# blackle/Megalania

Measured on AMD Instinct MI355X. Metric: SA neighbour-cost evals/s, higher is better.
Workload: dtype u64

## Files before the change

megalania_amd/csrc/mgl_api.hip:

```cpp
#include "mgl_kernels.hip"
#include "mgl_kernels2.hip"
#include "mgl_kernels3.hip"
#include "mgl_kernels4.hip"
#include "mgl_kernels5.hip"
#include "mgl_pbuild.hip"
#include "mgl_index.hip"
#include "../../include/megalania_hip.h"

#include <math.h>
#include <stdio.h>
#include <stdlib.h>
#include <string.h>
#include <string>
#include <vector>

static const uint16_t k_cost_table[2048] = {
#include "mgl_cost_table.inc"
};

#define MGL_MAX_INPUT 176000000ull
static thread_local std::string g_err;
static int fail(int code, const std::string& msg)
{
	g_err = msg;
	return code;
}
#define HIPCHK(expr)                                                                         \
	do {                                                                                     \
		hipError_t e_ = (expr);                                                              \
		if (e_ != hipSuccess)                                                                \
			return fail(MGL_EDEVICE, std::string(#expr) + ": " + hipGetErrorString(e_));     \
	} while (0)

__attribute__((constructor)) static void mgl_more_hw_queues(void) { if (getenv("MGL_LOOKAHEAD")) setenv("GPU_MAX_HW_QUEUES", "8", 0); }

extern "C" const char* mgl_version(void) { return "megalania-hip 0.1 (gfx950)"; }
extern "C" const char* mgl_last_error(void) { return g_err.c_str(); }
extern "C" int mgl_device_count(void)
{
	int n = 0;
	if (hipGetDeviceCount(&n) != hipSuccess) return 0;
	return n;
}
extern "C" uint32_t mgl_rng_draw_at(uint64_t seed, uint64_t step, uint32_t j, uint32_t n)
{
	return mgl_rng_draw(mgl_rng_key(seed, step, j), n);
}

struct BaseMem {
	BaseView v;
	Control* ctl;
};

struct mgl_sa {
	int device;
	hipStream_t stream;
	hipStream_t stream2;
	hipEvent_t ev_fork, ev_join;
	hipEvent_t ev_tgt = nullptr, ev_tgt_go = nullptr;
	int tgt_ahead = 0;
	hipStream_t stream3 = nullptr;
	hipEvent_t ev_rest[8] = { nullptr, nullptr, nullptr, nullptr, nullptr, nullptr, nullptr, nullptr }, ev_sim = nullptr;
	uint32_t halves;
	uint32_t n;
	mgl_properties props;
	mgl_sa_config cfg;
	uint64_t temperature = 0;
	DevCtx ctx;
	uint8_t* d_data;
	uint32_t* d_bucket_off;
	uint32_t* d_bucket_pos;
	uint16_t* d_bucket_nx;
	uint32_t* d_quad_pos;
	uint16_t* d_quad_nx;
	uint32_t *d_quad_rank = nullptr, *d_quad_run = nullptr;
	uint32_t* d_xpos[6] = { nullptr, nullptr, nullptr, nullptr, nullptr, nullptr };
	uint32_t* d_xrank[6] = { nullptr, nullptr, nullptr, nullptr, nullptr, nullptr };
	uint32_t* d_xrun[6] = { nullptr, nullptr, nullptr, nullptr, nullptr, nullptr };
	uint8_t* d_xnxb[6] = { nullptr, nullptr, nullptr, nullptr, nullptr, nullptr };
	uint32_t *d_oct_pos = nullptr, *d_oct_rank = nullptr, *d_oct_run = nullptr;
	uint32_t *d_hex_pos = nullptr, *d_hex_rank = nullptr, *d_hex_run = nullptr;
	uint64_t *d_oct_nx8 = nullptr, *d_hex_nx8 = nullptr;
	uint16_t* d_cost_tbl;
	BaseMem base, scratch;
	mgl_pk* d_best;
	NbrOut nbr;
	uint32_t* d_aos;
	uint64_t* d_cum;
	uint16_t* d_final_probs;
	mgl_pk* d_topk_pk;
	uint64_t* d_topk_cost;
	uint32_t* d_small;
	uint32_t* d_sub_offs;
	uint32_t* d_sub_lens;
	uint32_t sub_cap;
	uint64_t sqrt_thresh;
	uint32_t per_wave_bytes, waves_per_block, nbr_lds, walk_lds;
	bool incremental;
	Base2 b2;
	unsigned long long* d_prof;
	uint32_t* d_todo;
	uint32_t per_wave2, waves_per_block2, nbr2_lds, build_lds;
	uint32_t chg_cap = MGL_CHG_CAP;
	uint32_t per_wave_pick, per_wave_rest, pick_waves;
	size_t b2_bytes;
	BigScratch big;
	uint32_t* d_todo2;
	uint32_t* d_todo3 = nullptr;
	uint4* d_pickstate;
	uint4* d_pickrec;
	bool split_nbr, adaptive;
	bool form_single = false;
	uint32_t* d_counts;
	ApplyBuf ab;
	uint32_t apply_blocks;
	bool incremental_apply;
	bool snapshots;
	Base2 snap_lit, snap_best;
	SnapMeta* d_snap_meta;
	bool parallel_build;
	PBuild pb;
	hipEvent_t ev_begin, ev_end;
	std::vector<hipEvent_t> ev_pool;
	int accept_mode = MGL_ACCEPT_AUTO;
	uint32_t bulk_threshold = 0;
	bool bulk_now = true;
	uint64_t bulk_hold = 0;
	uint64_t blk_done = 0;
	uint64_t blk_imp0 = 0, blk_acc0 = 0;
	BulkBuf bulk;
	BatchBuf batch;
	bool batch_ok = false;
	uint32_t* d_strat_tgt = nullptr;
	uint32_t* d_strat_pre = nullptr;
	bool select_small = false;
	uint32_t* h_bstat = nullptr;
	hipEvent_t ev_bstat = nullptr;
	uint32_t force_batch_fail = 0;
	uint64_t batch_accepts = 0, batch_fallbacks = 0;
	std::vector<uint8_t> mode_log;
	uint32_t force_rollbacks = 0;
	uint64_t bulk_rollbacks = 0;
	bool best_unverified = false;
	struct NbrSet { NbrOut nbr; uint4* pickrec; uint4* pickstate; uint4* sim_hdr; uint16_t* sim_keys; uint32_t* sim_pos; uint32_t* todo; uint32_t* counts; };
	NbrSet alt = {};
	uint32_t sim_waves = MGL_SIM_WAVES;
	std::vector<hipEvent_t> ev_sim_pool;
	int64_t time_sim_step = -1;
	bool count_traffic = false;
	unsigned long long* d_traffic = nullptr;
	bool la_enabled = false, la_ready = false;
	hipGraph_t nbr_graph = nullptr; hipGraphExec_t nbr_graph_exec = nullptr; uint64_t nbr_graph_key = 0; bool graph_ok = false;
	uint32_t short_looks = 0;
	uint8_t* d_la_mark = nullptr;
	uint32_t* d_la_list = nullptr;
	uint32_t* d_la_hdr = nullptr;
	hipStream_t stream5 = nullptr, stream6 = nullptr;
	hipEvent_t ev_val = nullptr;
	hipEvent_t ev_la_check = nullptr, ev_la_zero = nullptr, ev_redo = nullptr, ev_spec[8] = { nullptr, nullptr, nullptr, nullptr, nullptr, nullptr, nullptr, nullptr };
};

static uint64_t ceil_sqrt_u64(uint64_t x)
{
	uint64_t r = (uint64_t)sqrt((double)x);
	while (r * r > x) r--;
	while ((r + 1) * (r + 1) <= x) r++;
	return r * r == x ? r : r + 1;
}

static void dfree(void* p) { if (p) (void)hipFree(p); }
static void free_base(BaseMem& b)
{
	dfree(b.v.slab); dfree(b.v.onwalk); dfree(b.v.ckpt_probs); dfree(b.v.ckpt_hdr); dfree(b.ctl);
	memset(&b, 0, sizeof b);
}
static hipError_t alloc_base(BaseMem& b, uint32_t n, uint32_t ckpt_elems)
{
	memset(&b, 0, sizeof b);
	hipError_t e;
	b.v.nckpt = (n + (1u << MGL_CKPT_SHIFT) - 1u) >> MGL_CKPT_SHIFT;
	b.v.ckpt_elems = ckpt_elems;
	if ((e = hipMalloc(&b.v.slab, sizeof(mgl_pk) * (size_t)n)) != hipSuccess) return e;
	if ((e = hipMalloc(&b.v.onwalk, sizeof(uint64_t) * (((size_t)n + 63) / 64 + 1))) != hipSuccess) return e;
	if ((e = hipMalloc(&b.v.ckpt_probs, sizeof(uint16_t) * (size_t)b.v.nckpt * ckpt_elems)) != hipSuccess) return e;
	if ((e = hipMalloc(&b.v.ckpt_hdr, sizeof(CkptHdr) * (size_t)b.v.nckpt)) != hipSuccess) return e;
	if ((e = hipMalloc(&b.ctl, sizeof(Control))) != hipSuccess) return e;
	if ((e = hipMemset(b.v.onwalk, 0, sizeof(uint64_t) * (((size_t)n + 63) / 64 + 1))) != hipSuccess) return e;
	return hipMemset(b.ctl, 0, sizeof(Control));
}

static size_t b2_pool_entries(const Base2& b) { return (size_t)b.pool_cap + 256; }
static int alloc_b2(Base2& b, size_t n, bool own_slab, bool init, size_t* bytes_out)
{
	size_t bytes = 0;
	if (own_slab) {
		HIPCHK(hipMalloc(&b.slab, sizeof(mgl_pk) * n)); bytes += sizeof(mgl_pk) * n;
		HIPCHK(hipMalloc(&b.onwalk, sizeof(uint64_t) * ((n + 63) / 64 + 1)));
	}
	HIPCHK(hipMalloc(&b.sp0, sizeof(uint64_t) * (b.nw0 + 64))); bytes += sizeof(uint64_t) * (b.nw0 + 64);
	HIPCHK(hipMalloc(&b.sp1, sizeof(uint64_t) * (b.nw1 + 64)));
	HIPCHK(hipMalloc(&b.sp2, sizeof(uint64_t) * (b.nw2 + 64)));
	HIPCHK(hipMalloc(&b.sp_state, sizeof(uint32_t) * 8 * n)); bytes += sizeof(uint32_t) * 8 * n;
	HIPCHK(hipMalloc(&b.ck_probs, sizeof(uint16_t) * (size_t)b.nck * b.ck_elems)); bytes += sizeof(uint16_t) * (size_t)b.nck * b.ck_elems;
	HIPCHK(hipMalloc(&b.ch_off, sizeof(uint32_t) * b.ck_elems));
	HIPCHK(hipMalloc(&b.ch_len, sizeof(uint32_t) * b.ck_elems));
	HIPCHK(hipMalloc(&b.ch_cap, sizeof(uint32_t) * b.ck_elems));
	HIPCHK(hipMalloc(&b.ch_pos, sizeof(uint32_t) * b2_pool_entries(b))); bytes += sizeof(uint32_t) * (size_t)b.pool_cap;
	HIPCHK(hipMalloc(&b.ch_ev, sizeof(uint16_t) * b2_pool_entries(b))); bytes += sizeof(uint16_t) * (size_t)b.pool_cap;
	HIPCHK(hipMalloc(&b.pool_top, sizeof(uint32_t)));
	HIPCHK(hipMalloc(&b.ch_sb, sizeof(uint32_t) * (size_t)b.ck_elems * b.sb_stride)); bytes += sizeof(uint32_t) * (size_t)b.ck_elems * b.sb_stride;
	if (init) {
		HIPCHK(hipMemset(b.ch_sb, 0, sizeof(uint32_t) * (size_t)b.ck_elems * b.sb_stride));
		HIPCHK(hipMemset(b.sp0, 0, sizeof(uint64_t) * (b.nw0 + 64)));
		HIPCHK(hipMemset(b.sp1, 0, sizeof(uint64_t) * (b.nw1 + 64)));
		HIPCHK(hipMemset(b.sp2, 0, sizeof(uint64_t) * (b.nw2 + 64)));
		HIPCHK(hipMemset(b.ch_pos, 0xFF, sizeof(uint32_t) * b2_pool_entries(b)));
		HIPCHK(hipMemset(b.ch_ev, 0, sizeof(uint16_t) * b2_pool_entries(b)));
	}
	if (bytes_out) *bytes_out = bytes;
	return MGL_OK;
}
static void free_b2(Base2& b, bool own_slab)
{
	if (own_slab) { dfree(b.slab); dfree(b.onwalk); }
	dfree(b.sp0); dfree(b.sp1); dfree(b.sp2); dfree(b.sp_state); dfree(b.ck_probs);
	dfree(b.ch_off); dfree(b.ch_len); dfree(b.ch_cap); dfree(b.ch_pos); dfree(b.ch_ev); dfree(b.pool_top); dfree(b.ch_sb);
	memset(&b, 0, sizeof b);
}
static int launch_snapshot(mgl_sa* sa, Base2& snap, uint32_t which, int dir, int cond)
{
	const Base2& from = dir == 0 ? sa->b2 : snap;
	const Base2& to = dir == 0 ? snap : sa->b2;
	const size_t n = sa->n;
	SnapPlan p;
	memset(&p, 0, sizeof p);
	uint32_t k = 0;
	auto seg = [&](const void* s, void* d, size_t bytes, uint32_t pool_elem) {
		p.seg[k].src = s; p.seg[k].dst = d; p.seg[k].bytes = bytes; p.seg[k].pool_elem = pool_elem; k++;
	};
	seg(from.slab, to.slab, sizeof(mgl_pk) * n, 0);
	seg(from.onwalk, to.onwalk, sizeof(uint64_t) * ((n + 63) / 64 + 1), 0);
	seg(from.sp0, to.sp0, sizeof(uint64_t) * (from.nw0 + 64), 0);
	seg(from.sp1, to.sp1, sizeof(uint64_t) * (from.nw1 + 64), 0);
	seg(from.sp2, to.sp2, sizeof(uint64_t) * (from.nw2 + 64), 0);
	seg(from.sp_state, to.sp_state, sizeof(uint32_t) * 8 * n, 0);
	seg(from.ck_probs, to.ck_probs, sizeof(uint16_t) * (size_t)from.nck * from.ck_elems, 0);
	seg(from.ch_off, to.ch_off, sizeof(uint32_t) * from.ck_elems, 0);
	seg(from.ch_len, to.ch_len, sizeof(uint32_t) * from.ck_elems, 0);
	seg(from.ch_cap, to.ch_cap, sizeof(uint32_t) * from.ck_elems, 0);
	seg(from.ch_pos, to.ch_pos, sizeof(uint32_t) * b2_pool_entries(from), 4);
	seg(from.ch_ev, to.ch_ev, sizeof(uint16_t) * b2_pool_entries(from), 2);
	seg(from.pool_top, to.pool_top, sizeof(uint32_t), 0);
	seg(from.ch_sb, to.ch_sb, sizeof(uint32_t) * (size_t)from.ck_elems * from.sb_stride, 0);
	p.nseg = k;
	p.src_pool_top = from.pool_top;
// ... 78 lines not shown
	hipLaunchKernelGGL(k_apply_walk, dim3(1), dim3(64), 0, sa->stream, sa->ctx, sa->b2, sa->base.ctl, sa->nbr, sa->ab);
	if (next_gstep != ~0ull) { int rc = launch_targets_ahead(sa, next_gstep); if (rc) return rc; }
	if (!sa->snapshots)
		hipLaunchKernelGGL(k_copy_best, dim3(256), dim3(256), 0, sa->stream, (const Control*)sa->base.ctl,
		                   (const mgl_pk*)sa->base.v.slab, sa->d_best, sa->ctx.n);
	hipLaunchKernelGGL(k_apply_chains, dim3(sa->apply_blocks), dim3(MGL_APPLY_THREADS), 0, sa->stream, sa->ctx, sa->b2, sa->base.ctl, sa->ab);
	hipLaunchKernelGGL(k_apply_jobs, dim3(1024), dim3(256), 0, sa->stream, sa->b2, (const Control*)sa->base.ctl, sa->ab, 0, (const uint32_t*)nullptr);
	hipLaunchKernelGGL(k_apply_jobs, dim3(1024), dim3(256), 0, sa->stream, sa->b2, (const Control*)sa->base.ctl, sa->ab, 1, (const uint32_t*)nullptr);
	hipLaunchKernelGGL(k_build_end, dim3(1), dim3(64), sa->build_lds, sa->stream, sa->ctx, sa->b2, sa->base.ctl, sa->snapshots ? 1 : 0, sa->d_counts, sa->adaptive ? 1 : 0, sa->form_single ? 1 : 0);
	HIPCHK(hipGetLastError());
	return MGL_OK;
}
static const bool g_trace = getenv("MGL_TRACE") != nullptr, g_prof_big = getenv("MGL_PROF_BIG") != nullptr, g_big_inline_sim = getenv("MGL_BIG_INLINE_SIM") != nullptr;
#define NBR_TRACE(name) do { if (g_trace) { fprintf(stderr, "[mgl] %s\n", name); hipError_t e_ = hipDeviceSynchronize(); if (e_ != hipSuccess) fprintf(stderr, "[mgl] %s -> %s\n", name, hipGetErrorString(e_)); } } while (0)
static hipEvent_t sim_event(mgl_sa* sa, size_t i)
{
	while (sa->ev_sim_pool.size() <= i) {
		hipEvent_t e = nullptr;
		if (hipEventCreate(&e) != hipSuccess) return nullptr;
		sa->ev_sim_pool.push_back(e);
	}
	return sa->ev_sim_pool[i];
}
static mgl_sa::NbrSet cur_set(const mgl_sa* sa)
{
	mgl_sa::NbrSet t = { sa->nbr, sa->d_pickrec, sa->d_pickstate, sa->big.sim_hdr, sa->big.sim_keys, sa->big.sim_pos, sa->d_todo, sa->d_counts };
	return t;
}
static void use_set(mgl_sa* sa, const mgl_sa::NbrSet& t)
{
	sa->nbr = t.nbr; sa->d_pickrec = t.pickrec; sa->d_pickstate = t.pickstate;
	sa->big.sim_hdr = t.sim_hdr; sa->big.sim_keys = t.sim_keys; sa->big.sim_pos = t.sim_pos;
	sa->d_todo = t.todo; sa->d_counts = t.counts;
	sa->big.todo_in = t.todo; sa->big.todo_in_count = t.counts; sa->big.spill_ctr = t.counts + 2;
}
static uint32_t nbr_slices(const mgl_sa* sa)
{
	const uint32_t K = sa->cfg.neighbours_per_step;
	return (sa->halves >= 2 && K >= 1024) ? sa->halves : 1u;
}
static int launch_pick_rest(mgl_sa* sa, const mgl_sa::NbrSet& t, uint64_t step_override, hipStream_t s_even, hipStream_t s_odd, hipEvent_t* done)
{
	const uint32_t K = sa->cfg.neighbours_per_step, slices = nbr_slices(sa);
	BigScratch g = sa->big;
	g.sim_hdr = t.sim_hdr; g.sim_keys = t.sim_keys; g.sim_pos = t.sim_pos;
	g.todo_in = t.todo; g.todo_in_count = t.counts; g.spill_ctr = t.counts + 2;
	for (uint32_t h = 0; h < slices; h++) {
		const uint32_t j0 = (uint32_t)((uint64_t)K * h / slices), j1 = (uint32_t)((uint64_t)K * (h + 1) / slices);
		hipStream_t st = (h & 1u) ? s_odd : s_even;
		hipLaunchKernelGGL((k_neighbours2<false, MGL_NBR_PICK>), dim3((j1 - j0 + sa->pick_waves - 1) / sa->pick_waves), dim3(64 * sa->pick_waves),
		                   (MGL_PICK_T_GLOBAL ? 0u : 4096u) + sa->pick_waves * sa->per_wave_pick, st, sa->ctx,
		                   sa->b2, sa->base.ctl, sa->cfg.seed, step_override, K, t.nbr, sa->per_wave_pick, t.todo, t.counts,
		                   (unsigned long long*)nullptr, g, t.pickrec, j0, j1, t.pickstate); NBR_TRACE("k_neighbours2<false, MGL_NBR_PICK>");
		hipLaunchKernelGGL((k_neighbours2<false, MGL_NBR_REST>), dim3(j1 - j0), dim3(64), sa->per_wave_rest, st, sa->ctx,
		                   sa->b2, sa->base.ctl, sa->cfg.seed, step_override, K, t.nbr, sa->per_wave_rest, t.todo, t.counts,
		                   g_prof_big ? (unsigned long long*)nullptr : sa->d_prof, g, t.pickrec, j0, j1, t.pickstate); NBR_TRACE("k_neighbours2<false, MGL_NBR_REST>");
		HIPCHK(hipEventRecord(done[h], st));
	}
	HIPCHK(hipGetLastError());
	return MGL_OK;
}
static int launch_lookahead(mgl_sa* sa, uint64_t gstep_next, bool after_check)
{
	const uint32_t slices = nbr_slices(sa);
	if (after_check) HIPCHK(hipStreamWaitEvent(sa->stream5, sa->ev_la_check, 0));
	else for (uint32_t h = 0; h < slices; h++) HIPCHK(hipStreamWaitEvent(sa->stream5, sa->ev_rest[h], 0));
	HIPCHK(hipMemsetAsync(sa->alt.counts, 0, 8 * sizeof(uint32_t), sa->stream5));
	HIPCHK(hipEventRecord(sa->ev_la_zero, sa->stream5));
	HIPCHK(hipStreamWaitEvent(sa->stream6, sa->ev_la_zero, 0));
	int rc = launch_pick_rest(sa, sa->alt, gstep_next, sa->stream5, sa->stream6, sa->ev_spec);
	if (rc) return rc;
	sa->la_ready = true;
	return MGL_OK;
}
static void launch_targets(mgl_sa* sa, hipStream_t st, uint64_t step_override)
{
	const uint32_t K = sa->cfg.neighbours_per_step;
	const uint64_t* onwalk = sa->incremental ? sa->b2.onwalk : sa->base.v.onwalk;
	const uint32_t nw0 = sa->incremental ? sa->b2.nw0 : (sa->ctx.n + 63u) >> 6;
	hipLaunchKernelGGL(k_rank_blocks, dim3(sa->ctx.strat_nblk), dim3(64), 0, st, onwalk, nw0, sa->d_strat_pre, sa->ctx.strat_nblk);
	hipLaunchKernelGGL(k_rank_scan, dim3(1), dim3(1024), 0, st, sa->d_strat_pre, sa->ctx.strat_nblk);
	hipLaunchKernelGGL(k_targets, dim3((K + 3u) / 4u), dim3(256), 0, st, sa->ctx, onwalk, nw0, (const Control*)sa->base.ctl, sa->cfg.seed, step_override, K, sa->d_strat_tgt);
}
static int launch_targets_ahead(mgl_sa* sa, uint64_t next_gstep)
{
	if (!sa->d_strat_pre || !sa->incremental) return MGL_OK;
	HIPCHK(hipEventRecord(sa->ev_tgt_go, sa->stream));
	HIPCHK(hipStreamWaitEvent(sa->stream2, sa->ev_tgt_go, 0));
	launch_targets(sa, sa->stream2, next_gstep);
	HIPCHK(hipEventRecord(sa->ev_tgt, sa->stream2));
	HIPCHK(hipGetLastError());
	sa->tgt_ahead = 1;
	return MGL_OK;
}
static uint64_t graph_key(const mgl_sa* sa);
static int launch_neighbours_body(mgl_sa* sa, uint64_t step_override, bool from_lookahead)
{
	const uint32_t K = sa->cfg.neighbours_per_step;
	const uint32_t blocks2 = (K + sa->waves_per_block2 - 1) / sa->waves_per_block2;
	const bool split_now = sa->split_nbr && !sa->form_single;
	const uint32_t sim_lds_regular = ((((sa->ctx.L.total + 31u) >> 5) + 3u) & ~3u) * 4u + sa->chg_cap * 16u;
	if (split_now) {
		const uint32_t slices = nbr_slices(sa);
		if (!from_lookahead) {
			HIPCHK(hipEventRecord(sa->ev_fork, sa->stream));
			if (slices >= 2) HIPCHK(hipStreamWaitEvent(sa->stream2, sa->ev_fork, 0));
			HIPCHK(hipStreamWaitEvent(sa->stream3, sa->ev_fork, 0));
			int rc = launch_pick_rest(sa, cur_set(sa), step_override, sa->stream, sa->stream2, sa->ev_rest);
			if (rc) return rc;
		} else {
			HIPCHK(hipMemsetAsync(sa->d_la_hdr, 0, 2 * sizeof(uint32_t), sa->stream));
			hipLaunchKernelGGL(k_la_check, dim3((K + 255u) / 256u), dim3(256), 0, sa->stream, sa->ctx, sa->b2, (const Control*)sa->base.ctl, sa->nbr,
			                   (const uint4*)sa->d_pickstate, sa->big.sim_hdr, (const uint32_t*)sa->d_counts, sa->d_la_mark, sa->d_la_list, sa->d_la_hdr, sa->cfg.seed, K); NBR_TRACE("k_la_check");
			HIPCHK(hipEventRecord(sa->ev_la_check, sa->stream));
			HIPCHK(hipStreamWaitEvent(sa->stream3, sa->ev_la_check, 0));
			HIPCHK(hipStreamWaitEvent(sa->stream2, sa->ev_la_check, 0));
		}
		for (uint32_t h = 0; h < slices; h++) {
			const uint32_t j0 = (uint32_t)((uint64_t)K * h / slices), j1 = (uint32_t)((uint64_t)K * (h + 1) / slices);
			if (!from_lookahead) HIPCHK(hipStreamWaitEvent(sa->stream3, sa->ev_rest[h], 0));
			if (sa->time_sim_step >= 0 && h < 2) HIPCHK(hipEventRecord(sim_event(sa, 6 * (size_t)sa->time_sim_step + 2 * h), sa->stream3));
			if (sa->count_traffic)
				hipLaunchKernelGGL(k_sim<true>, dim3(j1 - j0), dim3(64 * sa->sim_waves), sim_lds_regular, sa->stream3, sa->ctx, sa->b2, sa->base.ctl,
				                   sa->nbr, sa->big, j0, j1, sa->d_todo3, sa->d_counts + 4, (const uint32_t*)nullptr, (const uint32_t*)nullptr, sa->d_traffic);
			else
				hipLaunchKernelGGL(k_sim<false>, dim3(j1 - j0), dim3(64 * sa->sim_waves), sim_lds_regular, sa->stream3, sa->ctx, sa->b2, sa->base.ctl,
				                   sa->nbr, sa->big, j0, j1, sa->d_todo3, sa->d_counts + 4, (const uint32_t*)nullptr, (const uint32_t*)nullptr, (unsigned long long*)nullptr);
			NBR_TRACE("k_sim");
			if (sa->time_sim_step >= 0 && h < 2) HIPCHK(hipEventRecord(sim_event(sa, 6 * (size_t)sa->time_sim_step + 2 * h + 1), sa->stream3));
		}
		HIPCHK(hipEventRecord(sa->ev_sim, sa->stream3));
		if (!from_lookahead) {
			for (uint32_t h = 1; h < slices; h += 2) HIPCHK(hipStreamWaitEvent(sa->stream, sa->ev_rest[h], 0));
		} else {
			BigScratch g = sa->big;
			g.la_list = sa->d_la_list; g.la_count = sa->d_la_hdr;
			const uint32_t grid = blocks2 < 4096u ? blocks2 : 4096u;
			hipLaunchKernelGGL((k_neighbours2<false, MGL_NBR_FULL, true>), dim3(grid), dim3(64 * sa->waves_per_block2), sa->nbr2_lds, sa->stream2, sa->ctx,
			                   sa->b2, sa->base.ctl, sa->cfg.seed, step_override, K, sa->nbr, sa->per_wave2, sa->d_todo, sa->d_counts,
			                   sa->d_prof, g, sa->d_pickrec, 0u, K, sa->d_pickstate); NBR_TRACE("k_neighbours2<false, MGL_NBR_FULL, true>");
			HIPCHK(hipEventRecord(sa->ev_redo, sa->stream2));
		}
	}
	if (!sa->split_nbr || sa->form_single) {
		hipLaunchKernelGGL((k_neighbours2<false, MGL_NBR_FULL>), dim3(blocks2), dim3(64 * sa->waves_per_block2), sa->nbr2_lds, sa->stream, sa->ctx,
		                   sa->b2, sa->base.ctl, sa->cfg.seed, step_override, K, sa->nbr, sa->per_wave2, sa->d_todo, sa->d_counts,
		                   sa->d_prof, sa->big, sa->d_pickrec, 0u, K, sa->d_pickstate); NBR_TRACE("k_neighbours2<false, MGL_NBR_FULL>");
	}
	const uint32_t bigneed = (sa->big.slots + sa->waves_per_block2 - 1) / sa->waves_per_block2;
	const uint32_t bigblocks = bigneed < 1024u ? bigneed : 1024u;
	BigScratch big_now = sa->big;
	big_now.lds_cache = 1u;
	const uint32_t big_lds = sa->nbr2_lds + 12u * MGL_BIG_CAP;
	if (!split_now || g_big_inline_sim) big_now.sim_hdr2 = nullptr;
	const bool la_step = from_lookahead && split_now;
	if (la_step) {
		if (!sa->d_la_mark || !sa->d_la_hdr || !sa->d_la_list || !sa->d_todo || !sa->d_todo2 || !sa->d_pickrec || !sa->d_pickstate || !sa->big.ins_key || !sa->big.sim_slot2)
			return fail(MGL_EDEVICE, "launch_neighbours: look-ahead step without its buffers");
		big_now.la_mark = sa->d_la_mark; big_now.la_spec_count = sa->d_la_hdr + 1;
		big_now.todo_in_count = sa->d_la_hdr + 1;
	}
	if (la_step) {
		hipLaunchKernelGGL((k_neighbours2<true, MGL_NBR_FULL, true>), dim3(bigblocks), dim3(64 * sa->waves_per_block2), big_lds, sa->stream, sa->ctx,
		                   sa->b2, sa->base.ctl, sa->cfg.seed, step_override, K, sa->nbr, sa->per_wave2, sa->d_todo2, sa->d_counts + 1,
		                   (unsigned long long*)nullptr, big_now, sa->d_pickrec, 0u, K, sa->d_pickstate); NBR_TRACE("k_neighbours2<true, MGL_NBR_FULL, true>");
	} else {
		hipLaunchKernelGGL((k_neighbours2<true, MGL_NBR_FULL>), dim3(bigblocks), dim3(64 * sa->waves_per_block2), big_lds, sa->stream, sa->ctx,
		                   sa->b2, sa->base.ctl, sa->cfg.seed, step_override, K, sa->nbr, sa->per_wave2, sa->d_todo2, sa->d_counts + 1,
		                   g_prof_big ? sa->d_prof : (unsigned long long*)nullptr, big_now, (sa->split_nbr && !sa->form_single) ? sa->d_pickrec : (uint4*)nullptr, 0u, K, sa->d_pickstate); NBR_TRACE("k_neighbours2<true, MGL_NBR_FULL>");
	}
	if (la_step) {
		HIPCHK(hipStreamWaitEvent(sa->stream, sa->ev_redo, 0));
		big_now.todo_in_count = sa->d_counts;
		big_now.todo_first = sa->d_la_hdr + 1;
		hipLaunchKernelGGL((k_neighbours2<true, MGL_NBR_FULL, true>), dim3(bigblocks < 256u ? bigblocks : 256u), dim3(64 * sa->waves_per_block2), big_lds, sa->stream, sa->ctx,
		                   sa->b2, sa->base.ctl, sa->cfg.seed, step_override, K, sa->nbr, sa->per_wave2, sa->d_todo2, sa->d_counts + 1,
		                   (unsigned long long*)nullptr, big_now, sa->d_pickrec, 0u, K, sa->d_pickstate); NBR_TRACE("k_neighbours2<true, MGL_NBR_FULL, true>");
		big_now.todo_first = nullptr;
	}
	if (split_now) {
		const uint32_t sim_lds = ((((sa->ctx.L.total + 31u) >> 5) + 3u) & ~3u) * 4u + MGL_SIM2_CAP * 16u;
		if (sa->time_sim_step >= 0) HIPCHK(hipEventRecord(sim_event(sa, 6 * (size_t)sa->time_sim_step + 4), sa->stream));
		if (sa->count_traffic)
			hipLaunchKernelGGL(k_sim<true>, dim3(256), dim3(64 * MGL_SIM_WAVES_LIST), sim_lds, sa->stream, sa->ctx, sa->b2, sa->base.ctl, sa->nbr, big_now, 0u, K,
			                   sa->d_todo3, sa->d_counts + 4, (const uint32_t*)sa->d_todo, (const uint32_t*)sa->d_counts, sa->d_traffic);
		else
			hipLaunchKernelGGL(k_sim<false>, dim3(256), dim3(64 * MGL_SIM_WAVES_LIST), sim_lds, sa->stream, sa->ctx, sa->b2, sa->base.ctl, sa->nbr, big_now, 0u, K,
			                   sa->d_todo3, sa->d_counts + 4, (const uint32_t*)sa->d_todo, (const uint32_t*)sa->d_counts, (unsigned long long*)nullptr);
		NBR_TRACE("k_sim");
		if (sa->time_sim_step >= 0) HIPCHK(hipEventRecord(sim_event(sa, 6 * (size_t)sa->time_sim_step + 5), sa->stream));
		HIPCHK(hipStreamWaitEvent(sa->stream, sa->ev_sim, 0));
		BigScratch late = sa->big;
		late.todo_in = sa->d_todo3; late.todo_in_count = sa->d_counts + 4; late.sim_hdr2 = nullptr; late.lds_cache = 1u;
		late.cont = nullptr;
		hipLaunchKernelGGL((k_neighbours2<true, MGL_NBR_FULL>), dim3(bigblocks < 64u ? bigblocks : 64u), dim3(64 * sa->waves_per_block2), big_lds, sa->stream, sa->ctx,
		                   sa->b2, sa->base.ctl, sa->cfg.seed, step_override, K, sa->nbr, sa->per_wave2, sa->d_todo2, sa->d_counts + 1,
		                   (unsigned long long*)nullptr, late, sa->d_pickrec, 0u, K, sa->d_pickstate); NBR_TRACE("k_neighbours2<true, MGL_NBR_FULL>");
	}
	const uint32_t blocks = (K + sa->waves_per_block - 1) / sa->waves_per_block;
	hipLaunchKernelGGL(k_neighbours, dim3(blocks < 256u ? blocks : 256u), dim3(64 * sa->waves_per_block), sa->nbr_lds, sa->stream, sa->ctx, sa->base.v,
	                   (const Control*)sa->base.ctl, sa->cfg.seed, step_override, K, sa->nbr, sa->per_wave_bytes,
	                   (const uint32_t*)sa->d_todo2, (const uint32_t*)(sa->d_counts + 1)); NBR_TRACE("k_neighbours");
	HIPCHK(hipGetLastError());
	return MGL_OK;
}

static int launch_neighbours(mgl_sa* sa, uint64_t step_override, bool zero_counts = true, bool from_lookahead = false)
{
	const uint32_t K = sa->cfg.neighbours_per_step;
	if (sa->d_strat_pre) {
		if (sa->tgt_ahead) HIPCHK(hipStreamWaitEvent(sa->stream, sa->ev_tgt, 0));
		if (sa->tgt_ahead != 1) launch_targets(sa, sa->stream, step_override);
		sa->tgt_ahead = 0;
	}
	if (!sa->incremental) {
		const uint32_t blocks = (K + sa->waves_per_block - 1) / sa->waves_per_block;
		hipLaunchKernelGGL(k_neighbours, dim3(blocks), dim3(64 * sa->waves_per_block), sa->nbr_lds, sa->stream, sa->ctx, sa->base.v,
		                   (const Control*)sa->base.ctl, sa->cfg.seed, step_override, K, sa->nbr, sa->per_wave_bytes,
		                   (const uint32_t*)nullptr, (const uint32_t*)nullptr); NBR_TRACE("k_neighbours");
		HIPCHK(hipGetLastError());
		return MGL_OK;
	}
	if (zero_counts) HIPCHK(hipMemsetAsync(sa->d_counts, 0, 8 * sizeof(uint32_t), sa->stream));
	if (sa->graph_ok && step_override == ~0ull && !from_lookahead && !sa->la_enabled && sa->time_sim_step < 0 && !sa->count_traffic && !g_trace && !g_prof_big && sa->d_prof == nullptr) {
		const uint64_t key = graph_key(sa);
		if (sa->nbr_graph_exec == nullptr || key != sa->nbr_graph_key) {
			if (sa->nbr_graph_exec) { (void)hipGraphExecDestroy(sa->nbr_graph_exec); sa->nbr_graph_exec = nullptr; }
			if (sa->nbr_graph) { (void)hipGraphDestroy(sa->nbr_graph); sa->nbr_graph = nullptr; }
			HIPCHK(hipStreamBeginCapture(sa->stream, hipStreamCaptureModeRelaxed));
			const int rc = launch_neighbours_body(sa, ~0ull, false);
			const hipError_t ec = hipStreamEndCapture(sa->stream, &sa->nbr_graph);
			if (rc) return rc;
			if (ec != hipSuccess || sa->nbr_graph == nullptr) return fail(MGL_EDEVICE, "launch_neighbours: graph capture failed");
			HIPCHK(hipGraphInstantiate(&sa->nbr_graph_exec, sa->nbr_graph, nullptr, nullptr, 0));
			sa->nbr_graph_key = key;
		}
		HIPCHK(hipGraphLaunch(sa->nbr_graph_exec, sa->stream));
		return MGL_OK;
	}
	return launch_neighbours_body(sa, step_override, from_lookahead);
}

static uint64_t graph_key(const mgl_sa* sa)
{
	uint64_t h = 1469598103934665603ull;
	auto mix = [&](const void* p, size_t n) { const unsigned char* c = (const unsigned char*)p; for (size_t i = 0; i < n; i++) { h ^= c[i]; h *= 1099511628211ull; } };
	mix(&sa->ctx, sizeof sa->ctx); mix(&sa->b2, sizeof sa->b2); mix(&sa->base, sizeof sa->base); mix(&sa->nbr, sizeof sa->nbr); mix(&sa->big, sizeof sa->big);
	const uint64_t w[] = { sa->cfg.neighbours_per_step, sa->cfg.seed, (uint64_t)sa->form_single, (uint64_t)sa->split_nbr, sa->halves, sa->waves_per_block, sa->waves_per_block2,
	                       sa->pick_waves, sa->per_wave_pick, sa->per_wave_rest, sa->per_wave2, sa->per_wave_bytes, sa->nbr_lds, sa->nbr2_lds, sa->chg_cap, sa->sim_waves,
	                       (uint64_t)(uintptr_t)sa->d_todo, (uint64_t)(uintptr_t)sa->d_todo2, (uint64_t)(uintptr_t)sa->d_todo3, (uint64_t)(uintptr_t)sa->d_counts,
	                       (uint64_t)(uintptr_t)sa->d_pickrec, (uint64_t)(uintptr_t)sa->d_pickstate, (uint64_t)g_big_inline_sim };
	mix(w, sizeof w);
	return h;
}

static int import_slab(mgl_sa* sa, const mgl_packet* packets, mgl_pk* d_slab)
{
	HIPCHK(hipMemcpyAsync(sa->d_aos, packets, sizeof(mgl_packet) * (size_t)sa->n, hipMemcpyHostToDevice, sa->stream));
	hipLaunchKernelGGL(k_import, dim3(1024), dim3(256), 0, sa->stream, (const uint32_t*)sa->d_aos, d_slab, sa->n);
	HIPCHK(hipGetLastError());
	return MGL_OK;
}
static int export_slab(mgl_sa* sa, const mgl_pk* d_slab, mgl_packet* packets)
{
	hipLaunchKernelGGL(k_export, dim3(1024), dim3(256), 0, sa->stream, d_slab, sa->d_aos, sa->n);
	HIPCHK(hipGetLastError());
	HIPCHK(hipMemcpyAsync(packets, sa->d_aos, sizeof(mgl_packet) * (size_t)sa->n, hipMemcpyDeviceToHost, sa->stream));
	HIPCHK(hipStreamSynchronize(sa->stream));
	return MGL_OK;
}

extern "C" void mgl_sa_destroy(mgl_sa* sa)
{
	if (!sa) return;
	(void)hipSetDevice(sa->device);
	if (sa->stream) (void)hipStreamSynchronize(sa->stream);
	dfree(sa->d_data); dfree(sa->d_bucket_off); dfree(sa->d_bucket_pos); dfree(sa->d_bucket_nx); dfree(sa->d_quad_pos); dfree(sa->d_quad_nx); dfree(sa->d_cost_tbl);
	dfree(sa->d_quad_rank); dfree(sa->d_quad_run); dfree(sa->d_oct_pos);
	for (int i = 0; i < 6; i++) { if (i != 0 && i != 2) { dfree(sa->d_xpos[i]); dfree(sa->d_xrank[i]); dfree(sa->d_xrun[i]); } dfree(sa->d_xnxb[i]); } dfree(sa->d_oct_rank); dfree(sa->d_oct_run);
	dfree(sa->d_hex_pos); dfree(sa->d_hex_rank); dfree(sa->d_hex_run); dfree(sa->d_oct_nx8); dfree(sa->d_hex_nx8);
	free_base(sa->base); free_base(sa->scratch);
	if (!sa->snapshots) dfree(sa->d_best);
	dfree(sa->nbr.cost); dfree(sa->nbr.ndiffs); dfree(sa->nbr.walked); dfree(sa->nbr.win); dfree(sa->nbr.win2); dfree(sa->nbr.dpos);
	dfree(sa->bulk.ckey); dfree(sa->bulk.cwin); dfree(sa->bulk.taken); dfree(sa->bulk.cstate); dfree(sa->bulk.cflags); dfree(sa->bulk.hdr);
	dfree(sa->nbr.dold); dfree(sa->nbr.dnew);
	dfree(sa->d_aos); dfree(sa->d_cum); dfree(sa->d_final_probs);
	free_b2(sa->b2, false);
	free_b2(sa->snap_lit, true); free_b2(sa->snap_best, true); dfree(sa->d_snap_meta);
	dfree(sa->pb.exits); dfree(sa->pb.entry); dfree(sa->pb.gexits); dfree(sa->pb.gentry); dfree(sa->pb.gsum); dfree(sa->pb.ch_map); dfree(sa->pb.ch_vs); dfree(sa->pb.ch_pk); dfree(sa->pb.ch_state); dfree(sa->pb.tf_ctx); dfree(sa->pb.tf_dist); dfree(sa->pb.tf_pk);
	dfree(sa->pb.st_in); dfree(sa->pb.hist); dfree(sa->pb.stage); dfree(sa->pb.stage_n); dfree(sa->pb.stage_over); dfree(sa->pb.acc); dfree(sa->pb.seg_off); dfree(sa->pb.unres);
	{
		mgl_sa::NbrSet& t = sa->alt;
		dfree(t.nbr.cost); dfree(t.nbr.ndiffs); dfree(t.nbr.walked); dfree(t.nbr.win); dfree(t.nbr.win2); dfree(t.nbr.dpos); dfree(t.nbr.dold); dfree(t.nbr.dnew);
		dfree(t.pickrec); dfree(t.pickstate); dfree(t.sim_hdr); dfree(t.sim_keys); dfree(t.sim_pos); dfree(t.todo); dfree(t.counts);
		dfree(sa->d_la_mark); dfree(sa->d_la_list); dfree(sa->d_la_hdr);
		if (sa->stream5) (void)hipStreamDestroy(sa->stream5);
		if (sa->stream6) (void)hipStreamDestroy(sa->stream6);
		if (sa->ev_la_check) (void)hipEventDestroy(sa->ev_la_check);
		if (sa->ev_la_zero) (void)hipEventDestroy(sa->ev_la_zero);
		if (sa->ev_redo) (void)hipEventDestroy(sa->ev_redo);
		for (int i = 0; i < 8; i++) if (sa->ev_spec[i]) (void)hipEventDestroy(sa->ev_spec[i]);
	}
	dfree(sa->d_todo); dfree(sa->d_prof);
	dfree(sa->big.sim_hdr); dfree(sa->big.sim_keys); dfree(sa->big.sim_pos);
	dfree(sa->big.ins_key); dfree(sa->big.rem_key); dfree(sa->big.ins_pos); dfree(sa->big.rem_pos); dfree(sa->big.uctx);
	if (sa->h_bstat) (void)hipHostFree(sa->h_bstat);
	if (sa->ev_bstat) (void)hipEventDestroy(sa->ev_bstat);
	dfree(sa->big.cont); dfree(sa->d_traffic); dfree(sa->d_strat_pre); dfree(sa->d_strat_tgt);
	{
		BatchBuf& bt = sa->batch;
		dfree(bt.hdr); dfree(bt.cl); dfree(bt.jpos); dfree(bt.jnew); dfree(bt.jold); dfree(bt.st_ikey); dfree(bt.st_rkey); dfree(bt.st_ipos);
		dfree(bt.st_rpos); dfree(bt.ops); dfree(bt.ins_cl); dfree(bt.rem_cl); dfree(bt.acc); dfree(bt.runs);
		dfree(bt.cnt_i); dfree(bt.cnt_r); dfree(bt.off_i); dfree(bt.off_r); dfree(bt.cur_i); dfree(bt.cur_r); dfree(bt.touched);
		dfree(bt.bk_ipos); dfree(bt.bk_rpos); dfree(bt.bk_ibit); dfree(bt.bk_icl); dfree(bt.bk_rcl);
	}
	for (hipEvent_t e : sa->ev_sim_pool) if (e) (void)hipEventDestroy(e);
	dfree(sa->d_todo2); dfree(sa->d_todo3); dfree(sa->d_counts); dfree(sa->big.sim_hdr2); dfree(sa->big.sim_slot2); dfree(sa->d_pickrec); dfree(sa->d_pickstate);
	dfree(sa->ab.hdr); dfree(sa->ab.ins_key); dfree(sa->ab.rem_key); dfree(sa->ab.ins_pos); dfree(sa->ab.rem_pos);
	dfree(sa->ab.tctx); dfree(sa->ab.scratch_pos); dfree(sa->ab.scratch_ev);
	dfree(sa->ab.span_pos); dfree(sa->ab.span_ev); dfree(sa->ab.jobs_b); dfree(sa->ab.jobs_c);
	dfree(sa->d_topk_pk); dfree(sa->d_topk_cost); dfree(sa->d_small); dfree(sa->d_sub_offs); dfree(sa->d_sub_lens);
	for (hipEvent_t e : sa->ev_pool) (void)hipEventDestroy(e);
	if (sa->ev_begin) (void)hipEventDestroy(sa->ev_begin);
	if (sa->ev_end) (void)hipEventDestroy(sa->ev_end);
	if (sa->stream2) (void)hipStreamDestroy(sa->stream2);
	if (sa->stream3) (void)hipStreamDestroy(sa->stream3);
	for (auto& e : sa->ev_rest) if (e) (void)hipEventDestroy(e);
	if (sa->ev_sim) (void)hipEventDestroy(sa->ev_sim);
	if (sa->ev_val) (void)hipEventDestroy(sa->ev_val);
	if (sa->nbr_graph_exec) (void)hipGraphExecDestroy(sa->nbr_graph_exec);
	if (sa->nbr_graph) (void)hipGraphDestroy(sa->nbr_graph);
	if (sa->ev_fork) (void)hipEventDestroy(sa->ev_fork);
	if (sa->ev_tgt) (void)hipEventDestroy(sa->ev_tgt);
	if (sa->ev_tgt_go) (void)hipEventDestroy(sa->ev_tgt_go);
	if (sa->ev_join) (void)hipEventDestroy(sa->ev_join);
	if (sa->stream) (void)hipStreamDestroy(sa->stream);
	delete sa;
}

static int create_impl(mgl_sa* sa, const uint8_t* data, size_t n)
{
	HIPCHK(hipSetDevice(sa->device));
	HIPCHK(hipStreamCreate(&sa->stream));
	HIPCHK(hipStreamCreate(&sa->stream2));
	HIPCHK(hipEventCreateWithFlags(&sa->ev_fork, hipEventDisableTiming));
	HIPCHK(hipEventCreateWithFlags(&sa->ev_join, hipEventDisableTiming));
	HIPCHK(hipEventCreateWithFlags(&sa->ev_tgt, hipEventDisableTiming));
	HIPCHK(hipEventCreateWithFlags(&sa->ev_tgt_go, hipEventDisableTiming));
// ... 177 lines not shown
		if (sa->parallel_build) {
			PBuild& pb = sa->pb;
			memset(&pb, 0, sizeof pb);
			pb.shift = b.sb_shift;
			pb.nblk = (uint32_t)((n + (1u << pb.shift) - 1) >> pb.shift);
			HIPCHK(hipMalloc(&pb.exits, sizeof(uint16_t) * (size_t)pb.nblk * MGL_PB_ENTRIES));
			HIPCHK(hipMalloc(&pb.entry, sizeof(uint32_t) * ((size_t)pb.nblk + 1)));
			pb.ngrp = (pb.nblk + MGL_PB_GROUP - 1u) / MGL_PB_GROUP;
			HIPCHK(hipMalloc(&pb.gexits, sizeof(uint16_t) * (size_t)pb.ngrp * MGL_PB_ENTRIES));
			HIPCHK(hipMalloc(&pb.gentry, sizeof(uint16_t) * (size_t)pb.ngrp));
			{
				const size_t nch = ((size_t)pb.nblk + MGL_PB_SCAN_CHUNK - 1u) / MGL_PB_SCAN_CHUNK;
				HIPCHK(hipMalloc(&pb.ch_map, sizeof(uint64_t) * nch));
				HIPCHK(hipMalloc(&pb.ch_vs, sizeof(uint32_t) * 8 * nch));
				HIPCHK(hipMalloc(&pb.ch_pk, sizeof(uint32_t) * nch));
				HIPCHK(hipMalloc(&pb.ch_state, sizeof(uint32_t) * 8 * nch));
			}
			HIPCHK(hipMalloc(&pb.gsum, sizeof(uint32_t) * (size_t)((pb.nblk + MGL_PB_OFF_ROWS - 1u) / MGL_PB_OFF_ROWS) * ckpt_elems));
			HIPCHK(hipMalloc(&pb.tf_ctx, sizeof(uint64_t) * pb.nblk));
			HIPCHK(hipMalloc(&pb.tf_dist, sizeof(uint32_t) * 8 * (size_t)pb.nblk));
			HIPCHK(hipMalloc(&pb.tf_pk, sizeof(uint32_t) * pb.nblk));
			HIPCHK(hipMalloc(&pb.st_in, sizeof(uint32_t) * 8 * (size_t)pb.nblk));
			HIPCHK(hipMalloc(&pb.hist, sizeof(uint32_t) * (size_t)pb.nblk * ckpt_elems));
			HIPCHK(hipMalloc(&pb.stage, sizeof(uint64_t) * (size_t)pb.nblk * ((MGL_PB_STAGE_PER_POS << pb.shift) + 32u)));
			HIPCHK(hipMalloc(&pb.stage_n, sizeof(uint32_t) * (size_t)pb.nblk));
			HIPCHK(hipMalloc(&pb.stage_over, sizeof(uint32_t)));
			HIPCHK(hipMemset(pb.stage_over, 0, sizeof(uint32_t)));
			HIPCHK(hipMalloc(&pb.acc, sizeof(unsigned long long) * 16));
			HIPCHK(hipMemset(pb.acc, 0, sizeof(unsigned long long) * 16));
			pb.seg_cap = b.pool_cap / MGL_PB_SEG + ckpt_elems + 64u;
			HIPCHK(hipMalloc(&pb.seg_off, sizeof(uint32_t) * (ckpt_elems + 1)));
			HIPCHK(hipMalloc(&pb.unres, pb.seg_cap));
		}
		sa->snapshots = !(sa->cfg.flags & MGL_F_NO_SNAPSHOTS);
		if (sa->snapshots) {
			for (Base2* s : { &sa->snap_lit, &sa->snap_best }) {
				*s = b;
				s->slab = nullptr; s->onwalk = nullptr; s->sp0 = s->sp1 = s->sp2 = nullptr; s->sp_state = nullptr;
				s->ck_probs = nullptr; s->ch_off = s->ch_len = s->ch_cap = s->ch_pos = nullptr; s->ch_ev = nullptr;
				s->pool_top = nullptr;
				int rc = alloc_b2(*s, n, true, false, nullptr);
				if (rc) return rc;
			}
			HIPCHK(hipMalloc(&sa->d_snap_meta, sizeof(SnapMeta) * 2));
			HIPCHK(hipMemset(sa->d_snap_meta, 0, sizeof(SnapMeta) * 2));
			sa->d_best = sa->snap_best.slab;
		}
		if (sa->cfg.flags & MGL_F_PROFILE) {
			HIPCHK(hipMalloc(&sa->d_prof, sizeof(unsigned long long) * (32 + K)));
			HIPCHK(hipMemset(sa->d_prof, 0, sizeof(unsigned long long) * (32 + K)));
		}
		HIPCHK(hipMalloc(&sa->d_todo, sizeof(uint32_t) * (K + 1)));
		HIPCHK(hipMemset(sa->d_todo, 0, sizeof(uint32_t) * (K + 1)));
		sa->b2_bytes = bytes;
		sa->incremental_apply = getenv("MGL_NO_INCREMENTAL_APPLY") == nullptr;
		{
			ApplyBuf& ab = sa->ab;
			memset(&ab, 0, sizeof ab);
			sa->apply_blocks = 256;
			ab.scratch_cap = b.pool_cap + 256u;
			ab.span_cap = 1u << 22;
			ab.job_cap = 1u << 20;
			HIPCHK(hipMalloc(&ab.hdr, sizeof(uint32_t) * 16));
			HIPCHK(hipMemset(ab.hdr, 0, sizeof(uint32_t) * 16));
			HIPCHK(hipMalloc(&ab.ins_key, sizeof(uint16_t) * MGL_BATCH_ALLOC));
			HIPCHK(hipMalloc(&ab.rem_key, sizeof(uint16_t) * MGL_BATCH_ALLOC));
			HIPCHK(hipMalloc(&ab.ins_pos, sizeof(uint32_t) * MGL_BATCH_ALLOC));
			HIPCHK(hipMalloc(&ab.rem_pos, sizeof(uint32_t) * MGL_BATCH_ALLOC));
			HIPCHK(hipMalloc(&ab.tctx, sizeof(uint16_t) * 16384));
			HIPCHK(hipMalloc(&ab.scratch_pos, sizeof(uint32_t) * (size_t)ab.scratch_cap));
			HIPCHK(hipMalloc(&ab.scratch_ev, sizeof(uint16_t) * (size_t)ab.scratch_cap));
			HIPCHK(hipMalloc(&ab.span_pos, sizeof(uint32_t) * (size_t)ab.span_cap));
			HIPCHK(hipMalloc(&ab.span_ev, sizeof(uint16_t) * (size_t)ab.span_cap));
			HIPCHK(hipMalloc(&ab.jobs_b, sizeof(uint4) * (size_t)ab.job_cap));
			HIPCHK(hipMalloc(&ab.jobs_c, sizeof(uint4) * (size_t)ab.job_cap));
			BatchBuf& bt = sa->batch;
			memset(&bt, 0, sizeof bt);
			HIPCHK(hipMalloc(&bt.hdr, sizeof(uint32_t) * 16));
			HIPCHK(hipMemset(bt.hdr, 0, sizeof(uint32_t) * 16));
			HIPCHK(hipMalloc(&bt.cl, sizeof(uint32_t) * 8 * MGL_BATCH_MAX));
			HIPCHK(hipMalloc(&bt.jpos, sizeof(uint32_t) * MGL_BATCH_MAX * MGL_MAX_DIFFS));
			HIPCHK(hipMalloc(&bt.jnew, sizeof(mgl_pk) * MGL_BATCH_MAX * MGL_MAX_DIFFS));
			HIPCHK(hipMalloc(&bt.jold, sizeof(mgl_pk) * MGL_BATCH_MAX * MGL_MAX_DIFFS));
			HIPCHK(hipMalloc(&bt.st_ikey, sizeof(uint16_t) * MGL_BATCH_ALLOC));
			HIPCHK(hipMalloc(&bt.st_rkey, sizeof(uint16_t) * MGL_BATCH_ALLOC));
			HIPCHK(hipMalloc(&bt.st_ipos, sizeof(uint32_t) * MGL_BATCH_ALLOC));
			HIPCHK(hipMalloc(&bt.st_rpos, sizeof(uint32_t) * MGL_BATCH_ALLOC));
			HIPCHK(hipMalloc(&bt.ops, sizeof(uint4) * 2 * (size_t)MGL_BATCH_MAX * MGL_BATCH_OPCAP));
			HIPCHK(hipMalloc(&bt.ins_cl, MGL_BATCH_ALLOC));
			HIPCHK(hipMalloc(&bt.rem_cl, MGL_BATCH_ALLOC));
			bt.nctx = L.total;
			bt.runs_cap = 1u << 17;
			HIPCHK(hipMalloc(&bt.runs, sizeof(uint4) * 2 * (size_t)bt.runs_cap));
			for (uint32_t** p : { &bt.cnt_i, &bt.cnt_r, &bt.off_i, &bt.off_r, &bt.cur_i, &bt.cur_r, &bt.touched }) {
				HIPCHK(hipMalloc(p, sizeof(uint32_t) * (bt.nctx + 64u)));
				HIPCHK(hipMemset(*p, 0, sizeof(uint32_t) * (bt.nctx + 64u)));
			}
			HIPCHK(hipMalloc(&bt.bk_ipos, sizeof(uint32_t) * MGL_BATCH_ALLOC));
			HIPCHK(hipMalloc(&bt.bk_rpos, sizeof(uint32_t) * MGL_BATCH_ALLOC));
			HIPCHK(hipMalloc(&bt.bk_ibit, sizeof(uint16_t) * MGL_BATCH_ALLOC));
			HIPCHK(hipMalloc(&bt.bk_icl, MGL_BATCH_ALLOC));
			HIPCHK(hipMalloc(&bt.bk_rcl, MGL_BATCH_ALLOC));
			HIPCHK(hipMalloc(&bt.acc, sizeof(long long) * 4));
			HIPCHK(hipMemset(bt.acc, 0, sizeof(long long) * 4));
			HIPCHK(hipHostMalloc((void**)&sa->h_bstat, sizeof(uint32_t) * 16, hipHostMallocDefault));
			HIPCHK(hipEventCreateWithFlags(&sa->ev_bstat, hipEventDisableTiming));
			sa->batch_ok = sa->incremental_apply && getenv("MGL_NO_BATCH") == nullptr;

		}
		{
			const uint32_t fixed = MGL_MAX_DIFFS * (8u + 8u + 4u) + (((((L.total + 31u) >> 5) + 3u) & ~3u) * 4u) ;
			const uint32_t model = ckpt_elems * 2u + MGL_PRICE_WORDS * 4u;
			sa->chg_cap = K <= 1024u ? 4u * MGL_CHG_CAP : (K <= 2048u ? 2u * MGL_CHG_CAP : MGL_CHG_CAP);
			const uint32_t lists = sa->chg_cap * (4u + 4u + 2u + 2u) + 2u * sa->chg_cap * 2u;
			sa->per_wave2 = (fixed + (model > lists ? model : lists) + 15u) & ~15u;
			sa->per_wave_pick = (model + 15u) & ~15u;
			sa->per_wave_rest = (fixed + lists + 15u) & ~15u;
		}
		{
			BigScratch& g = sa->big;
			memset(&g, 0, sizeof g);
			g.chg_cap = sa->chg_cap;
			g.cap = MGL_BIG_CAP; g.uctx_cap = ckpt_elems; g.slots = (uint32_t)(K > 512 ? K : 512);
			HIPCHK(hipMalloc(&g.ins_key, sizeof(uint16_t) * (size_t)g.cap * g.slots));
			HIPCHK(hipMalloc(&g.rem_key, sizeof(uint16_t) * (size_t)g.cap * g.slots));
			HIPCHK(hipMalloc(&g.ins_pos, sizeof(uint32_t) * (size_t)g.cap * g.slots));
			HIPCHK(hipMalloc(&g.rem_pos, sizeof(uint32_t) * (size_t)g.cap * g.slots));
			HIPCHK(hipMalloc(&g.uctx, sizeof(uint16_t) * (size_t)g.uctx_cap * g.slots));
			HIPCHK(hipMalloc(&sa->d_todo2, sizeof(uint32_t) * (K + 1)));
			HIPCHK(hipMemset(sa->d_todo2, 0, sizeof(uint32_t) * (K + 1)));
		}
		{
			uint32_t best_w = 1, best_total = 0;
			for (uint32_t w = 1; w <= 8; w++) {
				const uint32_t bytes = 4096u + w * sa->per_wave2;
				if (bytes > 160u * 1024u) break;
				const uint32_t tot = (160u * 1024u / bytes) * w;
				if (tot > best_total) { best_total = tot; best_w = w; }
			}
			(void)best_w;
			sa->waves_per_block2 = 1;
		}
		sa->nbr2_lds = 4096u + sa->waves_per_block2 * sa->per_wave2;
		sa->build_lds = 4096u + ckpt_elems * 2u + ckpt_elems * 8u;
		HIPCHK(hipMalloc(&sa->d_counts, sizeof(uint32_t) * 16));
		HIPCHK(hipMemset(sa->d_counts, 0, sizeof(uint32_t) * 16));
		HIPCHK(hipMalloc(&sa->d_todo3, sizeof(uint32_t) * (K + 1)));
		HIPCHK(hipMemset(sa->d_todo3, 0, sizeof(uint32_t) * (K + 1)));
		sa->big.todo_in = sa->d_todo; sa->big.todo_in_count = sa->d_counts; sa->big.spill_ctr = sa->d_counts + 2;
		HIPCHK(hipFuncSetAttribute((const void*)k_neighbours2<false, MGL_NBR_FULL>, hipFuncAttributeMaxDynamicSharedMemorySize, (int)sa->nbr2_lds));
		HIPCHK(hipFuncSetAttribute((const void*)k_neighbours2<false, MGL_NBR_FULL, true>, hipFuncAttributeMaxDynamicSharedMemorySize, (int)sa->nbr2_lds));
		HIPCHK(hipFuncSetAttribute((const void*)k_neighbours2<false, MGL_NBR_PICK>, hipFuncAttributeMaxDynamicSharedMemorySize, 160 * 1024));
		HIPCHK(hipFuncSetAttribute((const void*)k_neighbours2<false, MGL_NBR_REST>, hipFuncAttributeMaxDynamicSharedMemorySize, (int)sa->nbr2_lds));
		HIPCHK(hipFuncSetAttribute((const void*)k_neighbours2<true, MGL_NBR_FULL>, hipFuncAttributeMaxDynamicSharedMemorySize, (int)(sa->nbr2_lds + 12u * MGL_BIG_CAP)));
		HIPCHK(hipFuncSetAttribute((const void*)k_neighbours2<true, MGL_NBR_FULL, true>, hipFuncAttributeMaxDynamicSharedMemorySize, (int)(sa->nbr2_lds + 12u * MGL_BIG_CAP)));
		HIPCHK(hipMalloc(&sa->d_pickrec, sizeof(uint4) * K));
		HIPCHK(hipMalloc(&sa->d_pickstate, sizeof(uint4) * 2 * K));
		sa->split_nbr = getenv("MGL_NO_SPLIT") == nullptr;
		if (sa->split_nbr) {
			BigScratch& g = sa->big;
			HIPCHK(hipMalloc(&g.sim_hdr, sizeof(uint4) * (size_t)K));
			HIPCHK(hipMalloc(&g.sim_keys, sizeof(uint16_t) * 2u * sa->chg_cap * (size_t)K));
			HIPCHK(hipMalloc(&g.sim_pos, sizeof(uint32_t) * 2u * sa->chg_cap * (size_t)K));
			HIPCHK(hipMemset(g.sim_hdr, 0xFF, sizeof(uint4) * (size_t)K));
			HIPCHK(hipMalloc(&g.sim_hdr2, sizeof(uint4) * (size_t)K));
			HIPCHK(hipMalloc(&g.sim_slot2, sizeof(uint32_t) * (size_t)K));
			HIPCHK(hipMemset(g.sim_hdr2, 0xFF, sizeof(uint4) * (size_t)K));
			if (getenv("MGL_NO_CONT") == nullptr && getenv("MGL_LOOKAHEAD") == nullptr) {
				HIPCHK(hipMalloc(&g.cont, sizeof(uint32_t) * MGL_CONT_WORDS * (size_t)g.slots));
				HIPCHK(hipMemset(g.cont, 0, sizeof(uint32_t) * MGL_CONT_WORDS * (size_t)g.slots));
			}
			sa->la_enabled = sa->incremental_apply && getenv("MGL_LOOKAHEAD") != nullptr;
			if (sa->la_enabled) {
				mgl_sa::NbrSet& t = sa->alt;
				HIPCHK(hipMalloc(&t.nbr.cost, sizeof(uint64_t) * K));
				HIPCHK(hipMalloc(&t.nbr.ndiffs, sizeof(uint32_t) * K));
				HIPCHK(hipMalloc(&t.nbr.walked, sizeof(uint32_t) * K));
				HIPCHK(hipMalloc(&t.nbr.win, sizeof(uint32_t) * 2 * K));
				HIPCHK(hipMemset(t.nbr.win, 0xFF, sizeof(uint32_t) * 2 * K));
				HIPCHK(hipMalloc(&t.nbr.win2, sizeof(uint32_t) * K));
				HIPCHK(hipMemset(t.nbr.win2, 0xFF, sizeof(uint32_t) * K));
				HIPCHK(hipMalloc(&t.nbr.dpos, sizeof(uint32_t) * K * MGL_MAX_DIFFS));
				HIPCHK(hipMalloc(&t.nbr.dold, sizeof(mgl_pk) * K * MGL_MAX_DIFFS));
				HIPCHK(hipMalloc(&t.nbr.dnew, sizeof(mgl_pk) * K * MGL_MAX_DIFFS));
				HIPCHK(hipMalloc(&t.pickrec, sizeof(uint4) * K));
				HIPCHK(hipMalloc(&t.pickstate, sizeof(uint4) * 2 * K));
				HIPCHK(hipMalloc(&t.sim_hdr, sizeof(uint4) * (size_t)K));
				HIPCHK(hipMemset(t.sim_hdr, 0xFF, sizeof(uint4) * (size_t)K));
				HIPCHK(hipMalloc(&t.sim_keys, sizeof(uint16_t) * 2u * sa->chg_cap * (size_t)K));
				HIPCHK(hipMalloc(&t.sim_pos, sizeof(uint32_t) * 2u * sa->chg_cap * (size_t)K));
				HIPCHK(hipMalloc(&t.todo, sizeof(uint32_t) * (K + 1)));
				HIPCHK(hipMemset(t.todo, 0, sizeof(uint32_t) * (K + 1)));
				HIPCHK(hipMalloc(&t.counts, sizeof(uint32_t) * 16));
				HIPCHK(hipMemset(t.counts, 0, sizeof(uint32_t) * 16));
				HIPCHK(hipMalloc(&sa->d_la_mark, K));
				HIPCHK(hipMemset(sa->d_la_mark, 0, K));
				HIPCHK(hipMalloc(&sa->d_la_list, sizeof(uint32_t) * K));
				HIPCHK(hipMalloc(&sa->d_la_hdr, sizeof(uint32_t) * 2));
				HIPCHK(hipMemset(sa->d_la_hdr, 0, sizeof(uint32_t) * 2));
				int plo = 0, phi = 0;
				HIPCHK(hipDeviceGetStreamPriorityRange(&plo, &phi));
				HIPCHK(hipStreamCreateWithPriority(&sa->stream5, hipStreamDefault, plo));
				HIPCHK(hipStreamCreateWithPriority(&sa->stream6, hipStreamDefault, plo));
				HIPCHK(hipEventCreateWithFlags(&sa->ev_redo, hipEventDisableTiming));
				HIPCHK(hipEventCreateWithFlags(&sa->ev_la_check, hipEventDisableTiming));
				HIPCHK(hipEventCreateWithFlags(&sa->ev_la_zero, hipEventDisableTiming));
				for (int i = 0; i < 8; i++) HIPCHK(hipEventCreateWithFlags(&sa->ev_spec[i], hipEventDisableTiming));
			}
		}
		if (getenv("MGL_SIMW")) { const int w = atoi(getenv("MGL_SIMW")); if (w == 1 || w == 2 || w == 4 || w == 8) sa->sim_waves = (uint32_t)w; }
		sa->adaptive = sa->split_nbr && getenv("MGL_NO_ADAPT") == nullptr;
		sa->form_single = !sa->split_nbr;
		sa->pick_waves = getenv("MGL_PICK_WAVES") ? (uint32_t)atoi(getenv("MGL_PICK_WAVES")) : 0u;
		if (sa->pick_waves != 1 && sa->pick_waves != 2 && sa->pick_waves != 4 && sa->pick_waves != 8) sa->pick_waves = 0;
		{
			uint32_t best_w = 1, best_resident = 0;
			for (uint32_t w = 1; w <= 8; w *= 2) {
				const uint32_t bytes = (MGL_PICK_T_GLOBAL ? 0u : 4096u) + w * sa->per_wave_pick;
				if (bytes > 160u * 1024u) break;
				const uint32_t resident = (160u * 1024u / ((bytes + 1279u) / 1280u * 1280u)) * w;
				if (resident > best_resident) { best_resident = resident; best_w = w; }
			}
			if (n > (1u << 20)) best_w = 1;
			if (sa->pick_waves == 0 || (MGL_PICK_T_GLOBAL ? 0u : 4096u) + sa->pick_waves * sa->per_wave_pick > 160u * 1024u) sa->pick_waves = best_w;
		}
		HIPCHK(hipFuncSetAttribute((const void*)k_sim<false>, hipFuncAttributeMaxDynamicSharedMemorySize, 96 * 1024));
		HIPCHK(hipFuncSetAttribute((const void*)k_sim<true>, hipFuncAttributeMaxDynamicSharedMemorySize, 96 * 1024));
		HIPCHK(hipMalloc(&sa->d_traffic, sizeof(unsigned long long) * 2));
		HIPCHK(hipMemset(sa->d_traffic, 0, sizeof(unsigned long long) * 2));
		HIPCHK(hipFuncSetAttribute((const void*)k_build, hipFuncAttributeMaxDynamicSharedMemorySize, (int)sa->build_lds));
		HIPCHK(hipFuncSetAttribute((const void*)k_build_end, hipFuncAttributeMaxDynamicSharedMemorySize, (int)sa->build_lds));
	}

	if (!(sa->cfg.flags & MGL_F_POSITION_TARGETS) && !sa->la_enabled && getenv("MGL_POSITION_TARGETS") == nullptr) {
		sa->ctx.strat_nblk = (uint32_t)((n + 4095u) / 4096u);
		HIPCHK(hipMalloc(&sa->d_strat_pre, sizeof(uint32_t) * (sa->ctx.strat_nblk + 2u)));
		HIPCHK(hipMemset(sa->d_strat_pre, 0, sizeof(uint32_t) * (sa->ctx.strat_nblk + 2u)));
		sa->ctx.strat_pre = sa->d_strat_pre;
		HIPCHK(hipMalloc(&sa->d_strat_tgt, sizeof(uint32_t) * sa->cfg.neighbours_per_step));
		sa->ctx.strat_tgt = sa->d_strat_tgt;
	}
	sa->sqrt_thresh = ceil_sqrt_u64(sa->cfg.iters_per_epoch);
	sa->bulk_threshold = getenv("MGL_BULK_THRESHOLD") ? (uint32_t)atoi(getenv("MGL_BULK_THRESHOLD"))
	                     : sa->batch_ok ? 2u : (n <= (1u << 20) ? 16u : n <= (1u << 24) ? 32u : 128u);
	if (sa->bulk_threshold == 0) sa->bulk_threshold = 1;

	hipLaunchKernelGGL(k_fill_literal, dim3(1024), dim3(256), 0, sa->stream, sa->base.v.slab, sa->ctx.n);
	if (!sa->d_best) HIPCHK(hipMalloc(&sa->d_best, sizeof(mgl_pk) * n));
	hipLaunchKernelGGL(k_fill_literal, dim3(1024), dim3(256), 0, sa->stream, sa->d_best, sa->ctx.n);
	HIPCHK(hipGetLastError());
	int rc = rebuild_base(sa, 0);
	if (rc) return rc;
	if (sa->incremental && sa->snapshots && (rc = launch_snapshot(sa, sa->snap_lit, 0, 0, 0))) return rc;
	HIPCHK(hipStreamSynchronize(sa->stream));
	{
		Control c0;
		HIPCHK(hipMemcpy(&c0, sa->base.ctl, sizeof c0, hipMemcpyDeviceToHost));
		if (c0.error_flags) return fail(MGL_EDEVICE, "mgl_sa_create: building the base structures of the all-literal slab failed");
	}
	return MGL_OK;
}

extern "C" mgl_sa* mgl_sa_create(const uint8_t* data, size_t n, mgl_properties props, const mgl_sa_config* cfg)
{
	if (!data || n == 0 || !cfg) { fail(MGL_EINVAL, "mgl_sa_create: bad data/size/config"); return nullptr; }
	if (n > MGL_MAX_INPUT) { fail(MGL_EINVAL, "mgl_sa_create: input larger than 176 000 000 bytes is not supported"); return nullptr; }
	if (props.lc + props.lp > 4 || props.pb > 4 || props.lc > 8) { fail(MGL_EINVAL, "mgl_sa_create: unsupported lc/lp/pb"); return nullptr; }
	mgl_sa* sa = new (std::nothrow) mgl_sa();
	if (!sa) { fail(MGL_ENOMEM, "mgl_sa_create: out of host memory"); return nullptr; }
	sa->cfg = *cfg;
	sa->props = props;
	sa->n = (uint32_t)n;
	sa->device = cfg->device;
	if (sa->cfg.neighbours_per_step == 0) sa->cfg.neighbours_per_step = 1;
	if (sa->cfg.neighbours_per_step > (1u << 20)) { delete sa; fail(MGL_EINVAL, "neighbours_per_step > 2^20"); return nullptr; }
	if (sa->cfg.top_k == 0) sa->cfg.top_k = 20;
	if (sa->cfg.top_k > MGL_MAX_TOPK) { delete sa; fail(MGL_EINVAL, "top_k > 32"); return nullptr; }
	if (sa->cfg.dict_limit == 0) sa->cfg.dict_limit = 0x400000u;
	if (sa->cfg.iters_per_epoch == 0) sa->cfg.iters_per_epoch = n;
	int rc = create_impl(sa, data, n);
	if (rc != MGL_OK) {
		std::string keep = g_err;
		mgl_sa_destroy(sa);
		g_err = keep;
		return nullptr;
	}
	return sa;
}

static int read_ctl(mgl_sa* sa, BaseMem& b, Control* out)
{
	HIPCHK(hipMemcpyAsync(out, b.ctl, sizeof(Control), hipMemcpyDeviceToHost, sa->stream));
	HIPCHK(hipStreamSynchronize(sa->stream));
	return MGL_OK;
}
static int write_ctl(mgl_sa* sa, BaseMem& b, const Control* in)
{
	HIPCHK(hipMemcpyAsync(b.ctl, in, sizeof(Control), hipMemcpyHostToDevice, sa->stream));
	HIPCHK(hipStreamSynchronize(sa->stream));
	return MGL_OK;
}

static int keep_best_before_overwrite(mgl_sa* sa, Control& c)
{
	if (!(sa->incremental && sa->snapshots) || !c.best_is_current) return MGL_OK;
	int rc = launch_snapshot(sa, sa->snap_best, 1, 0, 0);
	if (rc) return rc;
	c.best_is_current = 0;
	return MGL_OK;
}

// ... 630 lines not shown
```

megalania_amd/csrc/mgl_kernels.hip:

```cpp
#include "mgl_device.h"


struct TopK {
	uint64_t key;
	uint32_t count;
	uint32_t k;
};

__device__ __forceinline__ uint64_t topk_make_key(uint32_t cost, uint64_t seq)
{
	return ((uint64_t)cost << 44) | (MGL_SEQ_MASK - seq);
}
__device__ __forceinline__ uint64_t topk_threshold(const TopK& t)
{
	return t.count < t.k ? MGL_INVALID_COST : rdlane64(t.key, t.k - 1u);
}
__device__ __forceinline__ void topk_offer(TopK& t, uint64_t cand, uint32_t lane, bool allow_batch = true)
{
	const uint64_t thr0 = topk_threshold(t);
	unsigned long long m = __ballot(cand < thr0);
	if (!m) return;
	if (allow_batch && __popcll(m) >= 4) {
		uint32_t less_e = 0, less_c = 0, e_less = 0;
		for (unsigned long long mm = m; mm; mm &= mm - 1ull) {
			const uint32_t j = (uint32_t)__ffsll((long long)mm) - 1u;
			const uint64_t x = rdlane64(cand, j);
			less_e += x < t.key ? 1u : 0u;
			less_c += x < cand ? 1u : 0u;
			const uint32_t below = (uint32_t)__popcll(__ballot(t.key < x));
			if (lane == j) e_less = below;
		}
		const bool mine = (m >> lane) & 1ull;
		uint32_t dest_e = lane < t.count ? lane + less_e : 63u;
		uint32_t dest_c = mine ? e_less + less_c : 63u;
		dest_e = dest_e < 63u ? dest_e : 63u; dest_c = dest_c < 63u ? dest_c : 63u;
		const uint64_t ve = lane < t.count ? t.key : 0ull, vc = mine ? cand : 0ull;
		const uint32_t lo = (uint32_t)__builtin_amdgcn_ds_permute((int)(dest_e << 2), (int)(uint32_t)ve) |
		                    (uint32_t)__builtin_amdgcn_ds_permute((int)(dest_c << 2), (int)(uint32_t)vc);
		const uint32_t hi = (uint32_t)__builtin_amdgcn_ds_permute((int)(dest_e << 2), (int)(uint32_t)(ve >> 32)) |
		                    (uint32_t)__builtin_amdgcn_ds_permute((int)(dest_c << 2), (int)(uint32_t)(vc >> 32));
		uint32_t nc = t.count + (uint32_t)__popcll(m);
		nc = nc < t.k ? nc : t.k;
		t.count = nc;
		t.key = lane < nc ? ((uint64_t)lo | ((uint64_t)hi << 32)) : MGL_INVALID_COST;
		return;
	}
	for (;;) {
		uint64_t thr = topk_threshold(t);
		m = __ballot(cand < thr);
		if (!m) break;
		int src = __ffsll((long long)m) - 1;
		uint64_t x = rdlane64(cand, (uint32_t)src);
		uint32_t r = (uint32_t)__popcll(__ballot(t.key < x));
		uint64_t up = shfl_up64(t.key, 1);
		if (lane == r) t.key = x;
		else if (lane > r) t.key = up;
		if (lane >= t.k) t.key = MGL_INVALID_COST;
		if (t.count < t.k) t.count++;
		if ((int)lane == src) cand = MGL_INVALID_COST;
	}
}

__device__ __forceinline__ uint32_t bit_cost(const uint16_t* probs, const uint16_t* T, uint32_t ctx, uint32_t bit)
{
	uint32_t p = probs[ctx];
	return T[bit ? 2048u - p : p];
}
__device__ __forceinline__ uint32_t tree_cost(const uint16_t* probs, const uint16_t* T, uint32_t base,
                                              uint32_t val, uint32_t nbits)
{
	uint32_t m = 1, c = 0;
	for (uint32_t i = nbits; i-- > 0;) {
		uint32_t b = (val >> i) & 1u;
		c += bit_cost(probs, T, base + m, b);
		m = (m << 1) | b;
	}
	return c;
}
__device__ __forceinline__ uint32_t rev_tree_cost(const uint16_t* probs, const uint16_t* T, uint32_t base,
                                                  uint32_t val, uint32_t nbits)
{
	uint32_t m = 1, c = 0;
	for (uint32_t i = 0; i < nbits; i++) {
		uint32_t b = val & 1u;
		val >>= 1;
		c += bit_cost(probs, T, base + m, b);
		m = (m << 1) | b;
	}
	return c;
}
__device__ __forceinline__ uint32_t length_cost(const uint16_t* probs, const uint16_t* T, uint32_t base,
                                                uint32_t len, uint32_t pos_state)
{
	uint32_t l = len - 2;
	if (l < 8) return bit_cost(probs, T, base, 0) + tree_cost(probs, T, base + MGL_LEN_LOW + pos_state * 8, l, 3);
	uint32_t c = bit_cost(probs, T, base, 1);
	if (l < 16) return c + bit_cost(probs, T, base + 1, 0) + tree_cost(probs, T, base + MGL_LEN_MID + pos_state * 8, l - 8, 3);
	return c + bit_cost(probs, T, base + 1, 1) + tree_cost(probs, T, base + MGL_LEN_HIGH, l - 16, 8);
}

__device__ __forceinline__ uint32_t bucket_lower_bound(const uint32_t* bp, uint32_t a, uint32_t b, uint32_t x, uint32_t lane)
{
	while (b > a) {
		uint32_t span = b - a;
		uint32_t step = (span + 63u) / 64u;
		uint32_t idx = a + lane * step;
		bool ge = idx >= b ? true : (bp[idx] >= x);
		unsigned long long m = __ballot(ge);
		int f = m ? __ffsll((long long)m) - 1 : 64;
		if (f == 0) break;
		uint32_t na = a + (uint32_t)(f - 1) * step + 1u;
		uint32_t nb = a + (uint32_t)f * step;
		if (nb > b) nb = b;
		a = na; b = nb;
	}
	return a;
}

__device__ __forceinline__ uint32_t nx_lower_bound(const uint16_t* a, uint32_t lo, uint32_t hi, uint32_t x, uint32_t lane)
{
	while (hi > lo) {
		const uint32_t span = hi - lo, step = (span + 63u) / 64u;
		const uint32_t idx = lo + lane * step;
		const bool ge = idx >= hi ? true : ((uint32_t)a[idx] >= x);
		const unsigned long long m = __ballot(ge);
		const int f = m ? __ffsll((long long)m) - 1 : 64;
		if (f == 0) break;
		const uint32_t na = lo + (uint32_t)(f - 1) * step + 1u;
		uint32_t nb = lo + (uint32_t)f * step;
		if (nb > hi) nb = hi;
		lo = na; hi = nb;
	}
	return lo;
}

template <int W>
__device__ void topk_find(TopK& t, const DevCtx& c, const Walk& w, const uint16_t* probs, const uint16_t* T,
                          uint32_t* lencost, mgl_pk incumbent, uint32_t lane)
{
	const uint32_t pos = w.st.pos;
	const uint32_t state = w.st.ctx_state;
	const uint32_t pos_state = pos & ((1u << c.L.pb) - 1u);
	const uint32_t sp = (state << 4) + pos_state;
	t.key = MGL_INVALID_COST;
	t.count = 0;
	t.k = c.top_k;

	const uint32_t c_m1 = bit_cost(probs, T, MGL_CS_IS_MATCH + sp, 1);
	const uint32_t c_r0 = bit_cost(probs, T, MGL_CS_IS_REP + state, 0);
	const uint32_t c_r1 = bit_cost(probs, T, MGL_CS_IS_REP + state, 1);
	const uint32_t g0_0 = bit_cost(probs, T, MGL_CS_G0 + state, 0), g0_1 = bit_cost(probs, T, MGL_CS_G0 + state, 1);
	const uint32_t g1_0 = bit_cost(probs, T, MGL_CS_G1 + state, 0), g1_1 = bit_cost(probs, T, MGL_CS_G1 + state, 1);
	const uint32_t g2_0 = bit_cost(probs, T, MGL_CS_G2 + state, 0), g2_1 = bit_cost(probs, T, MGL_CS_G2 + state, 1);
	const uint32_t l_0 = bit_cost(probs, T, MGL_CS_REP0_LONG + sp, 0), l_1 = bit_cost(probs, T, MGL_CS_REP0_LONG + sp, 1);
	const uint32_t hdr_match = c_m1 + c_r0;
	const uint32_t hdr_rep = c_m1 + c_r1;
	const uint32_t hdr_lr0 = hdr_rep + g0_0 + l_1, hdr_lr1 = hdr_rep + g0_1 + g1_0;
	const uint32_t hdr_lr2 = hdr_rep + g0_1 + g1_1 + g2_0, hdr_lr3 = hdr_rep + g0_1 + g1_1 + g2_1;

	uint32_t* slotcost = lencost + 544;
	uint32_t* disttail = lencost + 800;
	uint32_t* aligncost = lencost + 928;
	if (lane < 32) {
		const uint32_t l = 2 + (lane & 15u);
		const uint32_t base = lane < 16 ? MGL_OFF_LEN : MGL_OFF_REP_LEN;
		lencost[(lane < 16 ? 0 : 272) + l - 2] = length_cost(probs, T, base, l, pos_state);
	}
	for (uint32_t e = lane; e < 256; e += 64) slotcost[e] = tree_cost(probs, T, MGL_OFF_DIST + (e & ~63u), e & 63u, 6);
	for (uint32_t d = 4 + lane; d < 128; d += 64) {
		const uint32_t nlow = mgl_msb32(d) - 2, low = d & ((1u << nlow) - 1u), high = d >> nlow;
		disttail[d] = rev_tree_cost(probs, T, MGL_OFF_DIST + MGL_DIST_POS + (high << nlow) - (nlow * 2 + high), low, nlow);
	}
	if (lane < 16) aligncost[lane] = rev_tree_cost(probs, T, MGL_OFF_DIST + MGL_DIST_ALIGN, lane, 4);
	bool high_ready = false;
	wave_sync();
	uint32_t* lbslot = lencost + 944;
	uint32_t* sufmin = lencost + 1008;
	{
		const uint32_t slot = lane;
		uint32_t m = slotcost[slot];
		for (uint32_t k = 1; k < 4; k++) { const uint32_t v = slotcost[64u * k + slot]; m = v < m ? v : m; }
		uint32_t amin = lane < 16 ? aligncost[lane] : 0xFFFFFFFFu;
		for (int o = 8; o > 0; o >>= 1) { const uint32_t a2 = (uint32_t)__shfl_xor((int)amin, o, 64); amin = a2 < amin ? a2 : amin; }
		amin = uni(amin);
		if (slot >= 14) m += (((slot >> 1) - 5u) << 11) + amin;
		lbslot[slot] = m;
		uint32_t sm = m;
		for (int o = 1; o < 64; o <<= 1) {
			const uint32_t tdn = (uint32_t)__shfl_down((int)sm, o, 64);
			if ((int)lane + o < 64) sm = tdn < sm ? tdn : sm;
		}
		sufmin[slot] = sm;
	}
	wave_sync();
	if (c.diag_stop == 31) return;
	uint32_t minlen_m, minlen_r;
	{
		uint32_t a = lane < 16 ? lencost[lane] : 0xFFFFFFFFu, b = lane < 16 ? lencost[272 + lane] : 0xFFFFFFFFu;
		for (int o = 8; o > 0; o >>= 1) {
			const uint32_t a2 = (uint32_t)__shfl_xor((int)a, o, 64), b2 = (uint32_t)__shfl_xor((int)b, o, 64);
			a = a2 < a ? a2 : a; b = b2 < b ? b2 : b;
		}
		minlen_m = uni(a); minlen_r = uni(b);
	}

	{
		uint64_t cand = MGL_INVALID_COST;
		uint32_t byte = walk_byte_at(w, pos);
		uint32_t rep_byte = (pos > 0 && w.st.dists[0] < pos) ? c.data[pos - w.st.dists[0] - 1] : 0x100u;
		uint32_t prev_byte = (c.L.lc > 0 && pos > 0) ? c.data[pos - 1] : 0;
		mgl_plan pl;
		mgl_plan_packet(&c.L, &w.st, MGL_LITERAL, 0, 1, byte, rep_byte, prev_byte, &pl);
		uint32_t ec = 0;
		if (lane < pl.nev) {
			uint32_t ctx, bit;
			mgl_plan_event(&pl, lane, &ctx, &bit);
			ec = bit_cost(probs, T, ctx, bit);
		}
		uint32_t lit = (uint32_t)wave_sum64(ec);
		if (lane == 0 && incumbent != MGL_PK_LITERAL) cand = topk_make_key(lit, 0);
		if (lane == 1 && pos > 0 && byte == rep_byte && incumbent != MGL_PK_SHORT_REP)
			cand = topk_make_key(hdr_rep + g0_0 + l_0, 1);
		topk_offer(t, cand, lane);
	}

	if (c.diag_stop == 32) return;
	if (pos == 0 || pos >= c.n - 1) return;
	const uint32_t bigram = ((uint32_t)walk_byte_at(w, pos) << 8) | c.data[pos + 1];
	uint32_t lo = c.bucket_off[bigram];
	const uint32_t end = c.bucket_off[bigram + 1];
	const uint32_t hi = bucket_lower_bound(c.bucket_pos, lo, end, pos, lane);
	if (pos > c.dict_limit) lo = bucket_lower_bound(c.bucket_pos, lo, hi, pos - c.dict_limit, lane);
	if (c.max_scan && hi - lo > c.max_scan) lo = hi - c.max_scan;
	const uint32_t nhits = hi - lo;
	if (c.diag_stop == 33) { t.count += nhits & 1u; return; }
	if (nhits == 0) return;
	const uint32_t wpos = c.bucket_pos[lo];
	const uint32_t maxlen = (c.n - pos) < MGL_MAX_MATCH ? (c.n - pos) : MGL_MAX_MATCH;
	const uint32_t inc_type = mgl_pk_type(incumbent), inc_len = mgl_pk_len(incumbent), inc_dist = mgl_pk_dist(incumbent);

	auto price_high_lengths = [&]() {
		for (uint32_t l = 18 + lane; l <= MGL_MAX_MATCH; l += 64) {
			lencost[l - 2] = length_cost(probs, T, MGL_OFF_LEN, l, pos_state);
			lencost[272 + l - 2] = length_cost(probs, T, MGL_OFF_REP_LEN, l, pos_state);
		}
		high_ready = true;
		wave_sync();
		uint32_t a = 0xFFFFFFFFu, b = 0xFFFFFFFFu;
		for (uint32_t l = 16 + lane; l < 272; l += 64) { a = lencost[l] < a ? lencost[l] : a; b = lencost[272 + l] < b ? lencost[272 + l] : b; }
		for (int o = 32; o > 0; o >>= 1) {
			const uint32_t a2 = (uint32_t)__shfl_xor((int)a, o, 64), b2 = (uint32_t)__shfl_xor((int)b, o, 64);
			a = a2 < a ? a2 : a; b = b2 < b ? b2 : b;
		}
		minlen_m = a < minlen_m ? uni(a) : minlen_m; minlen_r = b < minlen_r ? uni(b) : minlen_r;
	};

	if (c.diag_stop == 34) return;
	{
		const uint32_t b0 = bigram >> 8, b1 = bigram & 0xFFu;
#pragma unroll
		for (uint32_t k = 0; k < 4; k++) {
			const uint32_t dk = mgl_dist_at(&w.st, k);
			if (dk >= pos) continue;
			const uint32_t q = pos - dk - 1u;
			if (q < wpos || c.data[q] != b0 || c.data[q + 1] != b1) continue;
			uint32_t L = maxlen;
			for (uint32_t base = 0; base < maxlen; base += 64) {
				const uint32_t i = base + lane;
				const bool stop = i >= maxlen || c.data[q + i] != c.data[pos + i];
				const unsigned long long m = __ballot(stop);
				if (m) { const uint32_t f = base + (uint32_t)__ffsll((long long)m) - 1u; L = f < maxlen ? f : maxlen; break; }
			}
			if (L >= 18 && !high_ready) price_high_lengths();
			const uint32_t hdr = k == 0 ? hdr_lr0 : k == 1 ? hdr_lr1 : k == 2 ? hdr_lr2 : hdr_lr3;
			for (uint32_t top = L; top >= 2;) {
				const uint64_t thr = topk_threshold(t);
				const bool nolim = thr == MGL_INVALID_COST;
				const uint32_t lim = nolim ? 0u : (uint32_t)(thr >> 44) + 1u;
				if (!nolim && hdr + minlen_r >= lim * top) break;
				uint64_t cand = MGL_INVALID_COST;
				if (lane + 2u <= top) {
					const uint32_t len = top - lane;
					const uint32_t perp = hdr + lencost[272 + len - 2];
					if ((nolim || perp < lim * len) && !(inc_type == MGL_LONG_REP && len == inc_len && inc_dist == k)) {
						const uint64_t key = topk_make_key(perp / len, ((uint64_t)(q + 1) << 12) | ((uint64_t)len << 3) | (1u + k));
						if (key < thr) cand = key;
					}
				}
				topk_offer(t, cand, lane);
				top = top > 64u + 1u ? top - 64u : 0u;
			}
		}
	}

	uint64_t x8, x16, x0;
	__builtin_memcpy(&x0, c.data + pos, 8);
	__builtin_memcpy(&x8, c.data + pos + 8, 8);
	__builtin_memcpy(&x16, c.data + pos + 16, 8);
	const uint32_t r8 = c.oct_rank[pos], r16 = c.hex_rank[pos];
	const uint32_t l8 = bucket_lower_bound(c.oct_pos, c.oct_run[r8], r8, wpos, lane);
	const uint32_t l16 = bucket_lower_bound(c.hex_pos, c.hex_run[r16], r16, wpos, lane);
	if (c.diag_stop == 35) return;
	uint32_t min15;
	{
		uint32_t m15 = lane < 14 ? lencost[lane] : 0xFFFFFFFFu;
		for (int o = 8; o > 0; o >>= 1) { const uint32_t d2 = (uint32_t)__shfl_xor((int)m15, o, 64); m15 = d2 < m15 ? d2 : m15; }
		min15 = uni(m15);
	}
	uint32_t lim32;
	{ const uint64_t th = topk_threshold(t); lim32 = th == MGL_INVALID_COST ? 0xFFFFFFFFu : (uint32_t)(th >> 44) + 1u; }
	auto price_hits = [&](uint32_t hq, uint32_t hL, bool have) {
		if (!high_ready && __ballot(have && hL >= 18)) price_high_lengths();
		const uint32_t d = pos - hq - 1u;
		uint32_t slot = d, lb = 0;
		if (have) {
			if (d >= 4) { const uint32_t nlow = mgl_msb32(d) - 2; slot = nlow * 2 + (d >> nlow); }
			lb = hdr_match + minlen_m + lbslot[slot];
			if (lim32 != 0xFFFFFFFFu && lb >= lim32 * hL) have = false;
		}
		if (!__ballot(have)) return;
		uint32_t s0 = 0, s1 = 0, s2 = 0, s3 = 0, tail = 0;
		if (have) {
			if (d >= 4) {
				const uint32_t nlow = mgl_msb32(d) - 2;
				tail = d < 128 ? disttail[d] : ((nlow - 4) << 11) + aligncost[d & 15u];
			}
			s0 = slotcost[slot]; s1 = slotcost[64 + slot]; s2 = slotcost[128 + slot]; s3 = slotcost[192 + slot];
		}
		uint32_t len = hL;
		while (__ballot(have)) {
			const uint64_t thr = topk_threshold(t);
			const bool nolim = thr == MGL_INVALID_COST;
			const uint32_t lim = nolim ? 0u : (uint32_t)(thr >> 44) + 1u;
			uint64_t cand = MGL_INVALID_COST;
			while (have) {
				if (!nolim && lb >= lim * len) { have = false; break; }
				const uint32_t sc = len == 2 ? s0 : len == 3 ? s1 : len == 4 ? s2 : s3;
				const uint32_t perp = hdr_match + lencost[len - 2] + sc + tail;
				const uint32_t clen = len;
				len--;
				if (len < 2) have = false;
				if (!nolim && perp >= lim * clen) continue;
				if (inc_type == MGL_MATCH && clen == inc_len && d == inc_dist) continue;
				const uint64_t key = topk_make_key(perp / clen, ((uint64_t)(hq + 1) << 12) | ((uint64_t)clen << 3));
				if (key < thr) { cand = key; break; }
			}
			topk_offer(t, cand, lane);
		}
		{ const uint64_t th = topk_threshold(t); lim32 = th == MGL_INVALID_COST ? 0xFFFFFFFFu : (uint32_t)(th >> 44) + 1u; }
	};

	for (uint32_t ph = 0; ph < 2; ph++) {
		if (c.diag_stop >= 36 && c.diag_stop <= 38 && ph > c.diag_stop - 36u) break;
		const uint32_t* spos = ph == 0 ? c.hex_pos : c.oct_pos;
		const uint64_t* snx = ph == 0 ? c.hex_nx8 : c.oct_nx8;
		const uint32_t top = ph == 0 ? r16 : r8;
		const uint32_t cnt = top - (ph == 0 ? l16 : l8);
		const uint32_t lcap = ph == 0 ? maxlen : 15u;
		uint32_t q = 0, q1 = 0;
		uint64_t y = 0, y1 = 0;
		if (lane < cnt) { q = spos[top - 1u - lane]; y = snx[top - 1u - lane]; }
		for (uint32_t hb = 0; hb < cnt; hb += 64) {
			bool have = hb + lane < cnt;
			if (hb + 64u + lane < cnt) { q1 = spos[top - 65u - hb - lane]; y1 = snx[top - 65u - hb - lane]; }
			const uint32_t cq = q;
			const uint64_t cy = y;
			q = q1; y = y1;
			{
				const uint32_t dn = pos - rdlane(cq, 0) - 1u;
				uint32_t sn = dn;
				if (dn >= 4) { const uint32_t nl = mgl_msb32(dn) - 2; sn = nl * 2 + (dn >> nl); }
				const uint32_t ml = ph == 0 ? minlen_m : min15;
				if (lim32 != 0xFFFFFFFFu && hdr_match + ml + sufmin[sn] >= lim32 * lcap) break;
			}
			uint32_t L = 0;
			if (have) {
				if (ph == 0) {
					const uint64_t df = x16 ^ cy;
					if (df) L = 16u + (((uint32_t)__ffsll((long long)df) - 1u) >> 3);
					else {
						L = 24;
						while (L < maxlen) {
							uint64_t x, yy;
							__builtin_memcpy(&x, c.data + pos + L, 8);
							__builtin_memcpy(&yy, c.data + cq + L, 8);
							const uint64_t df2 = x ^ yy;
							if (df2) { L += ((uint32_t)__ffsll((long long)df2) - 1u) >> 3; break; }
							L += 8;
						}
					}
				} else {
					const uint64_t df = x8 ^ cy;
					if (!df) have = false;
					else L = 8u + (((uint32_t)__ffsll((long long)df) - 1u) >> 3);
				}
				if (L > maxlen) L = maxlen;
			}
			price_hits(cq, L, have);
		}
	}
	if (c.diag_stop == 36 || c.diag_stop == 37) return;

	for (uint32_t D = 7; D >= 2; D--) {
		if (c.diag_stop == 38 && D < 4) break;
		const uint32_t li = D - 2u;
		const uint32_t* spos = c.xpos[li];
		const uint8_t* snxb = c.xnxb[li];
		uint32_t top, low;
		if (D == 2) { top = hi; low = lo; }
		else {
			top = c.xrank[li][pos];
			low = bucket_lower_bound(spos, c.xrun[li][top], top, wpos, lane);
		}
		const uint32_t cnt = top - low;
		if (cnt == 0) continue;
		const uint32_t xb = (uint32_t)(x0 >> (8u * D)) & 0xFFu;
		const uint32_t hitlen = D < maxlen ? D : maxlen;
		uint32_t minup;
		{
			uint32_t v = lane < D - 1u ? lencost[lane] : 0xFFFFFFFFu;
			for (int o = 4; o > 0; o >>= 1) { const uint32_t a2 = (uint32_t)__shfl_xor((int)v, o, 64); v = a2 < v ? a2 : v; }
			minup = uni(v);
		}
		uint32_t dthr = 0xFFFFFFFFu, lim_seen = 0xFFFFFFFFu;
		auto refresh_threshold = [&]() {
			lim_seen = lim32;
			dthr = 0xFFFFFFFFu;
			if (lim32 == 0xFFFFFFFFu) return;
			const uint32_t fixed = hdr_match + minup, need = lim32 * D;
			const unsigned long long m = __ballot(need <= fixed || sufmin[lane] >= need - fixed);
			if (m) {
				const uint32_t sl = (uint32_t)__ffsll((long long)m) - 1u;
				dthr = sl < 4u ? sl : ((2u | (sl & 1u)) << ((sl >> 1) - 1u));
			}
		};
		auto loadw = [&](uint32_t hb, uint32_t qv[W], uint32_t& yv) {
			const uint32_t e0 = hb + (uint32_t)W * lane;
			if (W == 4 && e0 + 3u < cnt) {
				const uint32_t base = top - 4u - e0;
				uint4 qq;
				__builtin_memcpy(&qq, spos + base, 16);
				qv[0] = qq.w; qv[1 % W] = qq.z; qv[2 % W] = qq.y; qv[3 % W] = qq.x;
				uint32_t yy;
				__builtin_memcpy(&yy, snxb + base, 4);
				yv = __builtin_bswap32(yy);
			} else {
				yv = 0;
#pragma unroll
				for (uint32_t r = 0; r < (uint32_t)W; r++) {
					const bool in = e0 + r < cnt;
					const uint32_t idx = in ? top - 1u - (e0 + r) : top - 1u;
					qv[r] = in ? spos[idx] : pos;
					yv |= (uint32_t)snxb[idx] << (8u * r);
				}
			}
		};
		refresh_threshold();
		uint32_t qa[W], qb[W], ya, yb = 0;
#pragma unroll
		for (uint32_t r = 0; r < (uint32_t)W; r++) qb[r] = 0;
		loadw(0, qa, ya);
		for (uint32_t hb = 0; hb < cnt; hb += 64u * W) {
			if (hb + 64u * W < cnt) loadw(hb + 64u * W, qb, yb);
			if (lim_seen != lim32) refresh_threshold();
			if (pos - rdlane(qa[0], 0) - 1u >= dthr) break;
			uint32_t prmask = 0;
#pragma unroll
			for (uint32_t r = 0; r < (uint32_t)W; r++) {
				const uint32_t d = pos - qa[r] - 1u;
				const bool p = ((ya >> (8u * r)) & 0xFFu) != xb && d < dthr && d != 0xFFFFFFFFu;
				prmask |= (p ? 1u : 0u) << r;
			}
			if (c.diag_stop == 39) prmask = 0;
			for (uint32_t r = 0; r < (uint32_t)W && __ballot(prmask != 0); r++) {
				const bool p = (prmask >> r) & 1u;
				if (!__ballot(p)) continue;
				uint32_t q_r = qa[0];
#pragma unroll
				for (uint32_t k = 1; k < (uint32_t)W; k++) q_r = r == k ? qa[k] : q_r;
				price_hits(q_r, hitlen, p);
				prmask &= ~(1u << r);
			}
#pragma unroll
			for (uint32_t r = 0; r < (uint32_t)W; r++) qa[r] = qb[r];
			ya = yb;
		}
	}
}

__device__ __forceinline__ mgl_pk topk_packet(uint64_t key, uint32_t pos)
{
	uint64_t seq = MGL_SEQ_MASK - (key & MGL_SEQ_MASK);
	if (seq == 0) return MGL_PK_LITERAL;
	if (seq == 1) return MGL_PK_SHORT_REP;
	uint32_t q1 = (uint32_t)(seq >> 12), len = (uint32_t)(seq >> 3) & 0x1FFu, kind = (uint32_t)seq & 7u;
	if (kind == 0) return mgl_pack(MGL_MATCH, pos - q1, len);
	return mgl_pack(MGL_LONG_REP, kind - 1, len);
}


__device__ __forceinline__ void ckpt_store(const BaseView& b, const DevCtx& c, uint32_t ci, const uint16_t* probs,
                                           const Walk& w, uint64_t cum, uint32_t lane)
{
	uint32_t* dst = (uint32_t*)(b.ckpt_probs + (size_t)ci * b.ckpt_elems);
	const uint32_t* src = (const uint32_t*)probs;
	for (uint32_t i = lane; i < b.ckpt_elems / 2; i += 64) dst[i] = src[i];
	if (lane == 0) {
		CkptHdr h;
		h.pos = w.st.pos; h.ctx_state = w.st.ctx_state;
		h.dists[0] = w.st.dists[0]; h.dists[1] = w.st.dists[1]; h.dists[2] = w.st.dists[2]; h.dists[3] = w.st.dists[3];
		h.ordinal = w.packets; h.pad = 0; h.cum = cum;
		b.ckpt_hdr[ci] = h;
	}
}
__device__ __forceinline__ uint64_t ckpt_load(const BaseView& b, const DevCtx& c, uint32_t ci, uint16_t* probs,
                                              Walk& w, uint32_t lane)
{
	const uint32_t* src = (const uint32_t*)(b.ckpt_probs + (size_t)ci * b.ckpt_elems);
	uint32_t* dst = (uint32_t*)probs;
	for (uint32_t i = lane; i < b.ckpt_elems / 2; i += 64) dst[i] = src[i];
	const CkptHdr* h = &b.ckpt_hdr[ci];
	walk_reset(w);
	w.st.pos = uni(h->pos); w.st.ctx_state = uni(h->ctx_state);
	w.st.dists[0] = uni(h->dists[0]); w.st.dists[1] = uni(h->dists[1]);
	w.st.dists[2] = uni(h->dists[2]); w.st.dists[3] = uni(h->dists[3]);
	w.packets = uni(h->ordinal);
	uint64_t cum = uni64(h->cum);
	wave_sync();
	return cum;
}

__global__ void __launch_bounds__(64) k_rebuild(DevCtx c, BaseView b, Control* ctl, int from_dirty, uint64_t* cum_out,
                                                uint16_t* final_probs)
{
	extern __shared__ __attribute__((aligned(16))) unsigned char smem[];
	uint16_t* T = (uint16_t*)smem;
	uint16_t* probs = (uint16_t*)(smem + 4096);
	const uint32_t lane = threadIdx.x;
	for (uint32_t i = lane; i < 2048; i += 64) T[i] = c.cost_tbl[i];

	Walk w;
	uint64_t base_cum = 0;
	uint32_t ci = 0;
	if (from_dirty) {
		if (!ctl->accepted_flag) return;
		ci = uni(ctl->dirty_pos) >> MGL_CKPT_SHIFT;
	}
	if (ci == 0) {
		for (uint32_t i = lane; i < b.ckpt_elems; i += 64) probs[i] = MGL_PROB_INIT;
		walk_reset(w);
		wave_sync();
	} else {
		base_cum = ckpt_load(b, c, ci, probs, w, lane);
	}
	uint32_t next_ck = ci;
	uint32_t word = w.st.pos >> 6;
	uint64_t bits = 0;
	if (w.st.pos & 63u) bits = b.onwalk[word] & ((1ull << (w.st.pos & 63u)) - 1ull);

	uint32_t guard = 0;
	while (w.st.pos < c.n) {
		const uint32_t pos = w.st.pos;
		if (++guard > c.n) { if (lane == 0) atomicOr(&ctl->error_flags, MGL_ERR_WALK_OVERRUN); break; }
		while (next_ck < b.nckpt && (next_ck << MGL_CKPT_SHIFT) <= pos) {
			uint64_t cum = base_cum + wave_sum64(w.acc);
			ckpt_store(b, c, next_ck, probs, w, cum, lane);
			next_ck++;
		}
		const uint32_t pw = pos >> 6;
		if (pw != word) {
			if (lane == 0) b.onwalk[word] = bits;
			for (uint32_t z = word + 1 + lane; z < pw; z += 64) b.onwalk[z] = 0;
			word = pw; bits = 0;
		}
		bits |= 1ull << (pos & 63u);
		walk_window(w, c, b.slab, lane);
		const mgl_pk pk = walk_slab_at(w, pos);
		uint32_t type = mgl_pk_type(pk), len = mgl_pk_len(pk), dist = mgl_pk_dist(pk);
		if (type < MGL_LITERAL || type > MGL_LONG_REP || len == 0 || pos + len > c.n) {
			type = MGL_LITERAL; len = 1; dist = 0;
			if (lane == 0) atomicOr(&ctl->error_flags, MGL_ERR_WALK_OVERRUN);
		}
		walk_packet<true>(w, c, probs, T, type, dist, len, lane);
		if (cum_out) {
			uint64_t cum = base_cum + wave_sum64(w.acc);
			if (lane == 0) cum_out[w.packets - 1] = cum;
		}
	}
	if (lane == 0) b.onwalk[word] = bits;
	{
		const uint32_t nwords = (c.n + 63u) >> 6;
		for (uint32_t z = word + 1 + lane; z < nwords; z += 64) b.onwalk[z] = 0;
	}
	const uint64_t total = base_cum + wave_sum64(w.acc);
	wave_sync();
	if (final_probs) for (uint32_t i = lane; i < c.L.total; i += 64) final_probs[i] = probs[i];
	if (lane == 0) {
		ctl->packets = w.packets;
		ctl->rebuild_cost = total;
		ctl->final_ctx_state = w.st.ctx_state;
		ctl->final_dists[0] = w.st.dists[0]; ctl->final_dists[1] = w.st.dists[1];
		ctl->final_dists[2] = w.st.dists[2]; ctl->final_dists[3] = w.st.dists[3];
		if (from_dirty) {
			if (ctl->cur_cost != total) atomicOr(&ctl->error_flags, MGL_ERR_REBUILD_MISMATCH);
			ctl->accepted_flag = 0;
		}
	}
}


struct Journal {
	uint32_t* pos;
	mgl_pk* old;
	mgl_pk* neu;
	uint32_t count;
	bool overflow;
};
__device__ __forceinline__ void journal_set(Journal& jn, uint32_t pos, mgl_pk old, mgl_pk neu, uint32_t lane)
{
	for (uint32_t i = 0; i < jn.count && i < 2; i++) {
		if (jn.pos[i] == pos) { if (lane == 0) jn.neu[i] = neu; wave_sync(); return; }
	}
	if (jn.count >= MGL_MAX_DIFFS) { jn.overflow = true; return; }
	if (lane == 0) { jn.pos[jn.count] = pos; jn.old[jn.count] = old; jn.neu[jn.count] = neu; }
	jn.count++;
	wave_sync();
}

struct NbrRng { uint64_t key; uint32_t n; };
__device__ __forceinline__ uint32_t nbr_draw(NbrRng& r) { return mgl_rng_draw(r.key, r.n++); }

template <int W>
__device__ bool pick_from_top_k(const DevCtx& c, const Walk& w, const uint16_t* probs, const uint16_t* T, uint32_t* lencost,
                                mgl_pk incumbent, bool best, NbrRng& rng, uint32_t lane, mgl_pk* picked)
{
	TopK t;
	topk_find<W>(t, c, w, probs, T, lencost, incumbent, lane);
	const uint32_t count = t.count;
	if (count == 0) return false;
	uint32_t choice = nbr_draw(rng) % count;
	for (int i = 0; i < 7; i++) { uint32_t x = nbr_draw(rng) % count; choice = x > choice ? x : choice; }
	if (nbr_draw(rng) % 8u == 0 || best) choice = count - 1;
	uint64_t key = shfl64(t.key, (int)(count - 1 - choice));
	*picked = topk_packet(key, w.st.pos);
	return true;
}

__device__ __forceinline__ bool long_rep_ok(const DevCtx& c, const Walk& w, uint32_t idx, uint32_t len, uint32_t lane)
{
	const uint32_t rd = mgl_dist_at(&w.st, idx);
	if (rd >= w.st.pos || w.st.pos + len > c.n) return false;
	const uint32_t src = w.st.pos - rd - 1u;
	bool bad = false;
	for (uint32_t i = lane; i < len; i += 64) bad |= c.data[src + i] != c.data[w.st.pos + i];
	return __ballot(bad) == 0;
}

__device__ __forceinline__ mgl_pk journal_or_base(const Journal& jn, const mgl_pk* slab, uint32_t p, uint32_t lane)
{
	const bool hit = lane < jn.count && jn.pos[lane] == p;
	const unsigned long long m = __ballot(hit);
	if (m) return jn.neu[(uint32_t)__ffsll((long long)m) - 1u];
	return slab[p];
}
__device__ __forceinline__ uint32_t lit_steps_(uint32_t s, uint32_t n)
{
	if (n > 3) n = 3;
	for (uint32_t i = 0; i < n; i++) s = mgl_next_ctx_state(s, MGL_LITERAL);
	return s;
}
struct WinInfo { uint32_t end, soft, n_ins, n_rem, walked; };
__device__ __forceinline__ uint32_t packet_events(const DevCtx& c, const mgl_wstate& st, mgl_pk pk)
{
	mgl_plan pl;
	mgl_plan_packet(&c.L, &st, mgl_pk_type(pk), mgl_pk_dist(pk), mgl_pk_len(pk), 0u, 0u, 0u, &pl);
	return pl.nev;
}
__device__ WinInfo window_end_from_journal(const DevCtx& c, const mgl_pk* slab, const Journal& jn, mgl_wstate st, uint32_t lane)
{
	mgl_wstate nb = st, bs = st;
	uint32_t count = 0, wsoft = 0xFFFFFFFFu, taint = 0xFu, dep = 0u, wend = c.n, n_ins = 0, n_rem = 0, walked = 0;
	bool first = true;
	for (;;) {
		if (!first && nb.pos == bs.pos && count >= 3 && nb.ctx_state == bs.ctx_state) {
			if (wsoft == 0xFFFFFFFFu) wsoft = nb.pos;
			if (nb.dists[0] == bs.dists[0] && nb.dists[1] == bs.dists[1] && nb.dists[2] == bs.dists[2] && nb.dists[3] == bs.dists[3]) { wend = nb.pos; break; }
			if (nb.ctx_state < 7u && nb.pos < c.n) {
				uint32_t sx = nb.pos;
				while (sx < c.n && mgl_pk_type(uni64(slab[sx])) == MGL_LITERAL) sx++;
				if (sx > nb.pos) {
					const uint32_t cs = lit_steps_(nb.ctx_state, sx - nb.pos);
					nb.pos = bs.pos = sx; nb.ctx_state = bs.ctx_state = cs;
					count = 8;
					continue;
				}
			}
		}
		if (nb.pos >= c.n && bs.pos >= c.n) { wend = c.n; break; }
		if (walked > MGL_MAX_WALK) break;
		if (nb.pos <= bs.pos && nb.pos < c.n) {
			if (!first && count < 8) count++;
			first = false;
			walked++;
			const uint32_t p = nb.pos;
			const mgl_pk pk = uni64(journal_or_base(jn, slab, p, lane));
			const uint32_t ntype = mgl_pk_type(pk), ndist = mgl_pk_dist(pk);
			if (count > 0 && pk != uni64(slab[p])) wsoft = 0xFFFFFFFFu;
			if (ntype == MGL_SHORT_REP || ntype == MGL_LONG_REP) {
				const uint32_t slot = ntype == MGL_SHORT_REP ? 0u : ndist;
				const bool same_read = bs.pos == p && uni64(slab[p]) == pk && mgl_dist_at(&nb, slot) == mgl_dist_at(&bs, slot);
				if (!same_read) wsoft = 0xFFFFFFFFu;
				dep |= ntype == MGL_SHORT_REP ? (taint & 1u) : ((taint >> ndist) & 1u);
			}
			if (ntype == MGL_MATCH) taint = (taint << 1) & 0xFu;
			else if (ntype == MGL_LONG_REP) taint = (taint & ~((2u << ndist) - 1u)) | ((taint & ((1u << ndist) - 1u)) << 1) | ((taint >> ndist) & 1u);
			const bool paired = bs.pos == p;
			mgl_pk bpk = pk;
			bool cancelled = false;
			if (paired) {
				bpk = uni64(slab[p]);
				cancelled = bpk == pk && nb.ctx_state == bs.ctx_state;
				if (cancelled && ntype == MGL_LITERAL && nb.ctx_state >= 7) {
					const uint32_t mn = nb.dists[0] < p ? c.data[p - nb.dists[0] - 1] : 0u;
					const uint32_t mb = bs.dists[0] < p ? c.data[p - bs.dists[0] - 1] : 0u;
					cancelled = mn == mb;
				}
			}
			if (!cancelled) {
				n_ins += packet_events(c, nb, pk);
				if (paired) n_rem += packet_events(c, bs, bpk);
			}
			if (paired) mgl_advance(&bs, mgl_pk_type(bpk), mgl_pk_dist(bpk), mgl_pk_len(bpk));
			mgl_advance(&nb, ntype, ndist, mgl_pk_len(pk));
		} else {
			const mgl_pk pk = uni64(slab[bs.pos]);
			n_rem += packet_events(c, bs, pk);
			mgl_advance(&bs, mgl_pk_type(pk), mgl_pk_dist(pk), mgl_pk_len(pk));
		}
	}
	WinInfo wi;
	wi.n_ins = n_ins; wi.n_rem = n_rem; wi.walked = walked;
	wi.end = wend;
	wi.soft = (wsoft < wend ? wsoft : wend) | (dep << 31);
	return wi;
}

__device__ void nbr_fullwalk_one(const DevCtx& c, const BaseView& b, const Control* ctl, uint64_t seed, uint64_t step_override, uint32_t K,
                                 const NbrOut& out, uint32_t per_wave_bytes, bool from_zero, unsigned char* smem, const uint16_t* T, uint32_t j,
                                 uint32_t lane, uint32_t wid)
{
	if (j >= K) return;
	unsigned char* mine = smem + 4096 + (size_t)wid * per_wave_bytes;
	uint16_t* probs = (uint16_t*)mine;
	uint32_t* lencost = (uint32_t*)(mine + (size_t)b.ckpt_elems * 2);
	Journal jn;
	jn.old = (mgl_pk*)(lencost + MGL_PRICE_WORDS);
	jn.neu = jn.old + MGL_MAX_DIFFS;
	jn.pos = (uint32_t*)(jn.neu + MGL_MAX_DIFFS);
	jn.count = 0; jn.overflow = false;

	const uint64_t gstep = step_override != ~0ull ? step_override : ctl->gstep;
	NbrRng rng; rng.key = mgl_rng_key(seed, gstep, j); rng.n = 0;

	uint32_t target;
	if (c.strat_pre != nullptr) {
		target = uni(c.strat_tgt[j]);
		rng.n = 1;
	} else {
		uint32_t mydraw = lane < 32 ? mgl_rng_draw(rng.key, lane) % c.n : 0;
		bool on = lane < 32 && ((b.onwalk[mydraw >> 6] >> (mydraw & 63u)) & 1ull);
		unsigned long long m = __ballot(on);
		if (m) {
			int f = __ffsll((long long)m) - 1;
			target = rdlane(mydraw, (uint32_t)f);
			rng.n = (uint32_t)f + 1;
		} else {
			rng.n = 32;
			uint32_t p = rdlane(mydraw, 31);
			const uint32_t nwords = (c.n + 63u) >> 6;
			uint32_t wd = p >> 6;
			uint64_t bits = b.onwalk[wd] & (~0ull << (p & 63u));
			while (!bits && ++wd < nwords) bits = b.onwalk[wd];
			target = bits ? (wd << 6) + (uint32_t)__ffsll((long long)bits) - 1u : 0u;
			target = uni(target);
		}
	}

	Walk w;
	uint64_t base_cum = 0;
	if (from_zero) {
		for (uint32_t i = lane; i < b.ckpt_elems; i += 64) probs[i] = MGL_PROB_INIT;
		walk_reset(w);
		wave_sync();
	} else {
		base_cum = ckpt_load(b, c, target >> MGL_CKPT_SHIFT, probs, w, lane);
	}
	const uint32_t first_packet = w.packets;
	while (w.st.pos < target) {
// ... 206 lines not shown
```

megalania_amd/csrc/mgl_kernels2.hip:

```cpp
#include "mgl_base2.h"


struct BitAcc {
	uint32_t word;
	uint64_t bits;
};
__device__ __forceinline__ void bitacc_move(BitAcc& a, uint64_t* arr, uint32_t new_word, uint32_t lane)
{
	if (new_word == a.word) return;
	if (lane == 0) arr[a.word] = a.bits;
	for (uint32_t z = a.word + 1 + lane; z < new_word; z += 64) arr[z] = 0;
	a.word = new_word; a.bits = 0;
}

__device__ void build_body(const DevCtx& c, const Base2& b, Control* ctl, int check_cost)
{
	extern __shared__ __attribute__((aligned(16))) unsigned char smem[];
	uint16_t* T = (uint16_t*)smem;
	uint16_t* probs = (uint16_t*)(smem + 4096);
	uint32_t* cnt = (uint32_t*)(smem + 4096 + (size_t)b.ck_elems * 2);
	uint32_t* off = cnt + b.ck_elems;
	const uint32_t lane = threadIdx.x;
	const uint32_t total = c.L.total;
	if (check_cost && !ctl->accepted_flag) return;
// ... 342 lines not shown
					if (nxt >= limit) { ended = true; break; }
					chain_block(b, cx, nxt, &blo, &bhi);
					k = chain_lower_bound(cpos, bhi, nxt, traffic ? &probes : nullptr, blo > k ? blo : k);
					if (traffic) *traffic += 8u;
					chunk(k);
					p = ev_at(k) & 0x7FFu;
					continue;
				}
			}
			delta -= T[bb ? 2048u - bp : bp];
			if (rpos == bpos) {
				ri = next_with_ctx(ch.rem_key, ri + 1, ch.n_rem, cx, 0xFFFFu);
				rpos = ri < ch.n_rem ? ch.rem_pos[ri] : MGL_POS_INF;
			} else {
				delta += T[bb ? 2048u - p : p];
				p = mgl_prob_update(p, bb);
			}
			k++;
		}
		if (ch.diag == 43) { delta += p; continue; }
		if (!ended) {
			uint32_t kb = k & ~15u;
			uint4 a0 = *reinterpret_cast<const uint4*>(cev + kb);
			uint4 a1 = *reinterpret_cast<const uint4*>(cev + kb + 8);
			int32_t d32 = 0;
			while (!ended) {
				const uint4 n0 = *reinterpret_cast<const uint4*>(cev + kb + 16);
				const uint4 n1 = *reinterpret_cast<const uint4*>(cev + kb + 24);
				if (traffic) *traffic += 32u;
#pragma unroll
				for (uint32_t e = 0; e < 16; e++) {
					const uint32_t idx = kb + e;
					if (ended || idx < k) continue;
					if (idx >= clen) { ended = true; continue; }
					const uint4 q = e < 8 ? a0 : a1;
					const uint32_t h = e & 7u;
					const uint32_t wd = h < 2 ? q.x : h < 4 ? q.y : h < 6 ? q.z : q.w;
					const uint32_t ev = (wd >> ((h & 1u) * 16u)) & 0xFFFFu;
					const uint32_t bp = ev & 0x7FFu, bb = ev >> 15;
					if (p == bp) { ended = true; continue; }
					d32 += (int32_t)T[bb ? 2048u - p : p] - (int32_t)T[bb ? 2048u - bp : bp];
					p = mgl_prob_update(p, bb);
				}
				delta += d32; d32 = 0;
				a0 = n0; a1 = n1; kb += 16;
			}
			k = kb;
		}
		if (ch.dbg) atomicMax(&ch.dbg[21], (unsigned long long)iters);
		if (traffic) *traffic += 4u * probes;
		if (overlay && (at_limit || (limit != MGL_POS_INF && cpos[k] == MGL_POS_INF))) overlay[cx] = (uint16_t)p;
		(void)c_base;
	}
	return delta;
}
__device__ int64_t chain_sim(const Base2& b, Changes& ch, const uint16_t* T, uint32_t limit, uint16_t* overlay,
                             uint32_t lane, bool* too_many)
{
	const uint32_t nu = chain_list(ch, lane, too_many);
	if (*too_many) return 0;
	if (ch.diag == 41) return (int64_t)nu;
	const int64_t delta = chain_sim_contexts(b, ch, T, limit, overlay, lane, 0u, 64u, nu);
	uint64_t u = (uint64_t)delta;
	u = wave_sum64(u);
	wave_sync();
	return (int64_t)u;
}


struct Prof {
	unsigned long long* acc;
	unsigned long long t;
};
__device__ __forceinline__ void prof_start(Prof& p, unsigned long long* acc) { p.acc = acc; if (acc) p.t = __builtin_readcyclecounter(); }
__device__ __forceinline__ void prof_mark(Prof& p, int phase, uint32_t lane)
{
	if (!p.acc) return;
	const unsigned long long now = __builtin_readcyclecounter();
	if (lane == 0) { atomicAdd(&p.acc[phase], now - p.t); atomicAdd(&p.acc[8 + phase], 1ull); atomicMax(&p.acc[16 + phase], now - p.t); }
	p.t = __builtin_readcyclecounter();
}

struct Win {
	uint32_t base;
	mgl_pk pk;
	uint32_t byte;
};
__device__ __forceinline__ void win_cover(Win& w, const DevCtx& c, const mgl_pk* slab, uint32_t pos, uint32_t lane)
{
	const uint32_t base = pos & ~63u;
	if (base != w.base) {
		const uint32_t p = base + lane;
		w.pk = p < c.n ? slab[p] : 0;
		w.byte = c.data[p < c.n ? p : c.n];
		w.base = base;
	}
}
__device__ __forceinline__ mgl_pk win_pk(const Win& w, uint32_t pos) { return rdlane64(w.pk, pos - w.base); }
__device__ __forceinline__ uint32_t win_byte(const Win& w, uint32_t pos) { return rdlane(w.byte, pos - w.base); }

__device__ __forceinline__ void plan_at(const DevCtx& c, const mgl_wstate& st, uint32_t type, uint32_t dist, uint32_t len,
                                        uint32_t byte, mgl_plan& pl)
{
	uint32_t match_byte = 0, prev_byte = 0;
	if (type == MGL_LITERAL) {
		if (st.ctx_state >= 7 && st.dists[0] < st.pos) match_byte = c.data[st.pos - st.dists[0] - 1];
		if (c.L.lc > 0 && st.pos > 0) prev_byte = c.data[st.pos - 1];
	}
	mgl_plan_packet(&c.L, &st, type, dist, len, byte, match_byte, prev_byte, &pl);
}

template <bool INS>
__device__ __forceinline__ uint32_t literal_run_events(const DevCtx& c, Changes& ch, const Win& win, mgl_wstate& st, uint32_t limit, uint32_t lane)
{
	if (st.ctx_state >= 7u) return 0;
	const uint32_t o = st.pos - win.base;
	const unsigned long long lit = __ballot(mgl_pk_type(win.pk) == MGL_LITERAL) >> o;
	uint32_t run = (uint32_t)__ffsll((long long)~lit) - 1u;
	if (~lit == 0ull) run = 64u;
	run = run < 64u - o ? run : 64u - o;
	run = run < limit ? run : limit;
	if (run < 2u) return 0;
	const uint32_t take = run < 7u ? run : 7u;
	uint32_t& n = INS ? ch.n_ins : ch.n_rem;
	if (n + 9u * take > ch.cap) { ch.overflow = true; ch.list_full = true; return take; }
	const uint32_t i = lane / 9u, slot = lane - i * 9u;
	const uint32_t p = st.pos + i;
	const bool active = i < take;
	const uint32_t byte = (uint32_t)__shfl((int)win.byte, (int)((p - win.base) & 63u), 64);
	uint32_t prev_byte = 0;
	if (c.L.lc > 0) {
		const uint32_t wprev = (uint32_t)__shfl((int)win.byte, (int)((p - 1u - win.base) & 63u), 64);
		prev_byte = p == 0 ? 0u : (p - 1u >= win.base ? wprev : (uint32_t)c.data[p - 1u]);
	}
	mgl_wstate sv = st;
	sv.pos = p;
	sv.ctx_state = lit_steps(st.ctx_state, i);
	mgl_plan pl;
	mgl_plan_packet(&c.L, &sv, MGL_LITERAL, 0, 1, byte, 0, prev_byte, &pl);
	if (__ballot(active && pl.nev != 9u)) return 0;
	if (active) {
		uint32_t ctx, bit;
		mgl_plan_event(&pl, slot, &ctx, &bit);
		const uint32_t at = n + i * 9u + slot;
		if (INS) { ch.ins_key[at] = (uint16_t)(ctx | (bit << 15)); ch.ins_pos[at] = p; }
		else { ch.rem_key[at] = (uint16_t)ctx; ch.rem_pos[at] = p; }
	}
	n += 9u * take;
	st.pos += take;
	st.ctx_state = lit_steps(st.ctx_state, take);
	return take;
}

__device__ void model_load(const DevCtx& c, const Base2& b, uint16_t* probs, const uint16_t* T, uint32_t y, uint32_t lane)
{
	const uint32_t ck = y >> MGL_CK2_SHIFT;
	const uint4* src = (const uint4*)(b.ck_probs + (size_t)ck * b.ck_elems);
	uint4* dst = (uint4*)probs;
	const uint32_t n16 = b.ck_elems / 8u;
	for (uint32_t base = 0; base < n16; base += 256u) {
		uint4 r[4];
#pragma unroll
		for (uint32_t u = 0; u < 4; u++) { const uint32_t i = base + u * 64u + lane; if (i < n16) r[u] = src[i]; }
#pragma unroll
		for (uint32_t u = 0; u < 4; u++) { const uint32_t i = base + u * 64u + lane; if (i < n16) dst[i] = r[u]; }
	}
	const uint32_t first = ck << MGL_CK2_SHIFT;
	const uint64_t bits = b.onwalk[first >> 6] & ((y & 63u) ? ((1ull << (y & 63u)) - 1ull) : 0ull) & (~0ull << (first & 63u));
	wave_sync();
	if (bits) {
		const uint32_t start = uni(((first >> 6) << 6) + ctz64(bits));
		Walk w;
		walk_reset(w);
		w.st = uni_state(base_state_at(b, start));
		while (w.st.pos < y) {
			walk_window(w, c, b.slab, lane);
			if (w.st.ctx_state < 7u) {
				const uint32_t o = w.st.pos - w.wbase;
				const unsigned long long lit = __ballot(mgl_pk_type(w.wpk) == MGL_LITERAL) >> o;
				uint32_t run = ~lit == 0ull ? 64u : (uint32_t)__ffsll((long long)~lit) - 1u;
				run = run < 64u - o ? run : 64u - o;
				run = run < y - w.st.pos ? run : y - w.st.pos;
				if (run >= 2u) {
					const uint32_t take = run < 7u ? run : 7u;
					const uint32_t i = lane / 9u, slot = lane - i * 9u, p = w.st.pos + i;
					const bool active = i < take;
					const uint32_t byte = (uint32_t)__shfl((int)w.wbyte, (int)((p - w.wbase) & 63u), 64);
					uint32_t prev_byte = 0;
					if (c.L.lc > 0) {
						const uint32_t wprev = (uint32_t)__shfl((int)w.wbyte, (int)((p - 1u - w.wbase) & 63u), 64);
						prev_byte = p == 0 ? 0u : (p - 1u >= w.wbase ? wprev : (uint32_t)c.data[p - 1u]);
					}
					mgl_wstate sv = w.st;
					sv.pos = p; sv.ctx_state = lit_steps(w.st.ctx_state, i);
					mgl_plan pl;
					mgl_plan_packet(&c.L, &sv, MGL_LITERAL, 0, 1, byte, 0, prev_byte, &pl);
					if (!__ballot(active && pl.nev != 9u)) {
						uint32_t ctx = 0, bit = 0;
						if (active) mgl_plan_event(&pl, slot, &ctx, &bit);
						for (uint32_t r = 0; r < take; r++) {
							if (active && i == r) probs[ctx] = (uint16_t)mgl_prob_update(probs[ctx], bit);
							wave_sync();
						}
						w.st.pos += take; w.st.ctx_state = lit_steps(w.st.ctx_state, take);
						w.packets += take;
						continue;
					}
				}
			}
			const mgl_pk pk = walk_slab_at(w, w.st.pos);
			walk_packet<true>(w, c, probs, T, mgl_pk_type(pk), mgl_pk_dist(pk), mgl_pk_len(pk), lane);
		}
		wave_sync();
	}
}

__device__ __forceinline__ void walk_from_state(Walk& w, const mgl_wstate& st)
{
	walk_reset(w);
	w.st = st;
}

struct BigScratch {
	uint16_t* ins_key; uint32_t* ins_pos; uint16_t* rem_key; uint32_t* rem_pos; uint16_t* uctx;
	uint32_t cap, uctx_cap, slots;
	const uint32_t* todo_in; const uint32_t* todo_in_count;
	uint32_t* spill_ctr;
	uint32_t chg_cap;
	uint4* sim_hdr;
	uint4* sim_hdr2;
	uint32_t* sim_slot2;
	uint32_t lds_cache;
	uint16_t* sim_keys;
	uint32_t* sim_pos;
	const uint32_t* la_list; const uint32_t* la_count;
	const uint8_t* la_mark; const uint32_t* la_spec_count;
	const uint32_t* todo_first;
	uint32_t* cont;
};
#define MGL_CONT_WORDS 368u
#define MGL_CONT_MAGIC 0x434F4E54u
#ifndef MGL_PICK_T_GLOBAL
#define MGL_PICK_T_GLOBAL 1
#endif
#ifndef MGL_REST_WAVES_PER_SIMD
#define MGL_REST_WAVES_PER_SIMD 4
#endif
#define MGL_SIM2_CAP 4096u
#define MGL_NBR_FULL 0
#define MGL_NBR_PICK 1
#define MGL_NBR_REST 2
template <bool BIG, int MODE, bool LIST>
__device__ __forceinline__ void nbr2_one(const DevCtx& c, const Base2& b, Control* ctl, uint64_t seed,
                                         uint64_t step_override, uint32_t K, const NbrOut& out, uint32_t per_wave_bytes,
                                         uint32_t* todo, uint32_t* todo_count, unsigned long long* prof_acc,
                                         const BigScratch& big, uint4* pickrec, uint32_t j_base, uint32_t j_end, uint4* pickstate,
                                         unsigned char* smem, const uint16_t* T, uint32_t unit, uint32_t lane, uint32_t wid)
{
	uint32_t j = j_base + unit;
	uint32_t slot = 0;
	const unsigned long long t_begin = prof_acc ? __builtin_readcyclecounter() : 0ull;
	if (!BIG && LIST) j = uni(big.la_list[unit]);
	if (BIG) {
		slot = unit + ((LIST && big.todo_first != nullptr) ? *big.todo_first : 0u);
		const uint32_t nflag = *big.todo_in_count;
		if (slot >= nflag) return;
		j = uni(big.todo_in[slot]);
		if (LIST && big.la_mark != nullptr && slot < *big.la_spec_count && j < K && big.la_mark[j]) return;
		if (lane == 0) atomicAdd((unsigned long long*)&ctl->big_nbrs, 1ull);
	}
	if (j >= K || (!BIG && j >= j_end)) return;
	unsigned char* mine = smem + ((MODE == MGL_NBR_REST || (MODE == MGL_NBR_PICK && MGL_PICK_T_GLOBAL)) ? 0u : 4096u) + (size_t)wid * per_wave_bytes;
	Journal jn;
	jn.old = (mgl_pk*)mine;
	jn.neu = jn.old + MGL_MAX_DIFFS;
	jn.pos = (uint32_t*)(jn.neu + MGL_MAX_DIFFS);
	jn.count = 0; jn.overflow = false;
	Changes ch;
	ch.nbitwords = (c.L.total + 31u) >> 5;
	ch.ctxbits = jn.pos + MGL_MAX_DIFFS;
	unsigned char* uni_base = MODE == MGL_NBR_PICK ? mine : (unsigned char*)(ch.ctxbits + ((ch.nbitwords + 3u) & ~3u));
	uint16_t* probs = (uint16_t*)uni_base;
	uint32_t* lencost = (uint32_t*)(uni_base + (size_t)b.ck_elems * 2);
	ch.ins_pos = (uint32_t*)uni_base;
	ch.rem_pos = ch.ins_pos + big.chg_cap;
	ch.ins_key = (uint16_t*)(ch.rem_pos + big.chg_cap);
	ch.rem_key = ch.ins_key + big.chg_cap;
	ch.uctx = ch.rem_key + big.chg_cap;
	ch.cap = big.chg_cap; ch.uctx_cap = 2 * big.chg_cap;
	if (BIG) {
		if (slot >= big.slots) {
			if (lane == 0) { const uint32_t s2 = atomicAdd(todo_count, 1u); todo[s2] = j; }
			return;
		}
		ch.ins_key = big.ins_key + (size_t)slot * big.cap; ch.ins_pos = big.ins_pos + (size_t)slot * big.cap;
		ch.rem_key = big.rem_key + (size_t)slot * big.cap; ch.rem_pos = big.rem_pos + (size_t)slot * big.cap;
		ch.uctx = big.uctx + (size_t)slot * big.uctx_cap;
		ch.cap = big.cap; ch.uctx_cap = big.uctx_cap;
	}
	ch.n_ins = ch.n_rem = 0; ch.direct = 0; ch.overflow = false; ch.list_full = false;
	bool too_many = false;
	bool spilled = BIG;
	const bool spilled_lds = false;

	const uint64_t gstep = step_override != ~0ull ? step_override : ctl->gstep;
	NbrRng rng; rng.key = mgl_rng_key(seed, gstep, j); rng.n = 0;
	uint32_t* const crec = (BIG && big.cont != nullptr) ? big.cont + (size_t)slot * MGL_CONT_WORDS : nullptr;
	bool resumed = false;
	if (BIG && crec != nullptr) resumed = uni(crec[0]) == MGL_CONT_MAGIC && uni(crec[1]) == j;

	uint32_t target;
	mgl_wstate nb;
	if (MODE == MGL_NBR_REST && lane == 0) big.sim_hdr[j] = make_uint4(0xFFFFFFFFu, 0u, 0u, 0u);
	if (BIG && big.sim_hdr2 != nullptr && lane == 0) big.sim_hdr2[j] = make_uint4(0xFFFFFFFFu, 0u, 0u, 0u);
	if (MODE == MGL_NBR_REST) {
		const uint4 s0 = pickstate[2u * j], s1 = pickstate[2u * j + 1u];
		target = s0.x; rng.n = s0.y;
		nb.pos = target; nb.ctx_state = s0.z;
		nb.dists[0] = s0.w; nb.dists[1] = s1.x; nb.dists[2] = s1.y; nb.dists[3] = s1.z;
	} else if (BIG && resumed) {
		target = uni(crec[2]);
		nb.pos = uni(crec[3]); nb.ctx_state = uni(crec[4]);
		nb.dists[0] = uni(crec[5]); nb.dists[1] = uni(crec[6]); nb.dists[2] = uni(crec[7]); nb.dists[3] = uni(crec[8]);
	} else if (c.strat_pre != nullptr) {
		target = uni(c.strat_tgt[j]);
		rng.n = 1;
		nb = uni_state(base_state_at(b, target));
		if (MODE == MGL_NBR_PICK && lane == 0) {
			pickstate[2u * j] = make_uint4(target, rng.n, nb.ctx_state, nb.dists[0]);
			pickstate[2u * j + 1u] = make_uint4(nb.dists[1], nb.dists[2], nb.dists[3], 0u);
		}
	} else {
		uint32_t mydraw = lane < 32 ? mgl_rng_draw(rng.key, lane) % c.n : 0;
		bool on = lane < 32 && ((b.onwalk[mydraw >> 6] >> (mydraw & 63u)) & 1ull);
		unsigned long long m = __ballot(on);
		if (m) {
			int f = __ffsll((long long)m) - 1;
			target = rdlane(mydraw, (uint32_t)f);
			rng.n = (uint32_t)f + 1;
		} else {
			rng.n = 32;
			uint32_t p = rdlane(mydraw, 31);
			uint32_t wd = p >> 6;
			uint64_t bits = b.onwalk[wd] & (~0ull << (p & 63u));
			while (!bits && ++wd < b.nw0) bits = b.onwalk[wd];
			target = uni(bits ? (wd << 6) + ctz64(bits) : 0u);
		}
		nb = uni_state(base_state_at(b, target));
		if (MODE == MGL_NBR_PICK && lane == 0) {
			pickstate[2u * j] = make_uint4(target, rng.n, nb.ctx_state, nb.dists[0]);
			pickstate[2u * j + 1u] = make_uint4(nb.dists[1], nb.dists[2], nb.dists[3], 0u);
		}
	}
	Prof prof;
	prof_start(prof, prof_acc);
	ch.dbg = prof_acc;
	ch.diag = c.diag_stop;
	const uint32_t pos = target;
	mgl_wstate bs = nb;
	Win win; win.base = 0xFFFFFFFFu; win.pk = 0; win.byte = 0;
	Walk tw;

	win_cover(win, c, b.slab, pos, lane);
	const mgl_pk first = win_pk(win, pos);
	mgl_pk m_first = first, m_second = 0;
	bool second_set = false, mutated = false;
	prof_mark(prof, 0, lane);
	if (c.diag_stop == 1) { if (lane == 0) { out.cost[j] = MGL_INVALID_COST; out.ndiffs[j] = 0; out.walked[j] = first; } return; }
	if (!(BIG && resumed) && pos + 1 < c.n && (nbr_draw(rng) % 2u) == 0) {
		const mgl_pk second = uni64(b.slab[pos + 1]);
		const uint32_t ft = mgl_pk_type(first), flen = mgl_pk_len(first);
		const uint32_t st = mgl_pk_type(second), slen = mgl_pk_len(second), sdist = mgl_pk_dist(second);
		if ((ft == MGL_LONG_REP || ft == MGL_MATCH) && flen > 2) {
			m_second = mgl_pack(ft, mgl_pk_dist(first), flen - 1);
			m_first = MGL_PK_LITERAL;
			if (MODE != MGL_NBR_PICK) { journal_set(jn, pos, first, m_first, lane); journal_set(jn, pos + 1, second, m_second, lane); }
			second_set = true; mutated = true;
		} else if ((ft == MGL_LITERAL || ft == MGL_SHORT_REP) && (st == MGL_MATCH || st == MGL_LONG_REP)) {
			uint32_t rep_start = pos - (st == MGL_LONG_REP ? mgl_dist_at(&nb, sdist) : sdist);
			if (slen < MGL_MAX_MATCH && rep_start > 0 && rep_start <= pos && win_byte(win, pos) == c.data[rep_start - 1]) {
				m_first = mgl_pack(st, sdist, slen + 1);
				if (MODE != MGL_NBR_PICK) journal_set(jn, pos, first, m_first, lane);
				mutated = true;
			}
		}
	}
	enum { P_MODEL, P_SIM, P_TOPK, P_WALK, P_OUT };
	uint32_t phase = mutated ? P_WALK : P_MODEL;
	if (MODE == MGL_NBR_PICK && mutated) return;
	if (MODE == MGL_NBR_REST && c.diag_stop != 0 && c.diag_stop != 4 && c.diag_stop < 40) return;
	bool pick_is_mutation = !mutated;
	uint32_t pick_pos = pos;
	mgl_pk pick_inc = first;
	bool pick_best = false;
	bool have_pick = false;
	mgl_pk picked_pk = 0, resume_old = 0;
	uint32_t sim_limit = MGL_POS_INF;
	bool sim_overlay = false;
	int64_t delta = 0;
	bool generate_failed = false, sim_deferred = false, walk_long = false;
	uint32_t npicks = 0;
	uint32_t count = 0;
	uint32_t walked = 0;
	uint32_t wend = 0;
	uint32_t wsoft = 0xFFFFFFFFu, taint = 0xFu, dep = 0u;
	bool first_packet = true;
	uint32_t guard = 0;
	if (BIG && resumed) {
		bs.pos = uni(crec[9]); bs.ctx_state = uni(crec[10]);
		bs.dists[0] = uni(crec[11]); bs.dists[1] = uni(crec[12]); bs.dists[2] = uni(crec[13]); bs.dists[3] = uni(crec[14]);
		count = uni(crec[15]); walked = uni(crec[16]); npicks = uni(crec[17]); wsoft = uni(crec[18]); taint = uni(crec[19]); dep = uni(crec[20]);
		rng.n = uni(crec[21]); guard = uni(crec[22]); jn.count = uni(crec[23]); ch.n_ins = uni(crec[24]); ch.n_rem = uni(crec[25]);
		const uint32_t fl = uni(crec[26]);
		pick_best = (fl & 1u) != 0; second_set = (fl & 2u) != 0;
		pick_inc = (mgl_pk)uni(crec[28]) | ((mgl_pk)uni(crec[29]) << 32);
		resume_old = (mgl_pk)uni(crec[30]) | ((mgl_pk)uni(crec[31]) << 32);
		m_second = (mgl_pk)uni(crec[32]) | ((mgl_pk)uni(crec[33]) << 32);
		ch.direct = (int64_t)((uint64_t)uni(crec[34]) | ((uint64_t)uni(crec[35]) << 32));
		if (lane < jn.count) {
			jn.pos[lane] = crec[48u + lane];
			jn.old[lane] = reinterpret_cast<const mgl_pk*>(crec + 112u)[lane];
			jn.neu[lane] = reinterpret_cast<const mgl_pk*>(crec + 240u)[lane];
		}
		wave_sync();
		if (lane == 0) crec[0] = 0u;
		pick_pos = nb.pos;
		mutated = true; pick_is_mutation = false; first_packet = false;
		phase = P_MODEL;
	}
	if ((MODE == MGL_NBR_REST || (BIG && pickrec != nullptr)) && !mutated) {
		const uint4 rec = pickrec[j];
		if (!(rec.w & 1u)) { generate_failed = true; phase = P_OUT; }
		else {
			m_first = (mgl_pk)rec.x | ((mgl_pk)rec.y << 32);
			journal_set(jn, pos, first, m_first, lane);
			rng.n = rec.z;
			pick_is_mutation = false;
			phase = P_WALK;
		}
	}

	for (;;) {
		if (MODE == MGL_NBR_REST && (phase == P_MODEL || phase == P_TOPK)) { ch.overflow = true; phase = P_OUT; continue; }
		if (MODE != MGL_NBR_REST && phase == P_MODEL) {
			if ((ch.n_ins + ch.n_rem) != 0 && !spilled) {
				if (!BIG && LIST) { ch.overflow = true; phase = P_OUT; continue; }
				uint32_t sl = 0;
				if (lane == 0) sl = atomicAdd(big.spill_ctr, 1u);
				sl = uni(sl);
				if (sl >= big.slots) { ch.overflow = true; phase = P_OUT; continue; }
				uint16_t* gik = big.ins_key + (size_t)sl * big.cap; uint32_t* gip = big.ins_pos + (size_t)sl * big.cap;
				uint16_t* grk = big.rem_key + (size_t)sl * big.cap; uint32_t* grp = big.rem_pos + (size_t)sl * big.cap;
				for (uint32_t i = lane; i < ch.n_ins; i += 64) { gik[i] = ch.ins_key[i]; gip[i] = ch.ins_pos[i]; }
				for (uint32_t i = lane; i < ch.n_rem; i += 64) { grk[i] = ch.rem_key[i]; grp[i] = ch.rem_pos[i]; }
				__threadfence_block();
				wave_sync();
				ch.ins_key = gik; ch.ins_pos = gip; ch.rem_key = grk; ch.rem_pos = grp;
				ch.uctx = big.uctx + (size_t)sl * big.uctx_cap;
				ch.cap = big.cap; ch.uctx_cap = big.uctx_cap;
				spilled = true;
			}
			model_load(c, b, probs, T, pick_pos, lane);
			if (!pick_is_mutation) prof_mark(prof, 5, lane);
			if (pick_is_mutation) {
				prof_mark(prof, 1, lane);
				if (c.diag_stop == 2) { if (lane == 0) { out.cost[j] = MGL_INVALID_COST; out.ndiffs[j] = 0; out.walked[j] = probs[lane]; } return; }
			}
			if ((ch.n_ins + ch.n_rem) != 0) { sim_limit = pick_pos; sim_overlay = true; phase = P_SIM; }
			else phase = P_TOPK;
		}
		if (BIG && big.sim_hdr2 != nullptr && !sim_overlay && !spilled_lds && ch.n_ins <= MGL_SIM2_CAP && ch.n_rem <= MGL_SIM2_CAP && phase == P_SIM) {
			if (lane == 0) {
				big.sim_slot2[j] = slot;
				big.sim_hdr2[j] = make_uint4(ch.n_ins, ch.n_rem, (uint32_t)(uint64_t)ch.direct, (uint32_t)((uint64_t)ch.direct >> 32));
			}
			sim_deferred = true;
			phase = P_OUT;
			continue;
		}
		if (MODE == MGL_NBR_REST && phase == P_SIM) {
			uint16_t* gk = big.sim_keys + (size_t)j * (2u * big.chg_cap);
			uint32_t* gp = big.sim_pos + (size_t)j * (2u * big.chg_cap);
			for (uint32_t e = lane; e < ch.n_ins; e += 64) { gk[e] = ch.ins_key[e]; gp[e] = ch.ins_pos[e]; }
			for (uint32_t e = lane; e < ch.n_rem; e += 64) { gk[big.chg_cap + e] = ch.rem_key[e]; gp[big.chg_cap + e] = ch.rem_pos[e]; }
			if (lane == 0) big.sim_hdr[j] = make_uint4(ch.n_ins, ch.n_rem, (uint32_t)(uint64_t)ch.direct, (uint32_t)((uint64_t)ch.direct >> 32));
			sim_deferred = true;
			phase = P_OUT;
			continue;
		}
		if (MODE == MGL_NBR_FULL && phase == P_SIM) {
			int64_t r;
			if (BIG && big.lds_cache && ch.n_ins <= MGL_BIG_CAP && ch.n_rem <= MGL_BIG_CAP) {
				uint32_t* cp = (uint32_t*)(mine + per_wave_bytes);
				Changes cl = ch;
				cl.ins_pos = cp; cl.rem_pos = cp + MGL_BIG_CAP;
				cl.ins_key = (uint16_t*)(cp + 2u * MGL_BIG_CAP); cl.rem_key = cl.ins_key + MGL_BIG_CAP;
				for (uint32_t e = lane; e < ch.n_ins; e += 64) { cl.ins_pos[e] = ch.ins_pos[e]; cl.ins_key[e] = ch.ins_key[e]; }
				for (uint32_t e = lane; e < ch.n_rem; e += 64) { cl.rem_pos[e] = ch.rem_pos[e]; cl.rem_key[e] = ch.rem_key[e]; }
				wave_sync();
				r = chain_sim(b, cl, T, sim_limit, sim_overlay ? probs : nullptr, lane, &too_many);
			} else {
				r = chain_sim(b, ch, T, sim_limit, (MODE != MGL_NBR_REST && sim_overlay) ? probs : nullptr, lane, &too_many);
			}
			wave_sync();
			if (too_many) { phase = P_OUT; continue; }
			if (sim_overlay) { prof_mark(prof, 6, lane); phase = P_TOPK; }
			else { delta = r; prof_mark(prof, 4, lane); phase = P_OUT; }
		}
		if (MODE != MGL_NBR_REST && phase == P_TOPK) {
			walk_from_state(tw, nb);
			walk_window(tw, c, b.slab, lane);
			mgl_pk picked;
			const bool ok = pick_from_top_k<(MODE == MGL_NBR_PICK ? 4 : 1)>(c, tw, probs, T, lencost, pick_inc, pick_best, rng, lane, &picked);
			if (MODE == MGL_NBR_PICK) {
				if (lane == 0) pickrec[j] = make_uint4((uint32_t)picked, (uint32_t)(picked >> 32), rng.n, ok ? 1u : 0u);
				return;
			}
			if (pick_is_mutation) {
				if (!BIG && LIST && pickrec != nullptr && lane == 0)
					pickrec[j] = make_uint4((uint32_t)picked, (uint32_t)(picked >> 32), rng.n, ok ? 1u : 0u);
				if (!ok) { generate_failed = true; phase = P_OUT; continue; }
				m_first = picked;
				journal_set(jn, pos, first, m_first, lane);
				pick_is_mutation = false;
				prof_mark(prof, 2, lane);
				if (c.diag_stop == 3 || (c.diag_stop >= 31 && c.diag_stop <= 39)) { if (lane == 0) { out.cost[j] = MGL_INVALID_COST; out.ndiffs[j] = 0; out.walked[j] = (uint32_t)m_first; } return; }
			} else {
				picked_pk = ok ? picked : pick_inc;
				have_pick = true;
				prof_mark(prof, 7, lane);
			}
			win.base = 0xFFFFFFFFu;
			phase = P_WALK;
		}
		if (MODE != MGL_NBR_PICK && phase == P_WALK) {
			bool request_pick = false;
			while (nb.pos < c.n || bs.pos < c.n) {
				if (ch.overflow || jn.overflow || too_many || ++guard > (BIG ? (1u << 20) : 4096u)) { ch.overflow = true; break; }
				if (!first_packet && !have_pick && nb.pos == bs.pos && count >= 3) {
					const bool same_ctx = nb.ctx_state == bs.ctx_state;
					const bool same_d = nb.dists[0] == bs.dists[0] && nb.dists[1] == bs.dists[1] && nb.dists[2] == bs.dists[2] &&
					                    nb.dists[3] == bs.dists[3];
					if (same_ctx && wsoft == 0xFFFFFFFFu) wsoft = nb.pos;
					if (same_ctx && same_d) break;
					if (same_ctx && nb.ctx_state < 7) {
						uint32_t sx = uni(sp_find_next(b, nb.pos));
						if (sx == MGL_POS_INF || sx > c.n) sx = c.n;
						if (sx > nb.pos) {
							const uint32_t cs = lit_steps(nb.ctx_state, sx - nb.pos);
							nb.pos = bs.pos = sx; nb.ctx_state = bs.ctx_state = cs;
							count = 8;
							continue;
						}
					}
				}
				if (walked > MGL_MAX_WALK && !have_pick) { walk_long = true; break; }
				if ((have_pick || nb.pos <= bs.pos) && nb.pos < c.n) {
					const uint32_t p = nb.pos;
					win_cover(win, c, b.slab, p, lane);
					mgl_pk pk, old = 0;
					if (have_pick) {
						pk = picked_pk; old = resume_old; have_pick = false;
					} else if (first_packet) {
						pk = m_first;
					} else {
						if (count < 8) count++;
						old = (second_set && p == pos + 1) ? m_second : win_pk(win, p);
						pk = old;
						uint32_t type = mgl_pk_type(pk);
						if (type == MGL_SHORT_REP || (type == MGL_LITERAL && count < 4)) {
							const bool same = nb.dists[0] < p && win_byte(win, p) == c.data[p - nb.dists[0] - 1];
							if (same) { if (count < 4) pk = MGL_PK_SHORT_REP; }
							else pk = MGL_PK_LITERAL;
						}
						type = mgl_pk_type(pk);
						if (type == MGL_LONG_REP) {
							const uint32_t len = mgl_pk_len(pk);
							uint32_t idx = mgl_pk_dist(pk);
							walk_from_state(tw, nb);
							bool ok = long_rep_ok(c, tw, idx, len, lane);
							for (uint32_t i = 0; i < 4 && !ok; i++) { idx = i; ok = long_rep_ok(c, tw, idx, len, lane); }
							pk = mgl_pack(MGL_LONG_REP, idx, len);
							if (!ok) {
								if (++npicks > MGL_MAX_REPAIR_PICKS) { walk_long = true; break; }
								pick_best = (nbr_draw(rng) % 4u) == 0;
								while (bs.pos < p && !ch.overflow) {
									win_cover(win, c, b.slab, bs.pos, lane);
									const mgl_pk bpk = win_pk(win, bs.pos);
									mgl_plan bpl;
									plan_at(c, bs, mgl_pk_type(bpk), mgl_pk_dist(bpk), mgl_pk_len(bpk), win_byte(win, bs.pos), bpl);
									changes_add<false>(ch, bpl, bs.pos, lane);
									mgl_advance(&bs, mgl_pk_type(bpk), mgl_pk_dist(bpk), mgl_pk_len(bpk));
								}
								if (ch.overflow) break;
								if (MODE == MGL_NBR_REST && big.cont != nullptr) {
									uint32_t slot2 = 0;
									if (lane == 0) {
										atomicAdd(big.spill_ctr + 1, 1u);
										slot2 = atomicAdd(todo_count, 1u);
										todo[slot2] = j;
										out.cost[j] = MGL_INVALID_COST; out.ndiffs[j] = 0; out.walked[j] = 0; out.win[2u * j] = pos; out.win[2u * j + 1u] = MGL_WIN_NONE;
									}
									slot2 = uni(slot2);
									if (slot2 < big.slots) {
										uint16_t* gik = big.ins_key + (size_t)slot2 * big.cap; uint32_t* gip = big.ins_pos + (size_t)slot2 * big.cap;
										uint16_t* grk = big.rem_key + (size_t)slot2 * big.cap; uint32_t* grp = big.rem_pos + (size_t)slot2 * big.cap;
										for (uint32_t i = lane; i < ch.n_ins; i += 64) { gik[i] = ch.ins_key[i]; gip[i] = ch.ins_pos[i]; }
										for (uint32_t i = lane; i < ch.n_rem; i += 64) { grk[i] = ch.rem_key[i]; grp[i] = ch.rem_pos[i]; }
										uint32_t* rec = big.cont + (size_t)slot2 * MGL_CONT_WORDS;
										if (lane < jn.count) {
											rec[48u + lane] = jn.pos[lane];
											reinterpret_cast<mgl_pk*>(rec + 112u)[lane] = jn.old[lane];
											reinterpret_cast<mgl_pk*>(rec + 240u)[lane] = jn.neu[lane];
										}
										if (lane == 0) {
											rec[1] = j; rec[2] = pos;
											rec[3] = nb.pos; rec[4] = nb.ctx_state; rec[5] = nb.dists[0]; rec[6] = nb.dists[1]; rec[7] = nb.dists[2]; rec[8] = nb.dists[3];
											rec[9] = bs.pos; rec[10] = bs.ctx_state; rec[11] = bs.dists[0]; rec[12] = bs.dists[1]; rec[13] = bs.dists[2]; rec[14] = bs.dists[3];
											rec[15] = count; rec[16] = walked; rec[17] = npicks; rec[18] = wsoft; rec[19] = taint; rec[20] = dep;
											rec[21] = rng.n; rec[22] = guard; rec[23] = jn.count; rec[24] = ch.n_ins; rec[25] = ch.n_rem;
											rec[26] = (pick_best ? 1u : 0u) | (second_set ? 2u : 0u);
											rec[28] = (uint32_t)pk; rec[29] = (uint32_t)(pk >> 32);
											rec[30] = (uint32_t)old; rec[31] = (uint32_t)(old >> 32);
											rec[32] = (uint32_t)m_second; rec[33] = (uint32_t)(m_second >> 32);
											rec[34] = (uint32_t)(uint64_t)ch.direct; rec[35] = (uint32_t)((uint64_t)ch.direct >> 32);
											rec[0] = MGL_CONT_MAGIC;
										}
									}
									return;
								}
								resume_old = old; pick_pos = p; pick_inc = pk;
								request_pick = true;
								if (!BIG && lane == 0) atomicAdd(big.spill_ctr + 1, 1u);
								break;
							}
						}
					}
					if (!first_packet && pk != old) {
						const mgl_pk base_old = (second_set && p == pos + 1) ? uni64(b.slab[p]) : old;
						journal_set(jn, p, base_old, pk, lane);
						wsoft = 0xFFFFFFFFu;
					}
					first_packet = false;
					walked++;
					const uint32_t ntype = mgl_pk_type(pk), ndist = mgl_pk_dist(pk), nlen = mgl_pk_len(pk);
					if (ntype == MGL_SHORT_REP || ntype == MGL_LONG_REP) {
						const uint32_t slot = ntype == MGL_SHORT_REP ? 0u : ndist;
						const bool same_read = bs.pos == p && win_pk(win, p) == pk && mgl_dist_at(&nb, slot) == mgl_dist_at(&bs, slot);
						if (!same_read) wsoft = 0xFFFFFFFFu;
						dep |= ntype == MGL_SHORT_REP ? (taint & 1u) : ((taint >> ndist) & 1u);
					}
					if (ntype == MGL_MATCH) taint = (taint << 1) & 0xFu;
					else if (ntype == MGL_LONG_REP) taint = (taint & ~((2u << ndist) - 1u)) | ((taint & ((1u << ndist) - 1u)) << 1) | ((taint >> ndist) & 1u);
					bool cancelled = false;
					if (bs.pos == p && win_pk(win, p) == pk && nb.ctx_state == bs.ctx_state) {
						cancelled = true;
						if (ntype == MGL_LITERAL && nb.ctx_state >= 7) {
							const uint32_t mn = nb.dists[0] < p ? c.data[p - nb.dists[0] - 1] : 0u;
							const uint32_t mb = bs.dists[0] < p ? c.data[p - bs.dists[0] - 1] : 0u;
							cancelled = mn == mb;
						}
					}
					if (cancelled) {
						mgl_advance(&bs, ntype, ndist, nlen);
					} else {
						if (bs.pos == p) {
							const mgl_pk bpk = win_pk(win, p);
							const uint32_t btype = mgl_pk_type(bpk), bdist = mgl_pk_dist(bpk), blen = mgl_pk_len(bpk);
							mgl_plan bpl;
							plan_at(c, bs, btype, bdist, blen, win_byte(win, p), bpl);
							changes_add<false>(ch, bpl, p, lane);
							mgl_advance(&bs, btype, bdist, blen);
						}
						mgl_plan npl;
						plan_at(c, nb, ntype, ndist, nlen, win_byte(win, p), npl);
						changes_add<true>(ch, npl, p, lane);
					}
					mgl_advance(&nb, ntype, ndist, nlen);
				} else {
					win_cover(win, c, b.slab, bs.pos, lane);
					if (literal_run_events<false>(c, ch, win, bs, (nb.pos < c.n ? nb.pos : c.n) - bs.pos, lane)) continue;
					const mgl_pk bpk = win_pk(win, bs.pos);
					mgl_plan bpl;
					plan_at(c, bs, mgl_pk_type(bpk), mgl_pk_dist(bpk), mgl_pk_len(bpk), win_byte(win, bs.pos), bpl);
					changes_add<false>(ch, bpl, bs.pos, lane);
					mgl_advance(&bs, mgl_pk_type(bpk), mgl_pk_dist(bpk), mgl_pk_len(bpk));
				}
			}
			if (walk_long) { phase = P_OUT; continue; }
			if (request_pick) { prof_mark(prof, 3, lane); phase = P_MODEL; continue; }
			prof_mark(prof, 3, lane);
			if (c.diag_stop == 4) { if (lane == 0) { out.cost[j] = MGL_INVALID_COST; out.ndiffs[j] = 0; out.walked[j] = ch.n_ins + ch.n_rem; } return; }
			if (ch.overflow || jn.overflow || too_many) { phase = P_OUT; continue; }
			wend = nb.pos;
			sim_limit = MGL_POS_INF; sim_overlay = false; phase = P_SIM;
			continue;
		}
		if (phase == P_OUT) break;
	}

	if (generate_failed) {
		if (lane == 0) { out.cost[j] = MGL_INVALID_COST; out.ndiffs[j] = 0; out.walked[j] = 0; out.win[2u * j] = pos; out.win[2u * j + 1u] = MGL_WIN_NONE; }
		return;
	}
	if (jn.overflow) {
		if (lane == 0) { out.cost[j] = MGL_INVALID_COST; out.ndiffs[j] = 0; out.walked[j] = walked; out.win[2u * j] = pos; out.win[2u * j + 1u] = MGL_WIN_DROPPED; }
		return;
	}
	if (walk_long || (ch.list_full && ch.cap == big.cap && !jn.overflow)) {
		if (lane == 0) { out.cost[j] = MGL_INVALID_COST; out.ndiffs[j] = 0; out.walked[j] = walked; out.win[2u * j] = pos; out.win[2u * j + 1u] = MGL_WIN_DROPPED; }
		return;
	}
	if (ch.overflow || too_many) {
		if (lane == 0) {
			const uint32_t slot2 = atomicAdd(todo_count, 1u);
			todo[slot2] = j;
			if (BIG) atomicAdd((unsigned long long*)&ctl->fallback_nbrs, 1ull);
			out.cost[j] = MGL_INVALID_COST; out.ndiffs[j] = 0; out.walked[j] = 0; out.win[2u * j] = pos; out.win[2u * j + 1u] = MGL_WIN_NONE;
		}
		return;
	}
	const uint64_t total = (uint64_t)((int64_t)ctl->rebuild_cost + delta + ch.direct);
	uint32_t nd = 0;
	for (uint32_t i = 0; i < jn.count; i++) {
		if (jn.old[i] == jn.neu[i]) continue;
		if (lane == 0) {
			out.dpos[(size_t)j * MGL_MAX_DIFFS + nd] = jn.pos[i];
			out.dold[(size_t)j * MGL_MAX_DIFFS + nd] = jn.old[i];
			out.dnew[(size_t)j * MGL_MAX_DIFFS + nd] = jn.neu[i];
		}
		nd++;
	}
	if (lane == 0) { if (!sim_deferred) out.cost[j] = total; out.ndiffs[j] = nd; out.walked[j] = walked; out.win[2u * j] = pos; out.win[2u * j + 1u] = wend; out.win2[j] = (wsoft < wend ? wsoft : wend) | (dep << 31); }
	if (prof_acc && lane == 0)
		prof_acc[32 + j] = ((__builtin_readcyclecounter() - t_begin) & 0xFFFFFFFFFFull) |
		                   ((unsigned long long)((ch.n_ins + ch.n_rem) & 0xFFFu) << 40) | ((unsigned long long)(walked & 0xFFFu) << 52);
}

template <bool BIG, int MODE, bool LIST = false>
__global__ void __launch_bounds__((MODE == MGL_NBR_PICK ? 512 : 64), (MODE == MGL_NBR_FULL ? (BIG ? 1 : MGL_NBR_WAVES_PER_SIMD) : (MODE == MGL_NBR_REST ? MGL_REST_WAVES_PER_SIMD : 4))) k_neighbours2(DevCtx c, Base2 b, Control* ctl, uint64_t seed,
                                                     uint64_t step_override, uint32_t K, NbrOut out, uint32_t per_wave_bytes,
                                                     uint32_t* todo, uint32_t* todo_count, unsigned long long* prof_acc,
                                                     BigScratch big, uint4* pickrec, uint32_t j_base, uint32_t j_end, uint4* pickstate)
{
	const uint32_t waves = blockDim.x >> 6;
	if (BIG && blockIdx.x * waves + ((LIST && big.todo_first != nullptr) ? *big.todo_first : 0u) >= *big.todo_in_count) return;
	if (!BIG && LIST && blockIdx.x * waves >= *big.la_count) return;
	extern __shared__ __attribute__((aligned(16))) unsigned char smem[];
	uint16_t* T = (uint16_t*)smem;
	if (MODE == MGL_NBR_PICK && MGL_PICK_T_GLOBAL) {
		T = const_cast<uint16_t*>(c.cost_tbl);
	} else if (MODE != MGL_NBR_REST) {
		for (uint32_t i = threadIdx.x; i < 256; i += blockDim.x) reinterpret_cast<uint4*>(T)[i] = reinterpret_cast<const uint4*>(c.cost_tbl)[i];
		__syncthreads();
	}
	const uint32_t lane = threadIdx.x & 63u, wid = threadIdx.x >> 6;
	if (BIG) {
		const uint32_t first = (LIST && big.todo_first != nullptr) ? *big.todo_first : 0u;
		const uint32_t n = *big.todo_in_count > first ? *big.todo_in_count - first : 0u;
		for (uint32_t unit = blockIdx.x * waves + wid; unit < n; unit += gridDim.x * waves)
			nbr2_one<BIG, MODE, LIST>(c, b, ctl, seed, step_override, K, out, per_wave_bytes, todo, todo_count, prof_acc, big, pickrec, j_base, j_end, pickstate, smem, T, unit, lane, wid);
	} else if (LIST) {
		const uint32_t n = *big.la_count;
		for (uint32_t unit = blockIdx.x * waves + wid; unit < n; unit += gridDim.x * waves)
			nbr2_one<BIG, MODE, true>(c, b, ctl, seed, step_override, K, out, per_wave_bytes, todo, todo_count, prof_acc, big, pickrec, 0u, K, pickstate, smem, T, unit, lane, wid);
	} else {
		nbr2_one<BIG, MODE, false>(c, b, ctl, seed, step_override, K, out, per_wave_bytes, todo, todo_count, prof_acc, big, pickrec, j_base, j_end, pickstate, smem, T,
		                    blockIdx.x * waves + wid, lane, wid);
	}
}


#ifndef MGL_SIM_WAVES
#define MGL_SIM_WAVES 2u
#endif
#ifndef MGL_SIM_WAVES_LIST
#define MGL_SIM_WAVES_LIST 8u
#endif
#define MGL_SIM_WAVES_MAX 8u
struct SimShared {
	uint16_t* T;
	uint32_t* dyn;
	unsigned long long* sum;
	uint32_t* nu_many;
};
template <bool FROM_BIG, bool COUNT>
__device__ __forceinline__ void sim_one(const DevCtx& c, const Base2& b, Control* ctl, const NbrOut& out, const BigScratch& big, const uint4* hdrs,
                                        uint32_t j, uint32_t* todo, uint32_t* todo_count, const SimShared& sh, unsigned long long* traffic_ctr)
{
	const uint4 hdr = hdrs[j];
	if (hdr.x == 0xFFFFFFFFu) return;
	const uint32_t cap = FROM_BIG ? MGL_SIM2_CAP : big.chg_cap;
	const uint32_t slot = FROM_BIG ? big.sim_slot2[j] : 0u;
	uint32_t* s_bits = sh.dyn;
	uint32_t* s_pos = sh.dyn + ((((c.L.total + 31u) >> 5) + 3u) & ~3u);
	uint16_t* s_key = (uint16_t*)(s_pos + 2u * cap);
	uint16_t* s_uctx = s_key + 2u * cap;
	const uint32_t lane = threadIdx.x & 63u, wid = threadIdx.x >> 6;
	Changes ch;
	ch.n_ins = hdr.x; ch.n_rem = hdr.y;
	ch.ins_pos = s_pos; ch.rem_pos = s_pos + cap;
	ch.ins_key = s_key; ch.rem_key = s_key + cap;
	ch.uctx = s_uctx; ch.ctxbits = s_bits;
	ch.cap = cap; ch.uctx_cap = 2 * cap;
	ch.nbitwords = (c.L.total + 31u) >> 5;
	ch.direct = 0; ch.dbg = nullptr; ch.diag = c.diag_stop; ch.overflow = false; ch.list_full = false;
	__syncthreads();
	if (FROM_BIG) {
		const uint16_t* ik = big.ins_key + (size_t)slot * big.cap; const uint32_t* ip = big.ins_pos + (size_t)slot * big.cap;
		const uint16_t* rk = big.rem_key + (size_t)slot * big.cap; const uint32_t* rp = big.rem_pos + (size_t)slot * big.cap;
		for (uint32_t e = threadIdx.x; e < ch.n_ins; e += blockDim.x) { s_key[e] = ik[e]; s_pos[e] = ip[e]; }
		for (uint32_t e = threadIdx.x; e < ch.n_rem; e += blockDim.x) { s_key[cap + e] = rk[e]; s_pos[cap + e] = rp[e]; }
	} else {
		const uint16_t* gk = big.sim_keys + (size_t)j * (2u * cap);
		const uint32_t* gp = big.sim_pos + (size_t)j * (2u * cap);
		for (uint32_t e = threadIdx.x; e < ch.n_ins; e += blockDim.x) { s_key[e] = gk[e]; s_pos[e] = gp[e]; }
		for (uint32_t e = threadIdx.x; e < ch.n_rem; e += blockDim.x) { s_key[cap + e] = gk[cap + e]; s_pos[cap + e] = gp[cap + e]; }
	}
	__syncthreads();
	if (wid == 0) {
		bool too_many = false;
		const uint32_t nu = chain_list(ch, lane, &too_many);
		if (lane == 0) { sh.nu_many[0] = nu; sh.nu_many[1] = too_many ? 1u : 0u; }
	}
	__syncthreads();
	if (sh.nu_many[1]) {
		if (threadIdx.x == 0) {
			const uint32_t slot2 = atomicAdd(todo_count, 1u);
			todo[slot2] = j;
			out.cost[j] = MGL_INVALID_COST; out.ndiffs[j] = 0; out.walked[j] = 0; out.win[2u * j + 1u] = MGL_WIN_NONE;
		}
		return;
	}
	if (c.diag_stop == 41) { if (threadIdx.x == 0) out.cost[j] = sh.nu_many[0]; return; }
	uint32_t traffic = 0;
	const int64_t mine = chain_sim_contexts(b, ch, sh.T, MGL_POS_INF, nullptr, lane, wid * 64u, blockDim.x, sh.nu_many[0], COUNT ? &traffic : nullptr);
	const uint64_t u = wave_sum64((uint64_t)mine);
	if (lane == 0) sh.sum[wid] = u;
	if (COUNT) {
		const uint64_t tb = wave_sum64((uint64_t)traffic) + (wid == 0 ? 6ull * (ch.n_ins + ch.n_rem) + 16ull : 0ull);
		if (lane == 0) atomicAdd(traffic_ctr, (unsigned long long)tb);
	}
	__syncthreads();
	if (threadIdx.x == 0) {
		uint64_t d = 0;
		for (uint32_t w = 0; w < (blockDim.x >> 6); w++) d += sh.sum[w];
		const int64_t direct = (int64_t)((uint64_t)hdr.z | ((uint64_t)hdr.w << 32));
		out.cost[j] = (uint64_t)((int64_t)ctl->rebuild_cost + (int64_t)d + direct);
	}
}
template <bool COUNT>
__global__ void __launch_bounds__(64 * MGL_SIM_WAVES_MAX, 8) k_sim(DevCtx c, Base2 b, Control* ctl, NbrOut out, BigScratch big, uint32_t j_base, uint32_t j_end,
                                                           uint32_t* todo, uint32_t* todo_count, const uint32_t* list, const uint32_t* list_count,
                                                           unsigned long long* traffic_ctr)
{
	if (list ? blockIdx.x >= *list_count : j_base + blockIdx.x >= j_end) return;
	__shared__ __attribute__((aligned(16))) uint16_t T[2048];
	extern __shared__ __attribute__((aligned(16))) uint32_t s_dyn[];
	__shared__ unsigned long long s_sum[MGL_SIM_WAVES_MAX];
	__shared__ uint32_t s_nm[2];
	if (!list && big.sim_hdr[j_base + blockIdx.x].x == 0xFFFFFFFFu) return;
	for (uint32_t i = threadIdx.x; i < 256; i += blockDim.x) reinterpret_cast<uint4*>(T)[i] = reinterpret_cast<const uint4*>(c.cost_tbl)[i];
	SimShared sh;
	sh.T = T; sh.dyn = s_dyn; sh.sum = s_sum; sh.nu_many = s_nm;
	if (list) {
		const uint32_t n = *list_count;
		for (uint32_t i = blockIdx.x; i < n; i += gridDim.x) {
			if (big.la_mark != nullptr && i < *big.la_spec_count && big.la_mark[list[i]]) continue;
			sim_one<true, COUNT>(c, b, ctl, out, big, big.sim_hdr2, list[i], todo, todo_count, sh, traffic_ctr);
		}
	} else {
		sim_one<false, COUNT>(c, b, ctl, out, big, big.sim_hdr, j_base + blockIdx.x, todo, todo_count, sh, traffic_ctr);
	}
}


__global__ void __launch_bounds__(64) k_rank_blocks(const uint64_t* onwalk, uint32_t nw0, uint32_t* pre, uint32_t nblk)
{
	const uint32_t blk = blockIdx.x, lane = threadIdx.x;
	if (blk >= nblk) return;
	const uint32_t w = blk * 64u + lane;
	unsigned long long v = w < nw0 ? (unsigned long long)__popcll(onwalk[w]) : 0ull;
	v = wave_sum64(v);
	if (lane == 0) pre[blk + 1u] = (uint32_t)v;
}
__global__ void __launch_bounds__(1024) k_rank_scan(uint32_t* pre, uint32_t nblk)
{
	__shared__ uint32_t s_w[16], s_base;
	const uint32_t tid = threadIdx.x, lane = tid & 63u, wid = tid >> 6;
	if (tid == 0) { s_base = 0; pre[0] = 0; }
	__syncthreads();
	for (uint32_t base = 0; base < nblk; base += blockDim.x) {
		const uint32_t i = base + tid;
		const uint32_t v = i < nblk ? pre[i + 1u] : 0u;
		uint32_t incl = v;
		for (int o = 1; o < 64; o <<= 1) { const uint32_t t = (uint32_t)__shfl_up((int)incl, o, 64); if ((int)lane >= o) incl += t; }
		if (lane == 63) s_w[wid] = incl;
		__syncthreads();
		uint32_t bsum = s_base;
		for (uint32_t q = 0; q < wid; q++) bsum += s_w[q];
		if (i < nblk) pre[i + 1u] = bsum + incl;
		__syncthreads();
		if (tid == blockDim.x - 1u) s_base = bsum + incl;
		__syncthreads();
	}
}

__global__ void __launch_bounds__(256) k_targets(DevCtx c, const uint64_t* onwalk, uint32_t nw0, const Control* ctl, uint64_t seed, uint64_t step_override,
                                                 uint32_t K, uint32_t* tgt)
{
// ... 7 lines not shown
```

Before: 13.77 million.

## Let multiple waves cooperate on each big neighbour unit

The big-neighbour kernel now runs one work unit per block of several waves instead of one unit per wave. Wave 0 drives the unit, and helper waves join in through a shared LDS stage variable and block barriers. The helpers share the model copy, the chained context simulation and the top-k source scan, which is split by source with a shared atomic pruning threshold. The aim is to shorten the long serial tail of heavy units, at the cost of extra barriers, more LDS per block and idle helper waves during the serial phases.

```diff
diff --git a/megalania_amd/csrc/mgl_api.hip b/megalania_amd/csrc/mgl_api.hip
--- a/megalania_amd/csrc/mgl_api.hip
+++ b/megalania_amd/csrc/mgl_api.hip
@@ -101,6 +101,7 @@
 	unsigned long long* d_prof;
 	uint32_t* d_todo;
 	uint32_t per_wave2, waves_per_block2, nbr2_lds, build_lds;
+	uint32_t big_waves = MGL_BIG_WAVES;
 	uint32_t chg_cap = MGL_CHG_CAP;
 	uint32_t per_wave_pick, per_wave_rest, pick_waves;
 	size_t b2_bytes;
@@ -485,6 +486,7 @@
 	BigScratch big_now = sa->big;
 	big_now.lds_cache = 1u;
 	const uint32_t big_lds = sa->nbr2_lds + 12u * MGL_BIG_CAP;
+	const uint32_t coop_lds = big_lds + coop_lds_bytes(sa->big_waves);
 	if (!split_now || g_big_inline_sim) big_now.sim_hdr2 = nullptr;
 	const bool la_step = from_lookahead && split_now;
 	if (la_step) {
@@ -498,7 +500,7 @@
 		                   sa->b2, sa->base.ctl, sa->cfg.seed, step_override, K, sa->nbr, sa->per_wave2, sa->d_todo2, sa->d_counts + 1,
 		                   (unsigned long long*)nullptr, big_now, sa->d_pickrec, 0u, K, sa->d_pickstate); NBR_TRACE("k_neighbours2<true, MGL_NBR_FULL, true>");
 	} else {
-		hipLaunchKernelGGL((k_neighbours2<true, MGL_NBR_FULL>), dim3(bigblocks), dim3(64 * sa->waves_per_block2), big_lds, sa->stream, sa->ctx,
+		hipLaunchKernelGGL((k_neighbours2<true, MGL_NBR_FULL>), dim3(bigblocks), dim3(64 * sa->big_waves), coop_lds, sa->stream, sa->ctx,
 		                   sa->b2, sa->base.ctl, sa->cfg.seed, step_override, K, sa->nbr, sa->per_wave2, sa->d_todo2, sa->d_counts + 1,
 		                   g_prof_big ? sa->d_prof : (unsigned long long*)nullptr, big_now, (sa->split_nbr && !sa->form_single) ? sa->d_pickrec : (uint4*)nullptr, 0u, K, sa->d_pickstate); NBR_TRACE("k_neighbours2<true, MGL_NBR_FULL>");
 	}
@@ -526,7 +528,7 @@
 		BigScratch late = sa->big;
 		late.todo_in = sa->d_todo3; late.todo_in_count = sa->d_counts + 4; late.sim_hdr2 = nullptr; late.lds_cache = 1u;
 		late.cont = nullptr;
-		hipLaunchKernelGGL((k_neighbours2<true, MGL_NBR_FULL>), dim3(bigblocks < 64u ? bigblocks : 64u), dim3(64 * sa->waves_per_block2), big_lds, sa->stream, sa->ctx,
+		hipLaunchKernelGGL((k_neighbours2<true, MGL_NBR_FULL>), dim3(bigblocks < 64u ? bigblocks : 64u), dim3(64 * sa->big_waves), coop_lds, sa->stream, sa->ctx,
 		                   sa->b2, sa->base.ctl, sa->cfg.seed, step_override, K, sa->nbr, sa->per_wave2, sa->d_todo2, sa->d_counts + 1,
 		                   (unsigned long long*)nullptr, late, sa->d_pickrec, 0u, K, sa->d_pickstate); NBR_TRACE("k_neighbours2<true, MGL_NBR_FULL>");
 	}
@@ -1010,11 +1012,13 @@
 		HIPCHK(hipFuncSetAttribute((const void*)k_neighbours2<false, MGL_NBR_FULL, true>, hipFuncAttributeMaxDynamicSharedMemorySize, (int)sa->nbr2_lds));
 		HIPCHK(hipFuncSetAttribute((const void*)k_neighbours2<false, MGL_NBR_PICK>, hipFuncAttributeMaxDynamicSharedMemorySize, 160 * 1024));
 		HIPCHK(hipFuncSetAttribute((const void*)k_neighbours2<false, MGL_NBR_REST>, hipFuncAttributeMaxDynamicSharedMemorySize, (int)sa->nbr2_lds));
-		HIPCHK(hipFuncSetAttribute((const void*)k_neighbours2<true, MGL_NBR_FULL>, hipFuncAttributeMaxDynamicSharedMemorySize, (int)(sa->nbr2_lds + 12u * MGL_BIG_CAP)));
+		HIPCHK(hipFuncSetAttribute((const void*)k_neighbours2<true, MGL_NBR_FULL>, hipFuncAttributeMaxDynamicSharedMemorySize,
+		                           (int)(sa->nbr2_lds + 12u * MGL_BIG_CAP + coop_lds_bytes(MGL_BIG_WAVES))));
 		HIPCHK(hipFuncSetAttribute((const void*)k_neighbours2<true, MGL_NBR_FULL, true>, hipFuncAttributeMaxDynamicSharedMemorySize, (int)(sa->nbr2_lds + 12u * MGL_BIG_CAP)));
 		HIPCHK(hipMalloc(&sa->d_pickrec, sizeof(uint4) * K));
 		HIPCHK(hipMalloc(&sa->d_pickstate, sizeof(uint4) * 2 * K));
 		sa->split_nbr = getenv("MGL_NO_SPLIT") == nullptr;
+		sa->big_waves = getenv("MGL_BIG_ONE_WAVE") != nullptr ? 1u : MGL_BIG_WAVES;
 		if (sa->split_nbr) {
 			BigScratch& g = sa->big;
 			HIPCHK(hipMalloc(&g.sim_hdr, sizeof(uint4) * (size_t)K));
diff --git a/megalania_amd/csrc/mgl_kernels.hip b/megalania_amd/csrc/mgl_kernels.hip
--- a/megalania_amd/csrc/mgl_kernels.hip
+++ b/megalania_amd/csrc/mgl_kernels.hip
@@ -134,10 +134,33 @@
 	return lo;
 }
 
-template <int W>
+#define MGL_SRC_HEAD 1u
+#define MGL_SRC_OCT 2u
+__device__ __forceinline__ uint32_t MGL_SRC_EXACT(uint32_t D) { return 1u << (9u - D); }
+__device__ __forceinline__ uint32_t topk_sources_of(uint32_t wid, uint32_t nw)
+{
+	if (nw <= 1u) return ~0u;
+	if (nw == 2u) return wid == 0 ? MGL_SRC_HEAD | MGL_SRC_EXACT(7) | MGL_SRC_EXACT(6) | MGL_SRC_EXACT(5)
+	                              : MGL_SRC_OCT | MGL_SRC_EXACT(4) | MGL_SRC_EXACT(3) | MGL_SRC_EXACT(2);
+	uint32_t m = wid == 0 ? MGL_SRC_HEAD : wid == 1 ? MGL_SRC_OCT : 0u;
+	for (uint32_t i = 0; i < 6; i++)
+		if (wid >= 2u && (i % (nw - 2u)) == wid - 2u) m |= MGL_SRC_EXACT(7u - i);
+	return m;
+}
+template <int W, bool SPLIT = false>
 __device__ void topk_find(TopK& t, const DevCtx& c, const Walk& w, const uint16_t* probs, const uint16_t* T,
-                          uint32_t* lencost, mgl_pk incumbent, uint32_t lane)
-{
+                          uint32_t* lencost, mgl_pk incumbent, uint32_t lane, uint32_t srcmask = ~0u, unsigned long long* sthr = nullptr)
+{
+	auto owns = [&](uint32_t src) { return !SPLIT || (srcmask & src) != 0u; };
+	auto prune_thr = [&]() -> uint64_t {
+		uint64_t th = topk_threshold(t);
+		if (SPLIT) { const uint64_t s = uni64(*(volatile unsigned long long*)sthr); th = s < th ? s : th; }
+		return th;
+	};
+	auto offer = [&](uint64_t cand) {
+		topk_offer(t, cand, lane);
+		if (SPLIT && t.count == t.k) { const uint64_t own = topk_threshold(t); if (lane == 0) atomicMin(sthr, (unsigned long long)own); }
+	};
 	const uint32_t pos = w.st.pos;
 	const uint32_t state = w.st.ctx_state;
 	const uint32_t pos_state = pos & ((1u << c.L.pb) - 1u);
@@ -204,7 +227,7 @@
 		minlen_m = uni(a); minlen_r = uni(b);
 	}
 
-	{
+	if (owns(MGL_SRC_HEAD)) {
 		uint64_t cand = MGL_INVALID_COST;
 		uint32_t byte = walk_byte_at(w, pos);
 		uint32_t rep_byte = (pos > 0 && w.st.dists[0] < pos) ? c.data[pos - w.st.dists[0] - 1] : 0x100u;
@@ -221,7 +244,7 @@
 		if (lane == 0 && incumbent != MGL_PK_LITERAL) cand = topk_make_key(lit, 0);
 		if (lane == 1 && pos > 0 && byte == rep_byte && incumbent != MGL_PK_SHORT_REP)
 			cand = topk_make_key(hdr_rep + g0_0 + l_0, 1);
-		topk_offer(t, cand, lane);
+		offer(cand);
 	}
 
 	if (c.diag_stop == 32) return;
@@ -256,7 +279,7 @@
 	};
 
 	if (c.diag_stop == 34) return;
-	{
+	if (owns(MGL_SRC_HEAD)) {
 		const uint32_t b0 = bigram >> 8, b1 = bigram & 0xFFu;
 #pragma unroll
 		for (uint32_t k = 0; k < 4; k++) {
@@ -274,7 +297,7 @@
 			if (L >= 18 && !high_ready) price_high_lengths();
 			const uint32_t hdr = k == 0 ? hdr_lr0 : k == 1 ? hdr_lr1 : k == 2 ? hdr_lr2 : hdr_lr3;
 			for (uint32_t top = L; top >= 2;) {
-				const uint64_t thr = topk_threshold(t);
+				const uint64_t thr = prune_thr();
 				const bool nolim = thr == MGL_INVALID_COST;
 				const uint32_t lim = nolim ? 0u : (uint32_t)(thr >> 44) + 1u;
 				if (!nolim && hdr + minlen_r >= lim * top) break;
@@ -287,7 +310,7 @@
 						if (key < thr) cand = key;
 					}
 				}
-				topk_offer(t, cand, lane);
+				offer(cand);
 				top = top > 64u + 1u ? top - 64u : 0u;
 			}
 		}
@@ -298,8 +321,8 @@
 	__builtin_memcpy(&x8, c.data + pos + 8, 8);
 	__builtin_memcpy(&x16, c.data + pos + 16, 8);
 	const uint32_t r8 = c.oct_rank[pos], r16 = c.hex_rank[pos];
-	const uint32_t l8 = bucket_lower_bound(c.oct_pos, c.oct_run[r8], r8, wpos, lane);
-	const uint32_t l16 = bucket_lower_bound(c.hex_pos, c.hex_run[r16], r16, wpos, lane);
+	const uint32_t l8 = owns(MGL_SRC_OCT) ? bucket_lower_bound(c.oct_pos, c.oct_run[r8], r8, wpos, lane) : r8;
+	const uint32_t l16 = owns(MGL_SRC_HEAD) ? bucket_lower_bound(c.hex_pos, c.hex_run[r16], r16, wpos, lane) : r16;
 	if (c.diag_stop == 35) return;
 	uint32_t min15;
 	{
@@ -308,7 +331,8 @@
 		min15 = uni(m15);
 	}
 	uint32_t lim32;
-	{ const uint64_t th = topk_threshold(t); lim32 = th == MGL_INVALID_COST ? 0xFFFFFFFFu : (uint32_t)(th >> 44) + 1u; }
+	auto refresh_lim32 = [&]() { const uint64_t th = prune_thr(); lim32 = th == MGL_INVALID_COST ? 0xFFFFFFFFu : (uint32_t)(th >> 44) + 1u; };
+	refresh_lim32();
 	auto price_hits = [&](uint32_t hq, uint32_t hL, bool have) {
 		if (!high_ready && __ballot(have && hL >= 18)) price_high_lengths();
 		const uint32_t d = pos - hq - 1u;
@@ -329,7 +353,7 @@
 		}
 		uint32_t len = hL;
 		while (__ballot(have)) {
-			const uint64_t thr = topk_threshold(t);
+			const uint64_t thr = prune_thr();
 			const bool nolim = thr == MGL_INVALID_COST;
 			const uint32_t lim = nolim ? 0u : (uint32_t)(thr >> 44) + 1u;
 			uint64_t cand = MGL_INVALID_COST;
@@ -345,13 +369,14 @@
 				const uint64_t key = topk_make_key(perp / clen, ((uint64_t)(hq + 1) << 12) | ((uint64_t)clen << 3));
 				if (key < thr) { cand = key; break; }
 			}
-			topk_offer(t, cand, lane);
-		}
-		{ const uint64_t th = topk_threshold(t); lim32 = th == MGL_INVALID_COST ? 0xFFFFFFFFu : (uint32_t)(th >> 44) + 1u; }
+			offer(cand);
+		}
+		refresh_lim32();
 	};
 
 	for (uint32_t ph = 0; ph < 2; ph++) {
 		if (c.diag_stop >= 36 && c.diag_stop <= 38 && ph > c.diag_stop - 36u) break;
+		if (!owns(ph == 0 ? MGL_SRC_HEAD : MGL_SRC_OCT)) continue;
 		const uint32_t* spos = ph == 0 ? c.hex_pos : c.oct_pos;
 		const uint64_t* snx = ph == 0 ? c.hex_nx8 : c.oct_nx8;
 		const uint32_t top = ph == 0 ? r16 : r8;
@@ -366,6 +391,7 @@
 			const uint32_t cq = q;
 			const uint64_t cy = y;
 			q = q1; y = y1;
+			if (SPLIT) refresh_lim32();
 			{
 				const uint32_t dn = pos - rdlane(cq, 0) - 1u;
 				uint32_t sn = dn;
@@ -403,6 +429,7 @@
 
 	for (uint32_t D = 7; D >= 2; D--) {
 		if (c.diag_stop == 38 && D < 4) break;
+		if (!owns(MGL_SRC_EXACT(D))) continue;
 		const uint32_t li = D - 2u;
 		const uint32_t* spos = c.xpos[li];
 		const uint8_t* snxb = c.xnxb[li];
@@ -462,6 +489,7 @@
 		loadw(0, qa, ya);
 		for (uint32_t hb = 0; hb < cnt; hb += 64u * W) {
 			if (hb + 64u * W < cnt) loadw(hb + 64u * W, qb, yb);
+			if (SPLIT) refresh_lim32();
 			if (lim_seen != lim32) refresh_threshold();
 			if (pos - rdlane(qa[0], 0) - 1u >= dthr) break;
 			uint32_t prmask = 0;
@@ -630,20 +658,24 @@
 struct NbrRng { uint64_t key; uint32_t n; };
 __device__ __forceinline__ uint32_t nbr_draw(NbrRng& r) { return mgl_rng_draw(r.key, r.n++); }
 
-template <int W>
-__device__ bool pick_from_top_k(const DevCtx& c, const Walk& w, const uint16_t* probs, const uint16_t* T, uint32_t* lencost,
-                                mgl_pk incumbent, bool best, NbrRng& rng, uint32_t lane, mgl_pk* picked)
-{
-	TopK t;
-	topk_find<W>(t, c, w, probs, T, lencost, incumbent, lane);
+__device__ __forceinline__ bool topk_draw(const TopK& t, uint32_t pos, bool best, NbrRng& rng, mgl_pk* picked)
+{
 	const uint32_t count = t.count;
 	if (count == 0) return false;
 	uint32_t choice = nbr_draw(rng) % count;
 	for (int i = 0; i < 7; i++) { uint32_t x = nbr_draw(rng) % count; choice = x > choice ? x : choice; }
 	if (nbr_draw(rng) % 8u == 0 || best) choice = count - 1;
 	uint64_t key = shfl64(t.key, (int)(count - 1 - choice));
-	*picked = topk_packet(key, w.st.pos);
+	*picked = topk_packet(key, pos);
 	return true;
+}
+template <int W>
+__device__ bool pick_from_top_k(const DevCtx& c, const Walk& w, const uint16_t* probs, const uint16_t* T, uint32_t* lencost,
+                                mgl_pk incumbent, bool best, NbrRng& rng, uint32_t lane, mgl_pk* picked)
+{
+	TopK t;
+	topk_find<W>(t, c, w, probs, T, lencost, incumbent, lane);
+	return topk_draw(t, w.st.pos, best, rng, picked);
 }
 
 __device__ __forceinline__ bool long_rep_ok(const DevCtx& c, const Walk& w, uint32_t idx, uint32_t len, uint32_t lane)
diff --git a/megalania_amd/csrc/mgl_kernels2.hip b/megalania_amd/csrc/mgl_kernels2.hip
--- a/megalania_amd/csrc/mgl_kernels2.hip
+++ b/megalania_amd/csrc/mgl_kernels2.hip
@@ -518,19 +518,23 @@
 	return take;
 }
 
-__device__ void model_load(const DevCtx& c, const Base2& b, uint16_t* probs, const uint16_t* T, uint32_t y, uint32_t lane)
+__device__ __forceinline__ void model_copy(const Base2& b, uint16_t* probs, uint32_t y, uint32_t t, uint32_t nt)
 {
 	const uint32_t ck = y >> MGL_CK2_SHIFT;
 	const uint4* src = (const uint4*)(b.ck_probs + (size_t)ck * b.ck_elems);
 	uint4* dst = (uint4*)probs;
 	const uint32_t n16 = b.ck_elems / 8u;
-	for (uint32_t base = 0; base < n16; base += 256u) {
+	for (uint32_t base = 0; base < n16; base += 4u * nt) {
 		uint4 r[4];
 #pragma unroll
-		for (uint32_t u = 0; u < 4; u++) { const uint32_t i = base + u * 64u + lane; if (i < n16) r[u] = src[i]; }
+		for (uint32_t u = 0; u < 4; u++) { const uint32_t i = base + u * nt + t; if (i < n16) r[u] = src[i]; }
 #pragma unroll
-		for (uint32_t u = 0; u < 4; u++) { const uint32_t i = base + u * 64u + lane; if (i < n16) dst[i] = r[u]; }
-	}
+		for (uint32_t u = 0; u < 4; u++) { const uint32_t i = base + u * nt + t; if (i < n16) dst[i] = r[u]; }
+	}
+}
+__device__ void model_replay(const DevCtx& c, const Base2& b, uint16_t* probs, const uint16_t* T, uint32_t y, uint32_t lane)
+{
+	const uint32_t ck = y >> MGL_CK2_SHIFT;
 	const uint32_t first = ck << MGL_CK2_SHIFT;
 	const uint64_t bits = b.onwalk[first >> 6] & ((y & 63u) ? ((1ull << (y & 63u)) - 1ull) : 0ull) & (~0ull << (first & 63u));
 	wave_sync();
@@ -580,6 +584,11 @@
 		wave_sync();
 	}
 }
+__device__ __forceinline__ void model_load(const DevCtx& c, const Base2& b, uint16_t* probs, const uint16_t* T, uint32_t y, uint32_t lane)
+{
+	model_copy(b, probs, y, lane, 64u);
+	model_replay(c, b, probs, T, y, lane);
+}
 
 __device__ __forceinline__ void walk_from_state(Walk& w, const mgl_wstate& st)
 {
@@ -613,6 +622,83 @@
 #define MGL_REST_WAVES_PER_SIMD 4
 #endif
 #define MGL_SIM2_CAP 4096u
+
+#ifndef MGL_BIG_WAVES
+#define MGL_BIG_WAVES 4u
+#endif
+#define MGL_COOP_MAX_WAVES 8u
+static_assert(MGL_BIG_WAVES >= 1u && MGL_BIG_WAVES <= MGL_COOP_MAX_WAVES, "MGL_BIG_WAVES: 1 .. 8");
+#define MGL_ST_END 0u
+#define MGL_ST_MODEL 1u
+#define MGL_ST_SIM 2u
+#define MGL_ST_TOPK 3u
+struct Coop {
+	uint32_t stage, n_units;
+	uint32_t y;
+	uint32_t limit, cache;
+	uint32_t nu, too_many;
+	uint32_t pad;
+	Changes ch;
+	const uint16_t* g_ins_key; const uint32_t* g_ins_pos; const uint16_t* g_rem_key; const uint32_t* g_rem_pos;
+	uint16_t* overlay;
+	uint16_t* probs;
+	mgl_wstate st;
+	mgl_pk inc;
+	unsigned long long thr;
+	unsigned long long sum[MGL_COOP_MAX_WAVES];
+	unsigned long long keys[MGL_COOP_MAX_WAVES * 64u];
+};
+__host__ __device__ constexpr uint32_t coop_lds_bytes(uint32_t waves)
+{
+	return (uint32_t)((sizeof(Coop) + 15u) & ~(size_t)15u) + (waves - 1u) * MGL_PRICE_WORDS * 4u;
+}
+__device__ __forceinline__ void coop_model_stage(const Base2& b, Coop* co, uint32_t lane, uint32_t wid, uint32_t nw)
+{
+	model_copy(b, co->probs, co->y, wid * 64u + lane, nw * 64u);
+	__syncthreads();
+}
+__device__ __forceinline__ int64_t coop_sim_stage(const Base2& b, Coop* co, const uint16_t* T, uint32_t lane, uint32_t wid, uint32_t nw, bool* too_many)
+{
+	Changes ch = co->ch;
+	if (co->cache) {
+		const uint32_t t = wid * 64u + lane, nt = nw * 64u;
+		for (uint32_t e = t; e < ch.n_ins; e += nt) { ch.ins_pos[e] = co->g_ins_pos[e]; ch.ins_key[e] = co->g_ins_key[e]; }
+		for (uint32_t e = t; e < ch.n_rem; e += nt) { ch.rem_pos[e] = co->g_rem_pos[e]; ch.rem_key[e] = co->g_rem_key[e]; }
+	}
+	__syncthreads();
+	if (wid == 0) {
+		bool tm = false;
+		const uint32_t nu = chain_list(ch, lane, &tm);
+		if (lane == 0) { co->nu = nu; co->too_many = tm ? 1u : 0u; }
+	}
+	__syncthreads();
+	const uint32_t nu = uni(co->nu);
+	const bool tm = uni(co->too_many) != 0u;
+	int64_t d = 0;
+	if (!tm && ch.diag != 41) d = chain_sim_contexts(b, ch, T, co->limit, co->overlay, lane, wid * 64u, nw * 64u, nu);
+	const uint64_t u = wave_sum64((uint64_t)d);
+	if (lane == 0) co->sum[wid] = u;
+	__syncthreads();
+	if (tm) *too_many = true;
+	if (ch.diag == 41) return (int64_t)nu;
+	uint64_t s = 0;
+	for (uint32_t w = 0; w < nw; w++) s += co->sum[w];
+	return (int64_t)s;
+}
+__device__ __forceinline__ void coop_topk_stage(TopK& t, const DevCtx& c, const Base2& b, Coop* co, const uint16_t* T, uint32_t* lencost,
+                                                uint32_t lane, uint32_t wid, uint32_t nw)
+{
+	Walk tw;
+	walk_reset(tw);
+	tw.st = co->st;
+	tw.st = uni_state(tw.st);
+	walk_window(tw, c, b.slab, lane);
+	topk_find<1, true>(t, c, tw, co->probs, T, lencost, co->inc, lane, topk_sources_of(wid, nw), &co->thr);
+	if (wid != 0) co->keys[wid * 64u + lane] = lane < t.count ? t.key : MGL_INVALID_COST;
+	__syncthreads();
+	if (wid == 0)
+		for (uint32_t w = 1; w < nw; w++) topk_offer(t, co->keys[w * 64u + lane], lane);
+}
 #define MGL_NBR_FULL 0
 #define MGL_NBR_PICK 1
 #define MGL_NBR_REST 2
@@ -621,8 +707,10 @@
                                          uint64_t step_override, uint32_t K, const NbrOut& out, uint32_t per_wave_bytes,
                                          uint32_t* todo, uint32_t* todo_count, unsigned long long* prof_acc,
                                          const BigScratch& big, uint4* pickrec, uint32_t j_base, uint32_t j_end, uint4* pickstate,
-                                         unsigned char* smem, const uint16_t* T, uint32_t unit, uint32_t lane, uint32_t wid)
-{
+                                         unsigned char* smem, const uint16_t* T, uint32_t unit, uint32_t lane, uint32_t wid, Coop* co = nullptr)
+{
+	constexpr bool COOP = BIG && !LIST && MODE == MGL_NBR_FULL;
+	const uint32_t nw = COOP ? (blockDim.x >> 6) : 1u;
 	uint32_t j = j_base + unit;
 	uint32_t slot = 0;
 	const unsigned long long t_begin = prof_acc ? __builtin_readcyclecounter() : 0ull;
@@ -826,7 +914,14 @@
 				ch.cap = big.cap; ch.uctx_cap = big.uctx_cap;
 				spilled = true;
 			}
-			model_load(c, b, probs, T, pick_pos, lane);
+			if (COOP) {
+				if (lane == 0) { co->stage = MGL_ST_MODEL; co->y = pick_pos; co->probs = probs; }
+				__syncthreads();
+				coop_model_stage(b, co, lane, 0u, nw);
+				model_replay(c, b, probs, T, pick_pos, lane);
+			} else {
+				model_load(c, b, probs, T, pick_pos, lane);
+			}
 			if (!pick_is_mutation) prof_mark(prof, 5, lane);
 			if (pick_is_mutation) {
 				prof_mark(prof, 1, lane);
@@ -856,7 +951,22 @@
 		}
 		if (MODE == MGL_NBR_FULL && phase == P_SIM) {
 			int64_t r;
-			if (BIG && big.lds_cache && ch.n_ins <= MGL_BIG_CAP && ch.n_rem <= MGL_BIG_CAP) {
+			if (COOP) {
+				const bool cache = big.lds_cache && ch.n_ins <= MGL_BIG_CAP && ch.n_rem <= MGL_BIG_CAP;
+				if (lane == 0) {
+					Changes cl = ch;
+					if (cache) {
+						uint32_t* cp = (uint32_t*)(mine + per_wave_bytes);
+						cl.ins_pos = cp; cl.rem_pos = cp + MGL_BIG_CAP;
+						cl.ins_key = (uint16_t*)(cp + 2u * MGL_BIG_CAP); cl.rem_key = cl.ins_key + MGL_BIG_CAP;
+					}
+					co->stage = MGL_ST_SIM; co->ch = cl; co->cache = cache ? 1u : 0u;
+					co->g_ins_key = ch.ins_key; co->g_ins_pos = ch.ins_pos; co->g_rem_key = ch.rem_key; co->g_rem_pos = ch.rem_pos;
+					co->limit = sim_limit; co->overlay = sim_overlay ? probs : nullptr;
+				}
+				__syncthreads();
+				r = coop_sim_stage(b, co, T, lane, 0u, nw, &too_many);
+			} else if (BIG && big.lds_cache && ch.n_ins <= MGL_BIG_CAP && ch.n_rem <= MGL_BIG_CAP) {
 				uint32_t* cp = (uint32_t*)(mine + per_wave_bytes);
 				Changes cl = ch;
 				cl.ins_pos = cp; cl.rem_pos = cp + MGL_BIG_CAP;
@@ -874,10 +984,19 @@
 			else { delta = r; prof_mark(prof, 4, lane); phase = P_OUT; }
 		}
 		if (MODE != MGL_NBR_REST && phase == P_TOPK) {
-			walk_from_state(tw, nb);
-			walk_window(tw, c, b.slab, lane);
 			mgl_pk picked;
-			const bool ok = pick_from_top_k<(MODE == MGL_NBR_PICK ? 4 : 1)>(c, tw, probs, T, lencost, pick_inc, pick_best, rng, lane, &picked);
+			bool ok;
+			if (COOP) {
+				if (lane == 0) { co->stage = MGL_ST_TOPK; co->st = nb; co->inc = pick_inc; co->probs = probs; co->thr = MGL_INVALID_COST; }
+				__syncthreads();
+				TopK t;
+				coop_topk_stage(t, c, b, co, T, lencost, lane, 0u, nw);
+				ok = topk_draw(t, nb.pos, pick_best, rng, &picked);
+			} else {
+				walk_from_state(tw, nb);
+				walk_window(tw, c, b.slab, lane);
+				ok = pick_from_top_k<(MODE == MGL_NBR_PICK ? 4 : 1)>(c, tw, probs, T, lencost, pick_inc, pick_best, rng, lane, &picked);
+			}
 			if (MODE == MGL_NBR_PICK) {
 				if (lane == 0) pickrec[j] = make_uint4((uint32_t)picked, (uint32_t)(picked >> 32), rng.n, ok ? 1u : 0u);
 				return;
@@ -1104,12 +1223,13 @@
 }
 
 template <bool BIG, int MODE, bool LIST = false>
-__global__ void __launch_bounds__((MODE == MGL_NBR_PICK ? 512 : 64), (MODE == MGL_NBR_FULL ? (BIG ? 1 : MGL_NBR_WAVES_PER_SIMD) : (MODE == MGL_NBR_REST ? MGL_REST_WAVES_PER_SIMD : 4))) k_neighbours2(DevCtx c, Base2 b, Control* ctl, uint64_t seed,
+__global__ void __launch_bounds__((MODE == MGL_NBR_PICK ? 512 : ((BIG && !LIST && MODE == MGL_NBR_FULL) ? 64 * MGL_BIG_WAVES : 64)), (MODE == MGL_NBR_FULL ? (BIG ? 1 : MGL_NBR_WAVES_PER_SIMD) : (MODE == MGL_NBR_REST ? MGL_REST_WAVES_PER_SIMD : 4))) k_neighbours2(DevCtx c, Base2 b, Control* ctl, uint64_t seed,
                                                      uint64_t step_override, uint32_t K, NbrOut out, uint32_t per_wave_bytes,
                                                      uint32_t* todo, uint32_t* todo_count, unsigned long long* prof_acc,
                                                      BigScratch big, uint4* pickrec, uint32_t j_base, uint32_t j_end, uint4* pickstate)
 {
-	const uint32_t waves = blockDim.x >> 6;
+	constexpr bool COOP = BIG && !LIST && MODE == MGL_NBR_FULL;
+	const uint32_t waves = COOP ? 1u : blockDim.x >> 6;
 	if (BIG && blockIdx.x * waves + ((LIST && big.todo_first != nullptr) ? *big.todo_first : 0u) >= *big.todo_in_count) return;
 	if (!BIG && LIST && blockIdx.x * waves >= *big.la_count) return;
 	extern __shared__ __attribute__((aligned(16))) unsigned char smem[];
@@ -1121,7 +1241,32 @@
 		__syncthreads();
 	}
 	const uint32_t lane = threadIdx.x & 63u, wid = threadIdx.x >> 6;
-	if (BIG) {
+	if (COOP) {
+		Coop* co = (Coop*)(smem + 4096u + per_wave_bytes + 12u * MGL_BIG_CAP);
+		const uint32_t nw = blockDim.x >> 6;
+		if (threadIdx.x == 0) co->n_units = *big.todo_in_count;
+		__syncthreads();
+		const uint32_t n = uni(co->n_units);
+		for (uint32_t unit = blockIdx.x; unit < n; unit += gridDim.x) {
+			__syncthreads();
+			if (wid == 0) {
+				nbr2_one<BIG, MODE, LIST>(c, b, ctl, seed, step_override, K, out, per_wave_bytes, todo, todo_count, prof_acc, big, pickrec, j_base, j_end, pickstate, smem, T,
+				                          unit, lane, 0u, co);
+				if (lane == 0) co->stage = MGL_ST_END;
+				__syncthreads();
+			} else {
+				uint32_t* lencost = (uint32_t*)((unsigned char*)co + coop_lds_bytes(1u)) + (wid - 1u) * MGL_PRICE_WORDS;
+				for (;;) {
+					__syncthreads();
+					const uint32_t st = uni(*(volatile uint32_t*)&co->stage);
+					if (st == MGL_ST_MODEL) coop_model_stage(b, co, lane, wid, nw);
+					else if (st == MGL_ST_SIM) { bool tm = false; (void)coop_sim_stage(b, co, T, lane, wid, nw, &tm); }
+					else if (st == MGL_ST_TOPK) { TopK t; coop_topk_stage(t, c, b, co, T, lencost, lane, wid, nw); }
+					else break;
+				}
+			}
+		}
+	} else if (BIG) {
 		const uint32_t first = (LIST && big.todo_first != nullptr) ? *big.todo_first : 0u;
 		const uint32_t n = *big.todo_in_count > first ? *big.todo_in_count - first : 0u;
 		for (uint32_t unit = blockIdx.x * waves + wid; unit < n; unit += gridDim.x * waves)
```

Result: no change. 13.84 million (median of 6 runs) (+0.5%).
